# VIDILabs/instantvnr

Hardware: AMD Instinct MI355X
Metric: fps at 1024^2 on 1024^3 volume (higher is better)
Workload: dtype f16

## Files before the change

include/vnr_amd.h:

```cpp
#ifndef VNR_AMD_H
#define VNR_AMD_H

#include <stddef.h>
#include <stdint.h>

#ifdef __cplusplus
extern "C" {
#endif

#define VNR_AMD_OK 0
#define VNR_AMD_ERROR 1

typedef struct vnrAmdVolume_t*           vnrAmdVolume;
typedef struct vnrAmdRenderer_t*         vnrAmdRenderer;
typedef struct vnrAmdTransferFunction_t* vnrAmdTransferFunction;
typedef struct vnrAmdCamera_t*           vnrAmdCamera;

enum {
  VNR_AMD_OPTIX_NO_SHADING = 0,
  VNR_AMD_RAYMARCHING_NO_SHADING_DECODING = 4,
  VNR_AMD_RAYMARCHING_NO_SHADING_SAMPLE_STREAMING = 5,
  VNR_AMD_RAYMARCHING_NO_SHADING_IN_SHADER = 6,
  VNR_AMD_RAYMARCHING_GRADIENT_SHADING_SAMPLE_STREAMING = 8,
  VNR_AMD_RAYMARCHING_SINGLE_SHADE_HEURISTIC_SAMPLE_STREAMING = 11,
  VNR_AMD_PATHTRACING_SAMPLE_STREAMING = 14,
  VNR_AMD_INVALID = 16
};

enum {
  VNR_AMD_TYPE_UINT8 = 0, VNR_AMD_TYPE_INT8, VNR_AMD_TYPE_UINT16, VNR_AMD_TYPE_INT16,
  VNR_AMD_TYPE_UINT32, VNR_AMD_TYPE_INT32, VNR_AMD_TYPE_UINT64, VNR_AMD_TYPE_INT64,
  VNR_AMD_TYPE_FLOAT, VNR_AMD_TYPE_FLOAT2, VNR_AMD_TYPE_FLOAT3, VNR_AMD_TYPE_FLOAT4, VNR_AMD_TYPE_DOUBLE
};

enum {
  VNR_AMD_JSON_TEXT = 0,
  VNR_AMD_JSON_BSON = 1,
  VNR_AMD_JSON_TEXT_FILE = 2,
  VNR_AMD_JSON_BSON_FILE = 3
};

const char* vnrAmdGetLastError(void);
const char* vnrAmdVersion(void);
const char* vnrAmdBuildId(void);
int  vnrAmdInit(int device);
int  vnrAmdDeviceCount(void);
int  vnrAmdHasDevice(void);

void* vnrAmdMalloc(size_t bytes);
int   vnrAmdFree(void* d_ptr);
int   vnrAmdMemcpyH2D(void* d_dst, const void* h_src, size_t bytes);
int   vnrAmdMemcpyD2H(void* h_dst, const void* d_src, size_t bytes);
int   vnrAmdMemset(void* d_dst, int value, size_t bytes);
int   vnrAmdSynchronize(void);
void* vnrAmdDefaultStream(void);

int  vnrAmdJsonConvert(const void* data, size_t size, int format_in, int format_out ,
                       void** out, size_t* out_size);
int  vnrAmdJsonSave(const void* data, size_t size, int format_in, const char* filename, int format_out);
void vnrAmdFreeHost(void* p);

vnrAmdCamera vnrAmdCreateCamera(void);
int  vnrAmdCameraSet(vnrAmdCamera, const float from[3], const float at[3], const float up[3]);
int  vnrAmdCameraSetFromScene(vnrAmdCamera, const void* scene, size_t size, int format);
int  vnrAmdCameraSetFovy(vnrAmdCamera, float fovy_degrees);
int  vnrAmdCameraGet(vnrAmdCamera, float from[3], float at[3], float up[3], float* fovy);
void vnrAmdReleaseCamera(vnrAmdCamera);

vnrAmdTransferFunction vnrAmdCreateTransferFunction(void);
int  vnrAmdTransferFunctionSetColor(vnrAmdTransferFunction, const float* rgb, int n);
int  vnrAmdTransferFunctionSetAlpha(vnrAmdTransferFunction, const float* xy, int n);
int  vnrAmdTransferFunctionSetValueRange(vnrAmdTransferFunction, float lo, float hi);
int  vnrAmdTransferFunctionGetSizes(vnrAmdTransferFunction, int* n_colors, int* n_alphas);
int  vnrAmdTransferFunctionGet(vnrAmdTransferFunction, float* rgb, float* xy, float range[2]);
void vnrAmdReleaseTransferFunction(vnrAmdTransferFunction);

vnrAmdVolume vnrAmdCreateSimpleVolumeFromMemory(const void* host_data, const int dims[3], int value_type,
                                                float range_lo, float range_hi);
vnrAmdVolume vnrAmdCreateSimpleVolumeFromRawFile(const char* filename, const int dims[3], int value_type,
                                                 size_t offset, int big_endian, float range_lo, float range_hi);
vnrAmdVolume vnrAmdCreateSimpleVolumePerlin(const int dims[3], uint32_t seed, int octaves, float base_frequency);
const float* vnrAmdSimpleVolumeDeviceData(vnrAmdVolume);
vnrAmdVolume vnrAmdCreateSimpleVolumeOutOfCore(const char* filename, const int dims[3], int value_type, size_t offset,
                                               float range_lo, float range_hi, uint64_t n_concurrent_blocks, uint64_t n_blocks);
vnrAmdVolume vnrAmdCreateSimpleVolumeFromScene(const void* scene, size_t size, int format, const char* mode, int save_loaded_volume);
int  vnrAmdSimpleVolumeGetNumberOfTimeSteps(vnrAmdVolume);
int  vnrAmdSimpleVolumeSetCurrentTimeStep(vnrAmdVolume, int index);
int  vnrAmdSceneGetValueRange(const void* scene, size_t size, int format, float range[2]);
typedef struct vnrAmdOutOfCoreInfo {
  int file_dims[3];
  int block_dims[3];
  int block_index_space[3];
  uint64_t n_blocks, n_concurrent_blocks, block_size_aligned, bytes_read;
} vnrAmdOutOfCoreInfo;
int  vnrAmdSimpleVolumeOutOfCoreInfo(vnrAmdVolume, vnrAmdOutOfCoreInfo*);
int  vnrAmdSimpleVolumeOutOfCoreSetAsyncRefresh(vnrAmdVolume, int enable);
int  vnrAmdSimpleVolumeOutOfCoreRefreshStats(vnrAmdVolume, uint64_t* refreshes, uint64_t* steps_without_refresh);
int  vnrAmdSimpleVolumeOutOfCoreBlocks(vnrAmdVolume, int* block_index_yz, size_t n_slots);

vnrAmdVolume vnrAmdCreateNeuralVolume(const void* config, size_t size, int format, vnrAmdVolume groundtruth,
                                      int online_macrocell_construction);
vnrAmdVolume vnrAmdCreateNeuralVolumeFromDims(const void* config, size_t size, int format, const int dims[3]);
vnrAmdVolume vnrAmdCreateNeuralVolumeFromParams(const void* params, size_t size, int format);

int    vnrAmdNeuralVolumeSetModel(vnrAmdVolume, const void* config, size_t size, int format);
int    vnrAmdNeuralVolumeSetParams(vnrAmdVolume, const void* params, size_t size, int format);
double vnrAmdNeuralVolumeGetPSNR(vnrAmdVolume, int verbose);
double vnrAmdNeuralVolumeGetSSIM(vnrAmdVolume, int verbose);
double vnrAmdNeuralVolumeGetTestingLoss(vnrAmdVolume);
double vnrAmdNeuralVolumeGetTrainingLoss(vnrAmdVolume);
int    vnrAmdNeuralVolumeGetTrainingStep(vnrAmdVolume);
int    vnrAmdNeuralVolumeGetNumberOfBlobs(vnrAmdVolume);
int    vnrAmdNeuralVolumeTrain(vnrAmdVolume, int steps, int fast_mode);
int    vnrAmdNeuralVolumeDecodeProgressive(vnrAmdVolume);
int    vnrAmdNeuralVolumeDecodeInference(vnrAmdVolume, const char* filename);
int    vnrAmdNeuralVolumeDecodeReference(vnrAmdVolume, const char* filename);
const float* vnrAmdNeuralVolumeDecodedDeviceData(vnrAmdVolume);
int    vnrAmdNeuralVolumeSerializeParamsToFile(vnrAmdVolume, const char* filename);
int    vnrAmdNeuralVolumeSerializeParams(vnrAmdVolume, void** bson, size_t* size);

int    vnrAmdNeuralVolumeInference(vnrAmdVolume, size_t n, const float* d_coords, float* d_values, void* stream);
int    vnrAmdNeuralVolumeEncode(vnrAmdVolume, size_t n, const float* d_coords, uint16_t* d_features, void* stream);
int    vnrAmdNeuralVolumeBrickImageInfo(vnrAmdVolume, int* in_use, size_t* bytes, float* build_ms);
int    vnrAmdNeuralVolumeSetBrickImageMode(vnrAmdVolume, int mode);
int      vnrAmdNeuralVolumeSetBrickImageBudget(vnrAmdVolume, size_t bytes);
unsigned vnrAmdNeuralVolumeBrickImageLevels(vnrAmdVolume);
int      vnrAmdNeuralVolumeBrickImagePolicy(vnrAmdVolume, uint64_t* builds, unsigned* launches_before_next_build, int* tier, uint64_t* small_builds);
int      vnrAmdNeuralVolumeGridBackwardPlan(vnrAmdVolume, uint64_t batch, uint32_t out_u32[4], uint64_t out_u64[2]);
int      vnrAmdNeuralVolumeSetDeterministicTraining(vnrAmdVolume, int enable);
int      vnrAmdNeuralVolumeGetDeterministicTraining(vnrAmdVolume, int* enabled);
int    vnrAmdNeuralVolumeSetTrainProfiling(vnrAmdVolume, int enable);
int    vnrAmdNeuralVolumeGetTrainProfile(vnrAmdVolume, double ms_per_step[5], int* n_steps);
int    vnrAmdNeuralVolumeGetInfo(vnrAmdVolume, int* n_levels, int* n_features_per_level, int* padded_width,
                                 int* n_neurons, int* n_hidden_layers, uint64_t* n_params);
int    vnrAmdNeuralVolumeGetModelKind(vnrAmdVolume, int* activation, int* output_activation, int* grid_type, int* interpolation,
                                      int* mfma_inference, int* mfma_training);
int    vnrAmdNeuralVolumeLevelTable(vnrAmdVolume, int max_levels, uint32_t* resolution, uint32_t* entries, uint32_t* offset, uint32_t* kind);
int    vnrAmdNeuralVolumeGetParamsFP16(vnrAmdVolume, uint16_t* host_out, size_t count);
int    vnrAmdNeuralVolumeSetParamsFP16(vnrAmdVolume, const uint16_t* host_in, size_t count);

int    vnrAmdNeuralVolumeTrainBegin(vnrAmdVolume);
float* vnrAmdNeuralVolumeGradients(vnrAmdVolume, size_t* count);
int    vnrAmdNeuralVolumeTrainEnd(vnrAmdVolume, float grad_scale, int fast_mode);
int    vnrAmdNeuralVolumeForwardBackward(vnrAmdVolume, size_t n, const float* d_coords, const float* d_targets);
int    vnrAmdNeuralVolumeTrainingBuffer(vnrAmdVolume, int which, const void** d_ptr, size_t* bytes);
int    vnrAmdNeuralVolumeRescatterGridGradients(vnrAmdVolume, size_t n, const float* d_coords);
int    vnrAmdNeuralVolumeGradientDistance(vnrAmdVolume, const uint16_t* d_reference, double* out4);
int    vnrAmdNeuralVolumeSetSamplerSeed(vnrAmdVolume, uint64_t seed, uint64_t stream_id);
int    vnrAmdNeuralVolumeSetInitSeed(vnrAmdVolume, uint64_t seed);

int  vnrAmdVolumeSetClippingBox(vnrAmdVolume, const float lower[3], const float upper[3]);
int  vnrAmdVolumeSetScaling(vnrAmdVolume, const float scale[3]);
int  vnrAmdVolumeSetTransform(vnrAmdVolume, const float vx_vy_vz_p[12]);
int  vnrAmdSimpleVolumeGetDataRange(vnrAmdVolume, float range[2]);
int  vnrAmdVolumeGetValueRange(vnrAmdVolume, float range[2]);
int  vnrAmdVolumeGetDims(vnrAmdVolume, int dims[3]);
int  vnrAmdVolumeIsNetwork(vnrAmdVolume);
int  vnrAmdVolumeGetMacrocell(vnrAmdVolume, int mc_dims[3], float mc_spacings[3], const float** d_value_range,
                              const float** d_max_opacity);
void vnrAmdReleaseVolume(vnrAmdVolume);

vnrAmdRenderer vnrAmdCreateRenderer(vnrAmdVolume);
int  vnrAmdRendererSetFramebufferSize(vnrAmdRenderer, int width, int height);
int  vnrAmdRendererSetTransferFunction(vnrAmdRenderer, vnrAmdTransferFunction);
int  vnrAmdRendererSetCamera(vnrAmdRenderer, vnrAmdCamera);
int  vnrAmdRendererSetMode(vnrAmdRenderer, int mode);
int  vnrAmdRendererSetDenoiser(vnrAmdRenderer, int enable);
int  vnrAmdRendererSetVolumeSamplingRate(vnrAmdRenderer, float rate);
int  vnrAmdRendererSetVolumeDensityScale(vnrAmdRenderer, float scale);
int  vnrAmdRendererResetAccumulation(vnrAmdRenderer);
int  vnrAmdRender(vnrAmdRenderer);
const float* vnrAmdRendererMapFrame(vnrAmdRenderer);
int  vnrAmdRendererSetOutputAsDeviceFramebuffer(vnrAmdRenderer, int enable);
int  vnrAmdRendererSetPixelRange(vnrAmdRenderer, uint32_t pixel_lo, uint32_t pixel_hi);
int  vnrAmdRendererSetPixelInterleave(vnrAmdRenderer, uint32_t block_pixels, uint32_t n_parts, uint32_t part);

typedef struct {
  uint64_t n_samples;
  uint64_t n_reference_slots;
  uint32_t n_iterations;
  uint32_t n_rays_hit;
  double   infer_kernel_ms;
  uint64_t infer_kernel_launches;
  double   infer_union_ms;
} vnrAmdFrameStats;
int  vnrAmdRendererGetFrameStats(vnrAmdRenderer, vnrAmdFrameStats*);
int  vnrAmdRendererSetProfiling(vnrAmdRenderer, int enable);
int  vnrAmdRendererSetAsync(vnrAmdRenderer, int enable);
int  vnrAmdRendererSetInShaderKernel(vnrAmdRenderer, int mode);
int  vnrAmdRendererDebugQueues(vnrAmdRenderer, const float** d_coords, const uint32_t** d_counters, float* iteration_ms, int max_iterations);
int  vnrAmdRendererDebugSchedule(vnrAmdRenderer, int out[4]);
void vnrAmdReleaseRenderer(vnrAmdRenderer);

int  vnrAmdDistGetUniqueId(void* out128);
int  vnrAmdDistInit(int rank, int world_size, int local_rank, const void* unique_id, const char* transport, const char* address);
int  vnrAmdDistInitFromEnv(void);
int  vnrAmdDistFinalize(void);
int  vnrAmdDistRank(void);
int  vnrAmdDistWorldSize(void);
const char* vnrAmdDistTransport(void);
int  vnrAmdDistRcclRanksSeen(void);
int  vnrAmdDistBarrier(void);
int  vnrAmdDistAllReduceHost(double* values, int n, int op);
int  vnrAmdDistAllReduce(void* buf, size_t count, int dtype, int op);
int  vnrAmdDistAllGather(const void* send, void* recv, size_t bytes_per_rank);
int  vnrAmdDistReduceScatter(void* buf, size_t count_per_rank, int dtype);
int  vnrAmdDistBroadcast(void* buf, size_t bytes, int root);
int  vnrAmdDistSelfTest(double deadline_s, char* report, size_t report_size);
int  vnrAmdRendererSetDistributed(vnrAmdRenderer, int enable);
const float* vnrAmdRendererGatherFrame(vnrAmdRenderer);
int  vnrAmdRendererRenderPipelined(vnrAmdRenderer, const float** previous_frame);
int  vnrAmdRendererGetCompletedFrameStats(vnrAmdRenderer, vnrAmdFrameStats*);
int  vnrAmdRendererFlushPipeline(vnrAmdRenderer, const float** last_frame);
int  vnrAmdNeuralVolumeTrainDataParallel(vnrAmdVolume, int steps, int fast_mode);
int  vnrAmdNeuralVolumeSyncReplicas(vnrAmdVolume);
int  vnrAmdNeuralVolumeAllReduceGradients(vnrAmdVolume);
int  vnrAmdNeuralVolumeTrainEndDataParallel(vnrAmdVolume, int fast_mode, int sharded);
int  vnrAmdNeuralVolumeSetGradients(vnrAmdVolume, const float* host, size_t count);

int  vnrAmdMarchingCube(vnrAmdVolume, float isovalue, float** xyz, size_t* n_vertices, int on_device);
int  vnrAmdSaveTriangles(const char* filename, const float* xyz, size_t n_vertices);

void vnrAmdMemoryQuery(size_t* used_by_renderer, size_t* used_by_network);
void vnrAmdFreeTemporaryGPUMemory(void);

int  vnrAmdSimpleVolumeTakeSamples(vnrAmdVolume, size_t n, const float lower[3], const float upper[3],
                                   float* d_coords, float* d_values, void* stream);
int  vnrAmdSimpleVolumeTakeSamplesGrid(vnrAmdVolume, const int origin[3], const int size[3], float* d_coords, float* d_values,
                                       void* stream);
int  vnrAmdSimpleVolumeSample(vnrAmdVolume, size_t n, const float* d_coords, float* d_values, int nodal, void* stream);
int  vnrAmdNeuralVolumeUpdateMacrocell(vnrAmdVolume, size_t n, const float* d_coords, const float* d_values, void* stream);
int  vnrAmdVolumeUpdateMaxOpacity(vnrAmdVolume, vnrAmdTransferFunction);

#ifdef __cplusplus
}
#endif
#endif
```

instantvnr_amd/_lib.py:

```python
import ctypes as C
import os
import re
import subprocess
import sys

_HERE = os.path.dirname(os.path.abspath(__file__))
ROOT = os.path.dirname(_HERE)
SO_PATH = os.environ.get("VNR_AMD_LIB_PATH") or os.path.join(_HERE, "libvnr_amd.so")
HEADER = os.path.join(ROOT, "include", "vnr_amd.h")

_lib = None
_torch_imported_before_load = None


class VnrAmdError(RuntimeError):
    pass


def require_torch_loaded_first():
    if _lib is not None and not _torch_imported_before_load:
        raise VnrAmdError("libvnr_amd.so was loaded before `import torch`: PyTorch's bundled ROCm runtime cannot share the "
                          "GPU with the system runtime the library already initialised.  Import torch first (instantvnr_amd."
                          "dist.init_from_env does when WORLD_SIZE > 1; tests/conftest.py does for the test session).")


def build(force=False):
    args = ["make", "-C", os.path.join(_HERE, "csrc"), "-j8", "-s"]
    if force:
        subprocess.check_call(args + ["clean"])
    subprocess.check_call(args)
    return SO_PATH


class FrameStats(C.Structure):
    _fields_ = [("n_samples", C.c_uint64), ("n_reference_slots", C.c_uint64), ("n_iterations", C.c_uint32),
                ("n_rays_hit", C.c_uint32), ("infer_kernel_ms", C.c_double), ("infer_kernel_launches", C.c_uint64), ("infer_union_ms", C.c_double)]


class OutOfCoreInfo(C.Structure):
    _fields_ = [("file_dims", C.c_int * 3), ("block_dims", C.c_int * 3), ("block_index_space", C.c_int * 3),
                ("n_blocks", C.c_uint64), ("n_concurrent_blocks", C.c_uint64), ("block_size_aligned", C.c_uint64),
                ("bytes_read", C.c_uint64)]


def declared_symbols():
    text = open(HEADER).read()
    text = re.sub(r"/\*.*?\*/", "", text, flags=re.S)
    return sorted(set(re.findall(r"\b(vnrAmd[A-Za-z0-9_]+)\s*\(", text)))


def lib():
    global _lib
    if _lib is not None:
        return _lib
    if not os.path.exists(SO_PATH):
        raise VnrAmdError(f"{SO_PATH} is missing: run `python -c 'import __graft_entry__ as g; g.build()'` "
                          "(there is no CPU fallback)")
    global _torch_imported_before_load
    _torch_imported_before_load = "torch" in sys.modules
    L = C.CDLL(SO_PATH)
    P, I, U32, U64, F, D, SZ = C.c_void_p, C.c_int, C.c_uint32, C.c_uint64, C.c_float, C.c_double, C.c_size_t
    FP = C.POINTER(C.c_float)
    IP = C.POINTER(C.c_int)

    def sig(name, res, *args):
        fn = getattr(L, name)
        fn.restype = res
        fn.argtypes = list(args)

    sig("vnrAmdGetLastError", C.c_char_p)
    sig("vnrAmdBuildId", C.c_char_p)
    sig("vnrAmdVersion", C.c_char_p)
    sig("vnrAmdInit", I, I)
    sig("vnrAmdDeviceCount", I)
    sig("vnrAmdHasDevice", I)
    sig("vnrAmdMalloc", P, SZ)
    sig("vnrAmdFree", I, P)
    sig("vnrAmdMemcpyH2D", I, P, P, SZ)
    sig("vnrAmdMemcpyD2H", I, P, P, SZ)
    sig("vnrAmdMemset", I, P, I, SZ)
    sig("vnrAmdSynchronize", I)
    sig("vnrAmdDefaultStream", P)
    sig("vnrAmdJsonConvert", I, P, SZ, I, I, C.POINTER(P), C.POINTER(SZ))
    sig("vnrAmdJsonSave", I, P, SZ, I, C.c_char_p, I)
    sig("vnrAmdFreeHost", None, P)
    sig("vnrAmdCreateCamera", P)
    sig("vnrAmdCameraSet", I, P, FP, FP, FP)
    sig("vnrAmdCameraSetFovy", I, P, F)
    sig("vnrAmdCameraGet", I, P, FP, FP, FP, FP)
    sig("vnrAmdReleaseCamera", None, P)
    sig("vnrAmdCreateTransferFunction", P)
    sig("vnrAmdTransferFunctionSetColor", I, P, FP, I)
    sig("vnrAmdTransferFunctionSetAlpha", I, P, FP, I)
    sig("vnrAmdTransferFunctionSetValueRange", I, P, F, F)
    sig("vnrAmdTransferFunctionGetSizes", I, P, IP, IP)
    sig("vnrAmdTransferFunctionGet", I, P, FP, FP, FP)
    sig("vnrAmdReleaseTransferFunction", None, P)
    sig("vnrAmdCreateSimpleVolumeFromMemory", P, P, IP, I, F, F)
    sig("vnrAmdCreateSimpleVolumeFromRawFile", P, C.c_char_p, IP, I, SZ, I, F, F)
    sig("vnrAmdCreateSimpleVolumePerlin", P, IP, U32, I, F)
    sig("vnrAmdSimpleVolumeDeviceData", P, P)
    sig("vnrAmdCreateSimpleVolumeOutOfCore", P, C.c_char_p, IP, I, SZ, F, F, U64, U64)
    sig("vnrAmdCreateSimpleVolumeFromScene", P, P, SZ, I, C.c_char_p, I)
    sig("vnrAmdSimpleVolumeGetNumberOfTimeSteps", I, P)
    sig("vnrAmdSimpleVolumeSetCurrentTimeStep", I, P, I)
    sig("vnrAmdSceneGetValueRange", I, P, SZ, I, FP)
    sig("vnrAmdCameraSetFromScene", I, P, P, SZ, I)
    sig("vnrAmdSimpleVolumeOutOfCoreInfo", I, P, C.POINTER(OutOfCoreInfo))
    sig("vnrAmdSimpleVolumeOutOfCoreBlocks", I, P, IP, SZ)
    sig("vnrAmdSimpleVolumeOutOfCoreSetAsyncRefresh", I, P, I)
    sig("vnrAmdSimpleVolumeOutOfCoreRefreshStats", I, P, C.POINTER(C.c_uint64), C.POINTER(C.c_uint64))
    sig("vnrAmdCreateNeuralVolume", P, P, SZ, I, P, I)
    sig("vnrAmdCreateNeuralVolumeFromDims", P, P, SZ, I, IP)
    sig("vnrAmdCreateNeuralVolumeFromParams", P, P, SZ, I)
    sig("vnrAmdNeuralVolumeSetModel", I, P, P, SZ, I)
    sig("vnrAmdNeuralVolumeSetParams", I, P, P, SZ, I)
    sig("vnrAmdNeuralVolumeGetPSNR", D, P, I)
    sig("vnrAmdNeuralVolumeGetSSIM", D, P, I)
    sig("vnrAmdNeuralVolumeGetTestingLoss", D, P)
    sig("vnrAmdNeuralVolumeGetTrainingLoss", D, P)
    sig("vnrAmdNeuralVolumeGetTrainingStep", I, P)
    sig("vnrAmdNeuralVolumeGetNumberOfBlobs", I, P)
    sig("vnrAmdNeuralVolumeTrain", I, P, I, I)
    sig("vnrAmdNeuralVolumeSerializeParamsToFile", I, P, C.c_char_p)
    sig("vnrAmdNeuralVolumeDecodeProgressive", I, P)
    sig("vnrAmdNeuralVolumeDecodeInference", I, P, C.c_char_p)
    sig("vnrAmdNeuralVolumeDecodeReference", I, P, C.c_char_p)
    sig("vnrAmdNeuralVolumeDecodedDeviceData", P, P)
    sig("vnrAmdNeuralVolumeSerializeParams", I, P, C.POINTER(P), C.POINTER(SZ))
    sig("vnrAmdNeuralVolumeInference", I, P, SZ, P, P, P)
    sig("vnrAmdNeuralVolumeEncode", I, P, SZ, P, P, P)
    sig("vnrAmdNeuralVolumeBrickImageInfo", I, P, IP, C.POINTER(SZ), FP)
    sig("vnrAmdNeuralVolumeGetInfo", I, P, IP, IP, IP, IP, IP, C.POINTER(U64))
    sig("vnrAmdNeuralVolumeGetModelKind", I, P, IP, IP, IP, IP, IP, IP)
    sig("vnrAmdNeuralVolumeLevelTable", I, P, I, P, P, P, P)
    sig("vnrAmdNeuralVolumeGetParamsFP16", I, P, P, SZ)
    sig("vnrAmdNeuralVolumeSetParamsFP16", I, P, P, SZ)
    sig("vnrAmdNeuralVolumeTrainBegin", I, P)
    sig("vnrAmdNeuralVolumeGradients", P, P, C.POINTER(SZ))
    sig("vnrAmdNeuralVolumeTrainEnd", I, P, F, I)
    sig("vnrAmdNeuralVolumeForwardBackward", I, P, SZ, P, P)
    sig("vnrAmdNeuralVolumeTrainingBuffer", I, P, I, C.POINTER(P), C.POINTER(SZ))
    sig("vnrAmdNeuralVolumeRescatterGridGradients", I, P, SZ, P)
    sig("vnrAmdNeuralVolumeGradientDistance", I, P, P, C.POINTER(C.c_double))
    sig("vnrAmdNeuralVolumeSetSamplerSeed", I, P, U64, U64)
    sig("vnrAmdNeuralVolumeSetInitSeed", I, P, U64)
    sig("vnrAmdVolumeSetClippingBox", I, P, FP, FP)
    sig("vnrAmdVolumeSetScaling", I, P, FP)
    sig("vnrAmdVolumeSetTransform", I, P, FP)
    sig("vnrAmdSimpleVolumeGetDataRange", I, P, FP)
    sig("vnrAmdMarchingCube", I, P, F, C.POINTER(C.POINTER(C.c_float)), C.POINTER(SZ), I)
    sig("vnrAmdSaveTriangles", I, C.c_char_p, C.POINTER(C.c_float), SZ)
    sig("vnrAmdVolumeGetValueRange", I, P, FP)
    sig("vnrAmdVolumeGetDims", I, P, IP)
    sig("vnrAmdVolumeIsNetwork", I, P)
    sig("vnrAmdVolumeGetMacrocell", I, P, IP, FP, C.POINTER(P), C.POINTER(P))
    sig("vnrAmdReleaseVolume", None, P)
    sig("vnrAmdCreateRenderer", P, P)
    sig("vnrAmdRendererSetFramebufferSize", I, P, I, I)
    sig("vnrAmdRendererSetTransferFunction", I, P, P)
    sig("vnrAmdRendererSetCamera", I, P, P)
    sig("vnrAmdRendererSetMode", I, P, I)
    sig("vnrAmdRendererSetDenoiser", I, P, I)
    sig("vnrAmdRendererSetVolumeSamplingRate", I, P, F)
    sig("vnrAmdRendererSetVolumeDensityScale", I, P, F)
    sig("vnrAmdRendererResetAccumulation", I, P)
    sig("vnrAmdRender", I, P)
    sig("vnrAmdRendererMapFrame", P, P)
    sig("vnrAmdRendererSetOutputAsDeviceFramebuffer", I, P, I)
    sig("vnrAmdRendererSetPixelRange", I, P, U32, U32)
    sig("vnrAmdRendererSetPixelInterleave", I, P, U32, U32, U32)
    sig("vnrAmdRendererGetFrameStats", I, P, C.POINTER(FrameStats))
    sig("vnrAmdRendererSetProfiling", I, P, I)
    sig("vnrAmdRendererSetAsync", I, P, I)
    sig("vnrAmdRendererSetInShaderKernel", I, P, I)
    sig("vnrAmdRendererDebugQueues", I, P, C.POINTER(P), C.POINTER(P), FP, I)
    sig("vnrAmdRendererDebugSchedule", I, P, IP)
    sig("vnrAmdReleaseRenderer", None, P)
    sig("vnrAmdDistGetUniqueId", I, P)
    sig("vnrAmdDistInit", I, I, I, I, P, C.c_char_p, C.c_char_p)
    sig("vnrAmdDistInitFromEnv", I)
    sig("vnrAmdDistFinalize", I)
    sig("vnrAmdDistRank", I)
    sig("vnrAmdDistWorldSize", I)
    sig("vnrAmdDistTransport", C.c_char_p)
    sig("vnrAmdDistRcclRanksSeen", I)
    sig("vnrAmdDistBarrier", I)
    sig("vnrAmdDistAllReduceHost", I, C.POINTER(D), I, I)
    sig("vnrAmdDistAllReduce", I, P, SZ, I, I)
    sig("vnrAmdDistAllGather", I, P, P, SZ)
    sig("vnrAmdDistReduceScatter", I, P, SZ, I)
    sig("vnrAmdDistBroadcast", I, P, SZ, I)
    sig("vnrAmdDistSelfTest", I, C.c_double, C.c_char_p, SZ)
    sig("vnrAmdRendererSetDistributed", I, P, I)
    sig("vnrAmdRendererGatherFrame", P, P)
    sig("vnrAmdRendererRenderPipelined", I, P, C.POINTER(P))
    sig("vnrAmdRendererGetCompletedFrameStats", I, P, C.POINTER(FrameStats))
    sig("vnrAmdRendererFlushPipeline", I, P, C.POINTER(P))
    sig("vnrAmdNeuralVolumeTrainDataParallel", I, P, I, I)
    sig("vnrAmdNeuralVolumeSyncReplicas", I, P)
    sig("vnrAmdNeuralVolumeSetBrickImageMode", I, P, I)
    sig("vnrAmdNeuralVolumeSetBrickImageBudget", I, P, SZ)
    sig("vnrAmdNeuralVolumeBrickImageLevels", C.c_uint, P)
    sig("vnrAmdNeuralVolumeGridBackwardPlan", I, P, U64, C.POINTER(U32), C.POINTER(U64))
    sig("vnrAmdNeuralVolumeSetDeterministicTraining", I, P, I)
    sig("vnrAmdNeuralVolumeGetDeterministicTraining", I, P, C.POINTER(I))
    sig("vnrAmdNeuralVolumeBrickImagePolicy", I, P, C.POINTER(U64), C.POINTER(C.c_uint), IP, C.POINTER(U64))
    sig("vnrAmdNeuralVolumeSetTrainProfiling", I, P, I)
    sig("vnrAmdNeuralVolumeGetTrainProfile", I, P, C.POINTER(D), IP)
    sig("vnrAmdNeuralVolumeAllReduceGradients", I, P)
    sig("vnrAmdNeuralVolumeTrainEndDataParallel", I, P, I, I)
    sig("vnrAmdNeuralVolumeSetGradients", I, P, C.POINTER(C.c_float), SZ)
    sig("vnrAmdMemoryQuery", None, C.POINTER(SZ), C.POINTER(SZ))
    sig("vnrAmdFreeTemporaryGPUMemory", None)
    sig("vnrAmdSimpleVolumeTakeSamples", I, P, SZ, FP, FP, P, P, P)
    sig("vnrAmdSimpleVolumeTakeSamplesGrid", I, P, IP, IP, P, P, P)
    sig("vnrAmdSimpleVolumeSample", I, P, SZ, P, P, I, P)
    sig("vnrAmdNeuralVolumeUpdateMacrocell", I, P, SZ, P, P, P)
    sig("vnrAmdVolumeUpdateMaxOpacity", I, P, P)
    _lib = L
    return L


def last_error():
    return lib().vnrAmdGetLastError().decode("utf-8", "replace")


def check(status):
    if status != 0:
        raise VnrAmdError(last_error())


def check_ptr(p):
    if not p:
        raise VnrAmdError(last_error())
    return p


def require_device():
    if not lib().vnrAmdHasDevice():
        raise VnrAmdError("no HIP device: the MI355X path has no CPU fallback")
```

instantvnr_amd/api.py:

```python
import ctypes as C
import json

import numpy as np

from . import _lib
from ._lib import VnrAmdError, check, check_ptr, lib

JSON_TEXT, JSON_BSON, JSON_TEXT_FILE, JSON_BSON_FILE = 0, 1, 2, 3

VALUE_TYPES = {np.dtype(np.uint8): 0, np.dtype(np.int8): 1, np.dtype(np.uint16): 2, np.dtype(np.int16): 3,
               np.dtype(np.uint32): 4, np.dtype(np.int32): 5, np.dtype(np.float32): 8, np.dtype(np.float64): 12}


def _fp(a):
    return a.ctypes.data_as(C.POINTER(C.c_float))


def _vec(v, n=3):
    a = np.ascontiguousarray(v, dtype=np.float32).ravel()
    assert a.size == n
    return a


def _json_arg(j, params=False):
# ... 424 lines not shown
    check(lib().vnrAmdRendererSetFramebufferSize(r.h, int(size[0]), int(size[1])))
    r._size = (int(size[0]), int(size[1]))


def vnrRendererSetTransferFunction(r, t):
    check(lib().vnrAmdRendererSetTransferFunction(r.h, t.h))


def vnrRendererSetCamera(r, cam):
    check(lib().vnrAmdRendererSetCamera(r.h, cam.h))


def vnrRendererSetMode(r, mode):
    check(lib().vnrAmdRendererSetMode(r.h, int(mode)))


def vnrRendererSetDenoiser(r, flag):
    check(lib().vnrAmdRendererSetDenoiser(r.h, 1 if flag else 0))


def vnrRendererSetVolumeSamplingRate(r, v):
    check(lib().vnrAmdRendererSetVolumeSamplingRate(r.h, float(v)))


def vnrRendererSetVolumeDensityScale(r, v):
    check(lib().vnrAmdRendererSetVolumeDensityScale(r.h, float(v)))


def vnrRendererResetAccumulation(r):
    check(lib().vnrAmdRendererResetAccumulation(r.h))


def vnrRender(r):
    check(lib().vnrAmdRender(r.h))


def vnrRendererMapFrame(r):
    p = check_ptr(lib().vnrAmdRendererMapFrame(r.h))
    if r._device_output:
        return p
    w, h = r._size
    return np.ctypeslib.as_array(C.cast(p, C.POINTER(C.c_float)), shape=(h, w, 4))


def vnrMemoryQuery():
    r, n = C.c_size_t(), C.c_size_t()
    lib().vnrAmdMemoryQuery(C.byref(r), C.byref(n))
    return r.value, n.value


def vnrFreeTemporaryGPUMemory():
    lib().vnrAmdFreeTemporaryGPUMemory()


def vnrRendererSetPixelRange(r, lo, hi):
    check(lib().vnrAmdRendererSetPixelRange(r.h, int(lo), int(hi)))


def vnrRendererSetPixelInterleave(r, block_pixels, n_parts, part):
    check(lib().vnrAmdRendererSetPixelInterleave(r.h, int(block_pixels), int(n_parts), int(part)))


def vnrRendererSetOutputAsDeviceFramebuffer(r, flag):
    check(lib().vnrAmdRendererSetOutputAsDeviceFramebuffer(r.h, 1 if flag else 0))
    r._device_output = bool(flag)


def vnrRendererSetProfiling(r, flag):
    check(lib().vnrAmdRendererSetProfiling(r.h, 1 if flag else 0))


def vnrRendererGetFrameStats(r):
    s = _lib.FrameStats()
    check(lib().vnrAmdRendererGetFrameStats(r.h, C.byref(s)))
    return {k: getattr(s, k) for k, _ in s._fields_}


def renderer_schedule(r):
    out = (C.c_int * 4)()
    check(lib().vnrAmdRendererDebugSchedule(r.h, out))
    return {"n_iters": out[0], "n_parts": out[1], "fused_pack": bool(out[2]), "decoupled": bool(out[3])}


def neural_brick_image(v):
    u, b, ms = C.c_int(), C.c_size_t(), C.c_float()
    check(lib().vnrAmdNeuralVolumeBrickImageInfo(v.h, C.byref(u), C.byref(b), C.byref(ms)))
    builds, after, tier, small = C.c_uint64(), C.c_uint(), C.c_int(), C.c_uint64()
    check(lib().vnrAmdNeuralVolumeBrickImagePolicy(v.h, C.byref(builds), C.byref(after), C.byref(tier), C.byref(small)))
    return {"in_use": bool(u.value), "bytes": b.value, "build_ms": ms.value, "levels": int(lib().vnrAmdNeuralVolumeBrickImageLevels(v.h)),
            "builds": int(builds.value), "launches_before_next_build": int(after.value), "tier": int(tier.value), "small_builds": int(small.value)}


def neural_set_brick_budget(v, n_bytes):
    check(lib().vnrAmdNeuralVolumeSetBrickImageBudget(v.h, int(n_bytes)))


def neural_info(v):
    vals = [C.c_int() for _ in range(5)]
    n = C.c_uint64()
    check(lib().vnrAmdNeuralVolumeGetInfo(v.h, *[C.byref(x) for x in vals], C.byref(n)))
    keys = ["n_levels", "n_features_per_level", "padded_width", "n_neurons", "n_hidden_layers"]
    d = {k: x.value for k, x in zip(keys, vals)}
    d["n_params"] = n.value
    kind = [C.c_int() for _ in range(6)]
    check(lib().vnrAmdNeuralVolumeGetModelKind(v.h, *[C.byref(x) for x in kind]))
    d.update({k: x.value for k, x in zip(["activation", "output_activation", "grid_type", "interpolation", "mfma_kernels", "mfma_training_kernels"], kind)})
    return d


def neural_grid_backward_plan(v, batch=65536):
    u32, u64 = (C.c_uint32 * 4)(), (C.c_uint64 * 2)()
    check(lib().vnrAmdNeuralVolumeGridBackwardPlan(v.h, int(batch), u32, u64))
    return {"n_levels": u32[0], "lds_levels": u32[1], "tile_entries": u32[2], "lds_blocks": u32[3], "atomic_requests": int(u64[0]), "flush_requests_at_most": int(u64[1])}


def neural_set_deterministic_training(v, enable=True):
    check(lib().vnrAmdNeuralVolumeSetDeterministicTraining(v.h, 1 if enable else 0))


def neural_get_deterministic_training(v):
    e = C.c_int()
    check(lib().vnrAmdNeuralVolumeGetDeterministicTraining(v.h, C.byref(e)))
    return bool(e.value)


def neural_level_table(v):
    a = [np.zeros(32, np.uint32) for _ in range(4)]
    n = lib().vnrAmdNeuralVolumeLevelTable(v.h, 32, *[x.ctypes.data_as(C.c_void_p) for x in a])
    if n < 0:
        check(1)
    return [{"res": int(a[0][l]), "entries": int(a[1][l]), "offset": int(a[2][l]), "kind": int(a[3][l])} for l in range(n)]


def neural_set_params_fp16(v, params):
    p = np.ascontiguousarray(params).view(np.uint16)
    check(lib().vnrAmdNeuralVolumeSetParamsFP16(v.h, p.ctypes.data_as(C.c_void_p), p.size))


def neural_get_params_fp16(v):
    n = neural_info(v)["n_params"]
    p = np.empty(n, dtype=np.uint16)
    check(lib().vnrAmdNeuralVolumeGetParamsFP16(v.h, p.ctypes.data_as(C.c_void_p), n))
    return p.view(np.float16)


def neural_inference(v, coords):
    c = DeviceArray.from_numpy(np.ascontiguousarray(coords, dtype=np.float32))
    o = DeviceArray((c.shape[0],), np.float32)
    check(lib().vnrAmdNeuralVolumeInference(v.h, c.shape[0], c.ptr, o.ptr, None))
    check(lib().vnrAmdSynchronize())
    return o.numpy()


def neural_encode(v, coords):
    info = neural_info(v)
    c = DeviceArray.from_numpy(np.ascontiguousarray(coords, dtype=np.float32))
    o = DeviceArray((c.shape[0], info["padded_width"]), np.uint16)
    check(lib().vnrAmdNeuralVolumeEncode(v.h, c.shape[0], c.ptr, o.ptr, None))
    check(lib().vnrAmdSynchronize())
    return o.numpy().view(np.float16)


def volume_macrocell(v):
    dims = (C.c_int * 3)()
    sp = (C.c_float * 3)()
    vr, mo = C.c_void_p(), C.c_void_p()
    check(lib().vnrAmdVolumeGetMacrocell(v.h, dims, sp, C.byref(vr), C.byref(mo)))
    n = dims[0] * dims[1] * dims[2]
    value_range = np.empty((dims[2], dims[1], dims[0], 2), np.float32)
    max_opacity = np.empty((dims[2], dims[1], dims[0]), np.float32)
    check(lib().vnrAmdMemcpyD2H(value_range.ctypes.data_as(C.c_void_p), vr, n * 8))
    check(lib().vnrAmdMemcpyD2H(max_opacity.ctypes.data_as(C.c_void_p), mo, n * 4))
    return {"dims": tuple(dims), "spacings": np.array(list(sp), np.float32), "value_range": value_range,
            "max_opacity": max_opacity}


def simple_volume_sample(v, coords, nodal):
    c = DeviceArray.from_numpy(np.ascontiguousarray(coords, dtype=np.float32))
    o = DeviceArray((c.shape[0],), np.float32)
    check(lib().vnrAmdSimpleVolumeSample(v.h, c.shape[0], c.ptr, o.ptr, 1 if nodal else 0, None))
    check(lib().vnrAmdSynchronize())
    return o.numpy()


def simple_volume_take_samples_grid(v, origin, size):
    n = int(size[0]) * int(size[1]) * int(size[2])
    c = DeviceArray((n, 3), np.float32)
    o = DeviceArray((n,), np.float32)
    check(lib().vnrAmdSimpleVolumeTakeSamplesGrid(v.h, (C.c_int * 3)(*[int(x) for x in origin]), (C.c_int * 3)(*[int(x) for x in size]),
                                                  c.ptr, o.ptr, None))
    check(lib().vnrAmdSynchronize())
    return c.numpy(), o.numpy()


def simple_volume_take_samples(v, n, lower=(0, 0, 0), upper=(1, 1, 1)):
    c = DeviceArray((n, 3), np.float32)
    o = DeviceArray((n,), np.float32)
    check(lib().vnrAmdSimpleVolumeTakeSamples(v.h, n, _fp(_vec(lower)), _fp(_vec(upper)), c.ptr, o.ptr, None))
    check(lib().vnrAmdSynchronize())
    return c.numpy(), o.numpy()


def neural_forward_backward(v, coords, targets):
    c = DeviceArray.from_numpy(np.ascontiguousarray(coords, dtype=np.float32))
    t = DeviceArray.from_numpy(np.ascontiguousarray(targets, dtype=np.float32))
    check(lib().vnrAmdNeuralVolumeForwardBackward(v.h, c.shape[0], c.ptr, t.ptr))
    return neural_gradients(v)


def neural_gradients(v):
    n = C.c_size_t()
    p = check_ptr(lib().vnrAmdNeuralVolumeGradients(v.h, C.byref(n)))
    check(lib().vnrAmdSynchronize())
    out = np.empty(n.value, np.float32)
    check(lib().vnrAmdMemcpyD2H(out.ctypes.data_as(C.c_void_p), p, n.value * 4))
    return out


def neural_train_begin(v):
    check(lib().vnrAmdNeuralVolumeTrainBegin(v.h))


def neural_train_end(v, grad_scale=1.0, fast_mode=True):
    check(lib().vnrAmdNeuralVolumeTrainEnd(v.h, float(grad_scale), 1 if fast_mode else 0))
```

instantvnr_amd/csrc/capi.cpp:

```cpp
#include "../../include/vnr_amd.h"

#include <cstdlib>
#include <cstdio>
#include <fstream>
#include <memory>

#include "dist.h"
#include "renderer.h"
#include "scene.h"

using namespace vnr;

struct vnrAmdVolume_t { std::shared_ptr<VolumeBase> v; };
struct vnrAmdRenderer_t { std::unique_ptr<Renderer> r; std::shared_ptr<VolumeBase> volume; };
struct vnrAmdTransferFunction_t { TransferFunctionData d; };
struct vnrAmdCamera_t { CameraData d; };

namespace {
thread_local std::string g_last_error;

template <typename F>
int guarded(F&& f)
{
  try {
// ... 380 lines not shown
    for (size_t i = 0; i < b.size(); ++i) { block_index_yz[2 * i] = b[i].index_y; block_index_yz[2 * i + 1] = b[i].index_z; }
  });
}
const float* vnrAmdSimpleVolumeDeviceData(vnrAmdVolume v)
{
  const float* p = nullptr;
  guarded([&]() { p = as_simple(v)->d_data(); });
  return p;
}

vnrAmdVolume vnrAmdCreateNeuralVolume(const void* config, size_t size, int format, vnrAmdVolume groundtruth, int online_mc)
{
  return guarded_new<vnrAmdVolume_t>([&]() {
    SimpleVolume* src = as_simple(groundtruth);
    const Json cfg = resolve_config(parse_json_arg(config, size, format));
    auto nv = std::make_shared<NeuralVolume>();
    if (const char* e = std::getenv("VNR_AMD_INIT_SEED")) nv->init_seed = std::strtoull(e, nullptr, 10);
    nv->keep_source_alive(groundtruth->v);
    nv->set_network(src->dims(), cfg, src, !online_mc);
    auto* h = new vnrAmdVolume_t();
    h->v = nv;
    return h;
  });
}
vnrAmdVolume vnrAmdCreateNeuralVolumeFromDims(const void* config, size_t size, int format, const int dims[3])
{
  return guarded_new<vnrAmdVolume_t>([&]() {
    const Json cfg = resolve_config(parse_json_arg(config, size, format));
    auto nv = std::make_shared<NeuralVolume>();
    if (const char* e = std::getenv("VNR_AMD_INIT_SEED")) nv->init_seed = std::strtoull(e, nullptr, 10);
    nv->set_network({dims[0], dims[1], dims[2]}, cfg, nullptr, false);
    auto* h = new vnrAmdVolume_t();
    h->v = nv;
    return h;
  });
}
vnrAmdVolume vnrAmdCreateNeuralVolumeFromParams(const void* params, size_t size, int format)
{
  return guarded_new<vnrAmdVolume_t>([&]() {
    const Json p = resolve_params(parse_json_arg(params, size, format));
    if (!p.contains("volume")) throw std::runtime_error("expecting a model config with volume dims tag");
    const Json& d = p.at("volume").at("dims");
    const vec3i dims = {(int)d.at("x").as_int(), (int)d.at("y").as_int(), (int)d.at("z").as_int()};
    auto nv = std::make_shared<NeuralVolume>();
    nv->init_seed = 1;
    nv->set_network(dims, p.at("model"), nullptr, false);
    nv->load_params_from_json(p);
    auto* h = new vnrAmdVolume_t();
    h->v = nv;
    return h;
  });
}
int vnrAmdNeuralVolumeSetModel(vnrAmdVolume v, const void* config, size_t size, int format)
{
  return guarded([&]() { as_neural(v)->set_model(resolve_config(parse_json_arg(config, size, format))); });
}
int vnrAmdNeuralVolumeSetParams(vnrAmdVolume v, const void* params, size_t size, int format)
{
  return guarded([&]() { as_neural(v)->load_params_from_json(resolve_params(parse_json_arg(params, size, format))); });
}
double vnrAmdNeuralVolumeGetPSNR(vnrAmdVolume v, int verbose)
{
  double r = -1.0;
  guarded([&]() { r = as_neural(v)->get_psnr(!verbose); });
  return r;
}
double vnrAmdNeuralVolumeGetSSIM(vnrAmdVolume v, int verbose)
{
  double r = -1.0;
  guarded([&]() { r = as_neural(v)->get_ssim(!verbose); });
  return r;
}
double vnrAmdNeuralVolumeGetTestingLoss(vnrAmdVolume v)
{
  double r = -1.0;
  guarded([&]() { r = as_neural(v)->test_loss(); });
  return r;
}
double vnrAmdNeuralVolumeGetTrainingLoss(vnrAmdVolume v)
{
  double r = -1.0;
  guarded([&]() { NeuralVolume* n = as_neural(v); r = n->network().training_loss(n->stream); });
  return r;
}
int vnrAmdNeuralVolumeGetTrainingStep(vnrAmdVolume v)
{
  int r = -1;
  guarded([&]() { r = (int)as_neural(v)->network().steps(); });
  return r;
}
int vnrAmdNeuralVolumeGetNumberOfBlobs(vnrAmdVolume v)
{
  int r = -1;
  guarded([&]() { r = as_neural(v)->num_blobs(); });
  return r;
}
int vnrAmdNeuralVolumeTrain(vnrAmdVolume v, int steps, int fast_mode)
{
  return guarded([&]() { as_neural(v)->train((size_t)std::max(steps, 0), fast_mode != 0); });
}
int vnrAmdNeuralVolumeDecodeProgressive(vnrAmdVolume v)
{
  return guarded([&]() { as_neural(v)->decode_progressive(); });
}
int vnrAmdNeuralVolumeDecodeInference(vnrAmdVolume v, const char* filename)
{
  return guarded([&]() {
    if (!filename) throw std::runtime_error("filename is null");
    as_neural(v)->save_inference_volume(filename);
  });
}
int vnrAmdNeuralVolumeDecodeReference(vnrAmdVolume v, const char* filename)
{
  return guarded([&]() {
    if (!filename) throw std::runtime_error("filename is null");
    as_neural(v)->save_reference_volume(filename);
  });
}
const float* vnrAmdNeuralVolumeDecodedDeviceData(vnrAmdVolume v)
{
  const float* r = nullptr;
  guarded([&]() { r = as_neural(v)->decoded_data(); });
  return r;
}
int vnrAmdNeuralVolumeSerializeParamsToFile(vnrAmdVolume v, const char* filename)
{
  return guarded([&]() {
    Json root = Json::object();
    as_neural(v)->save_params_to_json(root);
    const std::vector<uint8_t> b = root.to_bson();
    std::ofstream ofs(filename, std::ios::binary | std::ios::out);
    ofs.write((const char*)b.data(), (std::streamsize)b.size());
    if (!ofs) throw std::runtime_error(std::string("cannot write ") + filename);
  });
}
int vnrAmdNeuralVolumeSerializeParams(vnrAmdVolume v, void** bson, size_t* size)
{
  return guarded([&]() {
    Json root = Json::object();
    as_neural(v)->save_params_to_json(root);
    const std::vector<uint8_t> b = root.to_bson();
    *bson = dup_bytes(b.data(), b.size());
    *size = b.size();
  });
}
int vnrAmdNeuralVolumeInference(vnrAmdVolume v, size_t n, const float* d_coords, float* d_values, void* stream)
{
  return guarded([&]() {
    NeuralVolume* nv = as_neural(v);
    if (!nv->network().valid()) throw std::runtime_error("network is not valid");
    nv->inference(n, d_coords, d_values, resolve_stream(stream));
  });
}
int vnrAmdNeuralVolumeEncode(vnrAmdVolume v, size_t n, const float* d_coords, uint16_t* d_features, void* stream)
{
  return guarded([&]() { as_neural(v)->network().encode(d_coords, d_features, n, resolve_stream(stream)); });
}
int vnrAmdNeuralVolumeBrickImageInfo(vnrAmdVolume v, int* in_use, size_t* bytes, float* build_ms)
{
  return guarded([&]() {
    Network& n = as_neural(v)->network();
    if (in_use) *in_use = n.brick_image_in_use() ? 1 : 0;
    if (bytes) *bytes = n.brick_image_bytes();
    if (build_ms) *build_ms = n.brick_build_ms();
  });
}
int vnrAmdNeuralVolumeGetModelKind(vnrAmdVolume v, int* activation, int* output_activation, int* grid_type, int* interpolation, int* mfma_inference,
                                   int* mfma_training)
{
  return guarded([&]() {
    Network& n = as_neural(v)->network();
    if (activation) *activation = (int)n.config().activation;
    if (output_activation) *output_activation = (int)n.config().output_activation;
    if (grid_type) *grid_type = (int)n.config().grid_type;
    if (interpolation) *interpolation = (int)n.config().interpolation;
    if (mfma_inference) *mfma_inference = 1;
    if (mfma_training) *mfma_training = 1;
  });
}

int vnrAmdNeuralVolumeGetInfo(vnrAmdVolume v, int* n_levels, int* n_features, int* padded_width, int* n_neurons,
                              int* n_hidden_layers, uint64_t* n_params)
{
  return guarded([&]() {
    Network& n = as_neural(v)->network();
    if (n_levels) *n_levels = (int)n.config().n_levels;
    if (n_features) *n_features = (int)n.config().n_features;
    if (padded_width) *padded_width = (int)n.padded_width();
    if (n_neurons) *n_neurons = (int)n.config().n_neurons;
    if (n_hidden_layers) *n_hidden_layers = (int)n.config().n_hidden_layers;
    if (n_params) *n_params = (uint64_t)n.n_params();
  });
}
int vnrAmdNeuralVolumeLevelTable(vnrAmdVolume v, int max_levels, uint32_t* resolution, uint32_t* entries, uint32_t* offset, uint32_t* kind)
{
  int n = -1;
  guarded([&]() {
    const Network& net = as_neural(v)->network();
    const GridDevice& g = net.grid();
    n = (int)net.config().n_levels;
    for (int l = 0; l < n && l < max_levels; ++l) {
      if (resolution) resolution[l] = g.levels[l].resolution;
      if (entries) entries[l] = g.levels[l].size;
      if (offset) offset[l] = g.levels[l].offset;
      if (kind) kind[l] = g.levels[l].hashed;
    }
  });
  return n;
}
int vnrAmdNeuralVolumeGetParamsFP16(vnrAmdVolume v, uint16_t* host_out, size_t count)
{
  return guarded([&]() { NeuralVolume* n = as_neural(v); n->network().get_params_f16(host_out, count, n->stream); });
}
int vnrAmdNeuralVolumeSetParamsFP16(vnrAmdVolume v, const uint16_t* host_in, size_t count)
{
  return guarded([&]() { NeuralVolume* n = as_neural(v); n->network().set_params_f16(host_in, count, n->stream); });
}
int vnrAmdNeuralVolumeTrainBegin(vnrAmdVolume v) { return guarded([&]() { as_neural(v)->train_begin(); }); }
float* vnrAmdNeuralVolumeGradients(vnrAmdVolume v, size_t* count)
{
  float* p = nullptr;
  guarded([&]() {
    NeuralVolume* nv = as_neural(v);
    Network& n = nv->network();
    p = n.grads_as_f32(nv->stream);
    if (count) *count = n.grads_count();
  });
  return p;
}
int vnrAmdNeuralVolumeTrainEnd(vnrAmdVolume v, float grad_scale, int fast_mode)
{
  return guarded([&]() { as_neural(v)->train_end(grad_scale, fast_mode != 0); });
}
int vnrAmdNeuralVolumeForwardBackward(vnrAmdVolume v, size_t n, const float* d_coords, const float* d_targets)
{
  return guarded([&]() { as_neural(v)->forward_backward(d_coords, d_targets, n); });
}
int vnrAmdNeuralVolumeTrainingBuffer(vnrAmdVolume v, int which, const void** d_ptr, size_t* bytes)
{
  return guarded([&]() {
    size_t b = 0;
    const void* p = as_neural(v)->network().training_buffer(which, &b);
    if (d_ptr) *d_ptr = p;
    if (bytes) *bytes = b;
  });
}
int vnrAmdNeuralVolumeRescatterGridGradients(vnrAmdVolume v, size_t n, const float* d_coords)
{
  return guarded([&]() { NeuralVolume* nv = as_neural(v); nv->network().rescatter_grid_gradients(d_coords, n, nv->stream); });
}
int vnrAmdNeuralVolumeGradientDistance(vnrAmdVolume v, const uint16_t* d_reference, double* out4)
{
  return guarded([&]() { NeuralVolume* nv = as_neural(v); nv->network().gradient_distance(d_reference, out4, nv->stream); });
}
int vnrAmdNeuralVolumeSetSamplerSeed(vnrAmdVolume v, uint64_t seed, uint64_t stream_id)
{
  return guarded([&]() {
    NeuralVolume* n = as_neural(v);
    if (!n->source()) throw std::runtime_error("missing a reference volume");
    n->source()->set_sampler_seed(seed, stream_id);
  });
}
int vnrAmdNeuralVolumeSetInitSeed(vnrAmdVolume v, uint64_t seed)
{
  return guarded([&]() { as_neural(v)->init_seed = seed; });
}

int vnrAmdVolumeSetClippingBox(vnrAmdVolume v, const float lower[3], const float upper[3])
{
  return guarded([&]() {
    if (!v || !v->v) throw std::runtime_error("null volume");
    VolumeBase& vb = *v->v;
    const vec3f half = {vb.desc.dims.x / 2.0f, vb.desc.dims.y / 2.0f, vb.desc.dims.z / 2.0f};
    const affine3f inv = affine_inverse(vb.transform);
    vb.clipbox.lower = xfm_point(inv, vec3f{lower[0], lower[1], lower[2]} - half);
    vb.clipbox.upper = xfm_point(inv, vec3f{upper[0], upper[1], upper[2]} - half);
  });
}
int vnrAmdVolumeSetScaling(vnrAmdVolume v, const float scale[3])
{
  return guarded([&]() {
    if (!v || !v->v) throw std::runtime_error("null volume");
    v->v->transform = affine_scale_then({scale[0], scale[1], scale[2]}, v->v->transform);
  });
}
int vnrAmdMarchingCube(vnrAmdVolume v, float isovalue, float** xyz, size_t* n_vertices, int on_device)
{
  return guarded([&]() {
    if (!v || !v->v) throw std::runtime_error("null volume");
    if (!xyz || !n_vertices) throw std::runtime_error("null output pointer");
    DeviceBuffer<vec3f> verts;
    const size_t n = marching_cubes(*v->v, isovalue, verts);
    *n_vertices = n;
    *xyz = nullptr;
    if (on_device) {
      *xyz = (float*)verts.ptr;
      verts.counter() -= verts.count * sizeof(vec3f);
      verts.ptr = nullptr; verts.count = 0;
    } else if (n) {
      float* h = (float*)std::malloc(n * sizeof(vec3f));
      if (!h) throw std::runtime_error("out of host memory");
      const hipError_t e = hipMemcpy(h, verts.ptr, n * sizeof(vec3f), hipMemcpyDeviceToHost);
      if (e != hipSuccess) { std::free(h); throw std::runtime_error("device to host copy of the vertices failed"); }
      *xyz = h;
    }
  });
// ... 344 lines not shown
```

instantvnr_amd/csrc/decoupled.h:

```cpp
#pragma once

namespace vnr {

struct DRays {
  uint32_t* pixel; float* jitter; vec3i* cell; vec3f* t_next; float* ncb; uint32_t* walking;
  float* alpha; vec3f* color; uint32_t* done;
};

enum { D_SAMPLES = 0, D_WALKING, D_HIT, D_TICKET_W, D_TICKET_C, D_NREF, D_NSMP, D_COUNT = 8 };
constexpr uint32_t kRecValid = 1u << 16, kRecLast = 1u << 17;

struct DRing {
  vec4f* queue;
  vec2f* arena;
  uint32_t* rec;
  uint32_t* ctr;
};

struct DHost {
  uint32_t walking[256], emitted[256], n_ref[256], n_smp[256];
  uint32_t hit;
};

template <bool FIRST>
__global__ void __launch_bounds__(256) walk_kernel(const RenderParams p, const DRays r, const DRing ring, DHost* __restrict__ host, uint32_t it)
{
  extern __shared__ float s_t[];
  float* s_t0 = s_t;
  float* s_t1 = s_t + (size_t)p.n_iters * 256;
  uint32_t* s_hist = (uint32_t*)(s_t + (size_t)2 * p.n_iters * 256);
  uint32_t* s_claim = s_hist + 256;
  uint16_t* s_rk = (uint16_t*)(s_claim + 16);
  const uint32_t tid = threadIdx.x, lane = tid & 63u;
  const uint32_t P = p.n_local;
  const uint32_t n_round = (P + 255u) & ~255u;
  uint32_t trip = 0;
  uint32_t n_walking = 0, n_hit = 0;
  vec4f* __restrict__ queue = ring.queue;
  vec2f* __restrict__ vd_out = ring.arena;

  for (uint32_t base = blockIdx.x * 256u; base < n_round; base += gridDim.x * 256u) {
    const uint32_t i = base + tid;
    const bool active = i < P;
    uint32_t pixel = 0;
    float jitter = 0.0f;
    DDAState it_;
    it_.t_next = {0, 0, 0}; it_.cell = {0, 0, 0}; it_.next_cell_begin = 0.0f;
    vec3f org = {0, 0, 0}, dir = {0, 0, 1}, m_dir = {0, 0, 1};
    float tmin = 0.0f, tmax = VNR_FLOAT_LARGE;
    bool walk = false;
    if (active) {
      if (FIRST) {
        if (map_pixel(p, i, pixel)) {
          jitter = tea_lcg_first((uint32_t)p.frame_index, pixel);
          compute_ray(p, pixel, org, dir);
          m_dir = dir * p.mc_rcp;
          walk = intersect_box(tmin, tmax, org, dir, p.bbox_lo, p.bbox_hi);
          if (walk) {
            dda_init(it_, org * p.mc_rcp, m_dir, tmin, p.mc_dims);
            r.pixel[i] = pixel; r.jitter[i] = jitter;
            r.alpha[i] = 0.0f; r.color[i] = {0, 0, 0}; r.done[i] = 0u;
            ++n_hit;
          } else {
            write_pixel(p, {0, 0, 0, 0}, pixel);
          }
        }
      } else if (r.walking[i]) {
        if (r.done[i]) {
          r.walking[i] = 0u;
        } else {
          pixel = r.pixel[i];
          jitter = r.jitter[i];
          it_.cell = r.cell[i];
          it_.t_next = r.t_next[i];
          it_.next_cell_begin = r.ncb[i];
          compute_ray(p, pixel, org, dir);
          m_dir = dir * p.mc_rcp;
          intersect_box(tmin, tmax, org, dir, p.bbox_lo, p.bbox_hi);
          walk = true;
        }
      }
    }
    uint32_t k = 0;
    bool last = false;
    if (walk) {
      const int n_iters = p.n_iters;
      iter_exec(p, it_, m_dir, tmin, tmax, p.step, [&](float t0, float t1) -> bool {
        s_t0[k * 256u + tid] = t0;
        s_t1[k * 256u + tid] = t1;
        return (int)(++k) < n_iters;
      });
      last = k == 0 || !dda_resumable(it_, m_dir, tmin, tmax, p.mc_dims);
      r.walking[i] = last ? 0u : 1u;
      if (!last) { r.cell[i] = it_.cell; r.t_next[i] = it_.t_next; r.ncb[i] = it_.next_cell_begin; ++n_walking; }
    } else if (FIRST && active) {
      r.walking[i] = 0u;
    }
    if (active) ring.rec[i] = walk ? (k | kRecValid | (last ? kRecLast : 0u)) : 0u;

    uint32_t incl = k;
#pragma unroll
    for (int d = 1; d < 64; d <<= 1) {
      const uint32_t y = __shfl_up(incl, d);
      if ((int)lane >= d) incl += y;
    }
    const uint32_t wave_samples = __shfl(incl, 63);
    uint32_t* claim = s_claim + 8u * (trip & 1u);
    if (lane == 0) claim[tid >> 6] = wave_samples;
    __syncthreads();
    if (tid == 0) {
      const uint32_t total = claim[0] + claim[1] + claim[2] + claim[3];
      claim[4] = total ? atomicAdd(ring.ctr + D_SAMPLES, total) : 0u;
    }
    __syncthreads();
    uint32_t smp_base = claim[4];
    for (uint32_t w = 0; w < (tid >> 6); ++w) smp_base += claim[w];
    ++trip;
    if (wave_samples == 0) continue;

    const bool emit = k > 0;
    float front = emit ? s_t0[tid] : VNR_FLOAT_LARGE;
#pragma unroll
    for (int d = 32; d > 0; d >>= 1) front = fminf(front, __shfl_xor(front, d));
    uint32_t* hist = s_hist + (tid & ~63u);
    hist[lane] = 0;
    __builtin_amdgcn_wave_barrier();
    if (emit) {
      for (uint32_t j = 0; j < k; ++j) {
        const float t0 = s_t0[j * 256u + tid], t1 = s_t1[j * 256u + tid];
        const float t = (1.0f - jitter) * t0 + jitter * t1;
        s_rk[j * 256u + tid] = (uint16_t)atomicAdd(&hist[depth_bin(p, t, front)], 1u);
      }
    }
    __builtin_amdgcn_wave_barrier();
    const uint32_t h = hist[lane];
    uint32_t hs = h;
#pragma unroll
    for (int d = 1; d < 64; d <<= 1) {
      const uint32_t y = __shfl_up(hs, d);
      if ((int)lane >= d) hs += y;
    }
    hist[lane] = smp_base + hs - h;
    __builtin_amdgcn_wave_barrier();
    if (emit) {
      const uint32_t sb = (i >> 6) * (uint32_t)p.n_iters * 64u + lane;
      for (uint32_t j = 0; j < k; ++j) {
        const float t0 = s_t0[j * 256u + tid], t1 = s_t1[j * 256u + tid];
        const float t = (1.0f - jitter) * t0 + jitter * t1;
        const vec3f c = org + t * dir;
        const uint32_t g = hist[depth_bin(p, t, front)] + s_rk[j * 256u + tid];
        if (g < p.slot_cap) queue[g] = {c.x, c.y, c.z, __uint_as_float(arena_value_index(sb + 64u * j))};
        vd_out[sb + 64u * j].y = t1 - t0;
      }
    }
    __builtin_amdgcn_wave_barrier();
  }

  __syncthreads();
#pragma unroll
  for (int d = 32; d > 0; d >>= 1) { n_walking += __shfl_xor(n_walking, d); n_hit += __shfl_xor(n_hit, d); }
  if (lane == 0) { s_hist[tid >> 6] = n_walking; s_hist[4 + (tid >> 6)] = n_hit; }
  __syncthreads();
// ... 100 lines not shown
```

instantvnr_amd/csrc/infer_kernel.h:

```cpp
#pragma once
#include <algorithm>
#include <cstdlib>

#include "infer_tile.h"
#include "pack_rays.h"

namespace vnr {

struct FusedMlp {
  const uint16_t* packed;
  uint32_t lds_halves, width, n_hidden_matmuls, activation, output_activation;
  bool general;
  bool weights_global;
  float quantize_threshold;
};

struct InferArgs {
  const LevelInfo* levels;
  uint32_t n_levels, interpolation;
  const half_t* table;
  uint32_t table_bytes;
  const uint8_t* brick_image;
  const half_t* packed_mlp;
  const float* coords;
  float* out;
  half_t* features_out;
  half_t* acts_out;
  const uint32_t* n_ptr;
  const uint32_t* dest;
  uint32_t queue_mode;
  uint32_t out_stride;
  uint32_t n;
  uint32_t n_hidden_matmuls;
  uint32_t activation;
  uint32_t output_activation;
  uint32_t lds_halves;
  uint32_t sharers;
  uint32_t weights_global;
  float quantize_threshold;
  PackArgs pack;
};

template <int F, int K_IN, int W, int MODE, bool GENERAL>
__global__ void __launch_bounds__(64 * MlpShape<W>::WAVES) fused_infer_kernel(const InferArgs args)
{
  constexpr int NCHUNK = K_IN / 8;
  constexpr uint32_t WAVES = MlpShape<W>::WAVES;
  extern __shared__ __attribute__((aligned(16))) half_t lds[];

  const uint32_t lane = threadIdx.x & 63u;
  const uint32_t wave = threadIdx.x >> 6;

  if (MODE == 0 && WAVES == 4 && args.pack.n_blocks) {
    uint32_t* s_part = (uint32_t*)lds;
    for (uint32_t item = blockIdx.x; item < args.pack.n_blocks; item += gridDim.x) {
      pack_rays_block<4>(args.pack, item, s_part);
      __syncthreads();
    }
  }
  const uint32_t n = args.n_ptr ? min(*args.n_ptr, args.n) : args.n;
  const uint32_t n_tiles = (n + 63u) >> 6;
  const uint32_t xcd = blockIdx.x & 7u;
  const uint32_t per_xcd = (n_tiles + 7u) >> 3;
  const uint32_t waves_per_xcd = (gridDim.x >> 3) * WAVES;
  const uint32_t tile_end = min(n_tiles, (xcd + 1u) * per_xcd);
  if (xcd * per_xcd + (blockIdx.x >> 3) * WAVES >= tile_end) return;

  constexpr bool CAN_GLOBAL = GENERAL;
  const bool wglobal = CAN_GLOBAL && args.weights_global != 0u;
  if (MODE != 1 && !wglobal) {
    const uint4_t* src = (const uint4_t*)args.packed_mlp;
    uint4_t* dst = (uint4_t*)lds;
    for (uint32_t i = threadIdx.x; i < args.lds_halves / 8; i += blockDim.x) dst[i] = src[i];
    __syncthreads();
  }
  const uint32_t nh = args.n_hidden_matmuls;
  const uint32_t act = args.activation;
  const uint32_t h = lane >> 5;
  const uint32_t r = lane & 31u;
  const table_rsrc_t rsrc = make_table_rsrc(args.table, args.table_bytes);

  for (uint32_t tile = xcd * per_xcd + (blockIdx.x >> 3) * WAVES + wave; tile < tile_end; tile += waves_per_xcd) {
    const uint32_t i = tile * 64u + lane;
    const uint32_t ic = min(i, n - 1u);
    float3_packed p;
    uint32_t out_index = i;
    if (args.queue_mode) {
      const uint4_t rec = ((const uint4_t*)args.coords)[ic];
      p = {__uint_as_float(rec.x), __uint_as_float(rec.y), __uint_as_float(rec.z)};
      out_index = rec.w * args.out_stride;
    } else {
      p = ((const float3_packed*)args.coords)[ic];
      if (args.dest) out_index = args.dest[ic];
    }

    half8_t feat[NCHUNK];
    encode_tile<F, K_IN, GENERAL>(args.levels, args.n_levels, args.interpolation, rsrc, args.brick_image, p.x, p.y, p.z, feat,
                                  GENERAL ? args.quantize_threshold : 0.0f);

    if (MODE != 0 && args.features_out && i < n) {
      half8_t* dst = (half8_t*)(args.features_out + (size_t)i * K_IN);
#pragma unroll
      for (int c = 0; c < NCHUNK; ++c) dst[c] = feat[c];
    }
    if (MODE == 1) continue;

    float y;
    if (CAN_GLOBAL && wglobal)
      y = mlp_tile<W, K_IN, MODE == 2, GENERAL>(args.packed_mlp, feat, nh, act, h, r, args.acts_out, n, tile * 64u);
    else
      y = mlp_tile<W, K_IN, MODE == 2, GENERAL>((const half_t*)lds, feat, nh, act, h, r, args.acts_out, n, tile * 64u);
    if (i < n) args.out[out_index] = finish_output<GENERAL>(y, args.output_activation);
  }
}

template <int F, int K_IN, int W, int MODE, bool GENERAL>
static void launch_one(const InferArgs& a, size_t n_max, hipStream_t s)
{
  constexpr uint32_t WAVES = MlpShape<W>::WAVES;
  const Runtime& rt = Runtime::get();
  const uint32_t n_tiles = div_round_up(n_max, 64);
  uint32_t blocks = div_round_up(n_tiles, WAVES);
  static const uint32_t forced = [] {
    const char* e = std::getenv("VNR_AMD_INFER_BLOCKS_PER_CU");
    const int v = e ? std::atoi(e) : 0;
    return (uint32_t)(v >= 1 && v <= 64 ? v : 0);
  }();
  const size_t shmem = (MODE == 1 || a.weights_global) ? 16 : (size_t)a.lds_halves * sizeof(uint16_t);
  const uint32_t fit = (uint32_t)std::max<size_t>(1, std::min<size_t>(4, (160 * 1024) / std::max<size_t>(shmem, 1)));
  uint32_t max_blocks = (uint32_t)rt.n_cus * (forced ? forced : std::min(fit, a.sharers >= 2 ? 3u : 4u));
  if (!forced && a.n_ptr && a.queue_mode) max_blocks = std::min((uint32_t)rt.n_cus * 32u, std::max((uint32_t)rt.n_cus * 4u, n_tiles / 33u));
  if (blocks > max_blocks) blocks = max_blocks;
  blocks = next_multiple(blocks, 8);
  auto kernel = fused_infer_kernel<F, K_IN, W, MODE, GENERAL>;
  static bool attr_set = false;
  if (!attr_set) {
    VNR_HIP_CHECK(hipFuncSetAttribute((const void*)kernel, hipFuncAttributeMaxDynamicSharedMemorySize, 160 * 1024));
    attr_set = true;
  }
  kernel<<<blocks, 64 * WAVES, shmem, s>>>(a);
  VNR_HIP_CHECK(hipGetLastError());
}

template <int W, int MODE, bool GENERAL>
static void dispatch(uint32_t F, uint32_t K_IN, const InferArgs& a, size_t n_max, hipStream_t s)
{
#define VNR_CASE(f, k) if (F == f && K_IN == k) return launch_one<f, k, W, MODE, GENERAL>(a, n_max, s)
  VNR_CASE(1, 16); VNR_CASE(1, 32);
  VNR_CASE(2, 16); VNR_CASE(2, 32); VNR_CASE(2, 48); VNR_CASE(2, 64);
  VNR_CASE(4, 16); VNR_CASE(4, 32); VNR_CASE(4, 48); VNR_CASE(4, 64); VNR_CASE(4, 80); VNR_CASE(4, 96); VNR_CASE(4, 112); VNR_CASE(4, 128);
  VNR_CASE(8, 16); VNR_CASE(8, 32); VNR_CASE(8, 48); VNR_CASE(8, 64); VNR_CASE(8, 80); VNR_CASE(8, 96); VNR_CASE(8, 112); VNR_CASE(8, 128);
#undef VNR_CASE
  throw std::runtime_error("unsupported encoding shape: n_features_per_level=" + std::to_string(F) +
                           " padded width=" + std::to_string(K_IN));
}

#define VNR_DEFINE_FUSED_WIDTH(W, GENERAL, SUFFIX)                                                                        \
  void launch_fused_w##W##SUFFIX(int mode, uint32_t F, uint32_t K_IN, const InferArgs& a, size_t n_max, hipStream_t s)    \
  {                                                                                                                       \
    if (mode == 0) dispatch<W, 0, GENERAL>(F, K_IN, a, n_max, s);                                                         \
    else dispatch<W, 2, GENERAL>(F, K_IN, a, n_max, s);                                                                   \
  }

}
```

instantvnr_amd/csrc/network.h:

```cpp
#pragma once

#include <functional>
#include <utility>
#include <vector>

#include "common.h"
#include "json.h"

namespace vnr {

constexpr int kMaxLevels = 32;
constexpr size_t kLdsBytes = 160 * 1024;
constexpr int kLossScale = 128;

struct LevelInfo {
  float scale;
  uint32_t resolution;
  uint32_t res2;
  uint32_t size;
  uint32_t offset;
  uint32_t hashed;
  uint32_t brick;
  uint32_t pad1;
};

template <int F> struct BrickShape;
template <> struct BrickShape<1> { static constexpr uint32_t lx = 2, ly = 2, lz = 2; };
template <> struct BrickShape<2> { static constexpr uint32_t lx = 2, ly = 2, lz = 1; };
template <> struct BrickShape<4> { static constexpr uint32_t lx = 2, ly = 1, lz = 1; };
template <> struct BrickShape<8> { static constexpr uint32_t lx = 1, ly = 1, lz = 1; };

struct GridDevice {
  LevelInfo levels[kMaxLevels];
  uint32_t n_levels;
  uint32_t n_features;
  uint32_t interpolation;
};

struct ModelConfig {
  uint32_t n_levels = 8, n_features = 8, log2_hashmap_size = 19, base_resolution = 16;
  float per_level_scale = 2.0f;
  uint32_t interpolation = 0;
  float quantize_threshold = 0.0f;
  float max_level = 1000.0f;
  uint32_t grid_type = 0;
  uint32_t n_neurons = 64, n_hidden_layers = 4;
  uint32_t activation = 1;
  uint32_t output_activation = 0;
  float learning_rate = 5e-3f, beta1 = 0.9f, beta2 = 0.999f, epsilon = 1e-15f, l2_reg = 1e-6f;
  uint32_t decay_start = 2000, decay_interval = 1000;
  float decay_base = 0.99f;
  bool has_decay = true;
  uint32_t loss = 0;
};

struct alignas(16) OptState {
  float master;
  float m, v;
  uint32_t step;
};
static_assert(sizeof(OptState) == 16, "OptState must be one 16-byte record");

struct TileNet;
struct PackArgs;
struct FusedMlp;

struct GradExchange {
  virtual ~GradExchange() = default;
  virtual void range_ready(size_t lo, size_t hi, hipStream_t s) = 0;
  virtual size_t bucket_params() const { return (size_t)16u << 20; }
};

struct GridBackwardPlan {
  uint32_t n_levels, lds_levels, tile_entries, lds_blocks;
  uint64_t atomic_requests, flush_requests_at_most;
};

class Network {
public:
  Network() = default;
  void configure(const Json& model, uint64_t init_seed);
  bool valid() const { return n_params_ > 0; }

  const ModelConfig& config() const { return cfg_; }
  const Json& model_json() const { return model_; }
  const GridDevice& grid() const { return grid_; }
  uint32_t padded_width() const { return in_width_; }
  uint32_t width() const { return cfg_.n_neurons; }
  uint32_t lds_halves() const { return lds_halves_; }
  bool weights_in_lds() const { return (size_t)lds_halves_ * 2 <= kLdsBytes; }
  bool common_kind() const
  {
    return cfg_.activation <= 1u && cfg_.output_activation == 0u && cfg_.interpolation != 2u && cfg_.grid_type != 2u && cfg_.quantize_threshold == 0.0f &&
           weights_in_lds();
  }
  uint32_t n_active_levels() const;
  uint32_t n_hidden_matmuls() const { return cfg_.n_hidden_layers - 1; }
  size_t n_params() const { return n_params_; }
  size_t n_mlp_params() const { return n_mlp_; }
  size_t n_grid_params() const { return n_params_ - n_mlp_; }
  size_t model_size_bytes() const { return n_params_ * sizeof(uint16_t); }
  uint64_t steps() const { return steps_; }

  void set_params_f16(const uint16_t* host, size_t count, hipStream_t s);
  void get_params_f16(uint16_t* host, size_t count, hipStream_t s) const;
  Json serialize_params(hipStream_t s) const;
  void deserialize_params(const Json& j, hipStream_t s);

  void inference(const float* d_coords, float* d_out, size_t n, const uint32_t* d_n, size_t n_max, hipStream_t s,
                 const uint32_t* d_dest = nullptr) const;
  bool tile_net(TileNet* out, hipStream_t s) const;
  bool inference_queue(const float* d_records, float* d_out, uint32_t out_stride, const uint32_t* d_n, size_t n_max, hipStream_t s,
                       uint32_t sharers = 1, const PackArgs* pack = nullptr) const;
  void encode(const float* d_coords, uint16_t* d_features, size_t n, hipStream_t s) const;

  void forward_backward(const float* d_coords, const float* d_targets, size_t batch, hipStream_t s, GradExchange* exchange = nullptr);
  uint16_t* grads_f16() { return grads_.ptr; }
  size_t grads_count() const { return grads_.count ? n_params_ : 0; }
  size_t grads_alloc() const { return n_params_ + (n_params_ & 1); }
  float* grads_as_f32(hipStream_t s);
  void optimizer_step(float grad_scale, hipStream_t s);
  void optimizer_step_range(size_t lo, size_t hi, float grad_scale, hipStream_t s);
  void optimizer_finish_step(hipStream_t s);
  float learning_rate() const { return lr_; }
  uint16_t* params_device() { return params_f16_.ptr; }
  OptState* opt_state_device() { return opt_state_.ptr; }
  void set_replica_state(uint64_t steps, float lr, hipStream_t s) { steps_ = steps; lr_ = lr; refresh_inference_weights(s); }
  void ensure_training_state(hipStream_t s);
  void reset_master_from_params(hipStream_t s);
  double training_loss(hipStream_t s);
  uint64_t params_generation() const { return params_generation_; }
  void set_opt_sharded(bool e) { opt_sharded_ = e; }
  bool opt_sharded() const { return opt_sharded_; }
  void set_deterministic(bool e) { deterministic_ = e; }
  bool deterministic() const { return deterministic_; }
  static bool deterministic_default();
  std::vector<std::pair<uint32_t, uint32_t>> exchange_level_buckets(size_t bucket) const;
  void for_each_exchange_range(size_t bucket, const std::function<void(size_t, size_t)>& fn) const;
  size_t level_range_lo(uint32_t level) const { return n_mlp_ + (size_t)grid_.levels[level].offset * cfg_.n_features; }
  size_t level_range_hi(uint32_t level_end) const { return n_mlp_ + ((size_t)grid_.levels[level_end - 1].offset + grid_.levels[level_end - 1].size) * cfg_.n_features; }
  const void* training_buffer(int which, size_t* bytes) const;
  void rescatter_grid_gradients(const float* d_coords, size_t n, hipStream_t s);
  void gradient_distance(const uint16_t* d_ref, double out[4], hipStream_t s);
  void scatter_grid_gradients(const float* d_coords, size_t batch, hipStream_t s, GradExchange* exchange, hipStream_t s_lds = nullptr);
  void set_grads_from_f32(const float* host, size_t count, hipStream_t s);

  size_t bytes_allocated() const;
  void release_temporary();
  static void release_temporary_of_all();

  void set_brick_resolution_cap(uint32_t cap) { brick_res_cap_ = cap; }
  void set_brick_mode(int mode);
  void set_brick_budget(size_t bytes);
  GridBackwardPlan grid_backward_plan(size_t batch) const;
  uint32_t brick_levels_mask() const { return brick_levels_mask_; }
  bool brick_image_in_use() const { return brick_valid_; }
  size_t brick_image_bytes() const { return brick_image_.bytes(); }
  float brick_build_ms() const { return brick_build_ms_; }
  uint64_t brick_builds() const { return brick_builds_; }
  uint64_t brick_small_builds() const { return brick_small_builds_; }
  int brick_tier() const { return brick_valid_ ? brick_tier_ : 0; }
  uint32_t brick_after_now() const;

private:
  void build_layout();
  void initialize_params(uint64_t seed, hipStream_t s);
  void refresh_inference_weights(hipStream_t s);
  FusedMlp fused_mlp() const;
  const LevelInfo* inference_levels(hipStream_t s, const uint8_t** image, size_t n_max) const;
  void build_brick_image(hipStream_t s, bool small) const;
  static double brick_small_budget();

  ModelConfig cfg_;
  Json model_;
  GridDevice grid_{};
  uint32_t in_width_ = 0;
  size_t n_params_ = 0, n_mlp_ = 0;
  uint64_t steps_ = 0;
  uint64_t params_generation_ = 0;
  bool opt_sharded_ = false;
  bool deterministic_ = deterministic_default();
  float lr_ = 0.0f;

  DeviceBuffer<uint16_t> params_f16_{MemTag::Network};
  DeviceBuffer<uint16_t> mlp_packed_{MemTag::Network};
  DeviceBuffer<uint16_t> mlp_packed_T_{MemTag::Network};
  DeviceBuffer<LevelInfo> levels_dev_{MemTag::Network};
  DeviceBuffer<OptState> opt_state_{MemTag::Network};
  DeviceBuffer<uint16_t> grads_{MemTag::Network};
  DeviceBuffer<float> grads_f32_{MemTag::Network};
  DeviceBuffer<uint16_t> ws_features_{MemTag::Network};
  DeviceBuffer<uint16_t> ws_acts_{MemTag::Network};
  DeviceBuffer<uint16_t> ws_dfeat_{MemTag::Network};
  DeviceBuffer<float> ws_loss_{MemTag::Network};
  size_t ws_batch_ = 0;
  hipStream_t side_stream_ = nullptr;
  hipEvent_t ev_fork_ = nullptr, ev_join_ = nullptr;
  uint32_t lds_halves_ = 0, lds_halves_T_ = 0;
  mutable DeviceBuffer<uint8_t> brick_image_{MemTag::Network};
  mutable DeviceBuffer<LevelInfo> levels_brick_dev_{MemTag::Network};
  mutable bool brick_valid_ = false, brick_refused_ = false;
  mutable uint32_t brick_stable_calls_ = 0;
  static constexpr uint32_t kBrickPaysAfter = 64;
  mutable uint32_t brick_served_calls_ = 0, brick_after_scale_ = 1;
  mutable uint64_t brick_builds_ = 0;
  static constexpr size_t kBrickSmallMinLaunch = (size_t)1 << 20;
  mutable int brick_tier_ = 0;
  mutable bool brick_small_refused_ = false;
  mutable uint64_t brick_small_builds_ = 0;
  mutable float brick_build_ms_ = 0.0f;
  uint32_t brick_res_cap_ = 0;
  size_t brick_budget_ = 0;
  mutable uint32_t brick_levels_mask_ = 0;
  int brick_mode_ = -1;

public:
  static constexpr int kTrainPhases = 5, kTrainProfileSteps = 64;
  void set_train_profiling(bool e);
  int train_profile(double* ms_per_step );
private:
  void profile_mark(int phase_boundary, hipStream_t s);
  bool train_profiling_ = false;
  std::vector<hipEvent_t> prof_events_;
  uint64_t prof_steps_ = 0;

public:
  ~Network();
  Network(const Network&) = delete;
  Network& operator=(const Network&) = delete;
};

uint32_t grid_make_layout(const ModelConfig& cfg, GridDevice* out);

}
```

instantvnr_amd/csrc/network_host.hip:

```cpp
#include "network.h"

#include <algorithm>
#include <cstdlib>
#include <set>

#include "infer_kernel.h"

namespace vnr {

void launch_pack_mlp(const uint16_t* params, uint16_t* packed, uint16_t* packedT, uint32_t in_width, uint32_t W, uint32_t n_hidden_matmuls, hipStream_t s);
void launch_fused(int mode, const GridDevice& grid, uint32_t in_width, const FusedMlp& mlp, const LevelInfo* d_levels, const uint16_t* table, size_t table_bytes,
                  const float* coords, float* out, uint16_t* features_out, uint16_t* acts_out, size_t n, const uint32_t* d_n, size_t n_max, hipStream_t s,
                  const uint32_t* d_dest = nullptr, uint32_t queue_out_stride = 0, const uint8_t* brick_image = nullptr,
                  uint32_t sharers = 1, const struct PackArgs* pack = nullptr);
void launch_init_params(OptState* state, uint16_t* params, size_t n_mlp, size_t n_total, uint32_t in_width,
                        uint32_t n_hidden_matmuls, uint32_t width, uint64_t seed, hipStream_t s);
void launch_master_from_f16(const uint16_t* params, OptState* state, size_t n, bool reset_optimizer, hipStream_t s);

uint16_t f32_to_f16(float f)
{
  uint32_t x;
  std::memcpy(&x, &f, 4);
  const uint32_t sign = (x >> 16) & 0x8000u;
  const uint32_t ax = x & 0x7fffffffu;
  if (ax >= 0x7f800000u) return (uint16_t)(sign | 0x7c00u | ((ax > 0x7f800000u) ? (0x200u | ((ax >> 13) & 0x3ffu)) : 0u));
  if (ax >= 0x477ff000u) return (uint16_t)(sign | 0x7c00u);
  if (ax < 0x33000001u) return (uint16_t)sign;
  const int32_t e = (int32_t)(ax >> 23) - 127;
  const uint32_t m = (ax & 0x7fffffu) | 0x800000u;
  const uint32_t shift = e < -14 ? (uint32_t)(-1 - e) : 13u;
  const uint32_t he = e < -14 ? 0u : (uint32_t)(e + 15);
  uint32_t q = m >> shift;
  const uint32_t rem = m & ((1u << shift) - 1u), half = 1u << (shift - 1);
  if (rem > half || (rem == half && (q & 1u))) q++;
  return (uint16_t)(sign | (he == 0 ? q : ((he - 1) << 10) + q));
}

float f16_to_f32(uint16_t h)
{
  const uint32_t sign = ((uint32_t)h & 0x8000u) << 16, e = (h >> 10) & 0x1fu, m = h & 0x3ffu;
  uint32_t x;
  if (e == 0) {
    if (m == 0) x = sign;
    else { float v = (float)m * 5.9604644775390625e-8f; std::memcpy(&x, &v, 4); x |= sign; }
  } else if (e == 31) x = sign | 0x7f800000u | (m << 13);
  else x = sign | ((e + 112u) << 23) | (m << 13);
  float f;
  std::memcpy(&f, &x, 4);
  return f;
}

uint32_t grid_make_layout(const ModelConfig& cfg, GridDevice* out)
{
  if (cfg.n_levels > (uint32_t)kMaxLevels) throw std::runtime_error("too many hash-grid levels");
  const float log2_pls = std::log2(cfg.per_level_scale);
  uint32_t offset = 0;
  for (uint32_t l = 0; l < cfg.n_levels; ++l) {
    const float scale = exp2f((float)l * log2_pls) * (float)cfg.base_resolution - 1.0f;
    const uint32_t res = (uint32_t)ceilf(scale) + 1u;
    const uint32_t max_params = 0xffffffffu / 2u;
    const double cube = (double)res * (double)res * (double)res;
    uint32_t n = cube > (double)max_params ? max_params : (uint32_t)cube;
    n = next_multiple(n, 8u);
    if (cfg.grid_type == 2u) {
      const double tile = (double)cfg.base_resolution * cfg.base_resolution * cfg.base_resolution;
      if ((double)n > tile) n = (uint32_t)tile;
    } else if (cfg.grid_type == 0u) {
      const uint32_t cap = 1u << cfg.log2_hashmap_size;
      if (n > cap) n = cap;
    }
    if (n == 0) throw std::runtime_error("grid level without entries");
    uint32_t stride = 1, dims = 0;
    for (; dims < 3 && stride <= n; ++dims) stride *= res;
    LevelInfo& lv = out->levels[l];
    lv.scale = scale;
    lv.resolution = res;
    lv.res2 = res * res;
    lv.size = n;
    lv.offset = offset;
    if (cfg.grid_type == 0u) lv.hashed = n < stride ? 1u : 0u;
    else lv.hashed = (dims == 3 && (uint64_t)res * res * res <= (uint64_t)n) ? 0u : 1u + dims;
    lv.brick = lv.pad1 = 0;
    if (lv.hashed == 1u && (n & (n - 1)) != 0) throw std::runtime_error("internal: hashed level with non power-of-two size");
    if ((uint64_t)offset + n > 0xffffffffull) throw std::runtime_error("grid encoding too large (more than 2^32 entries)");
    offset += n;
  }
  out->n_levels = cfg.n_levels;
  out->n_features = cfg.n_features;
  out->interpolation = cfg.interpolation;
  return offset;
}

static std::set<Network*>& live_networks()
{
  static std::set<Network*> s;
  return s;
}

static uint32_t json_u32(const Json& j, const char* key, uint32_t def) { return j.contains(key) ? (uint32_t)j.at(key).as_int() : def; }
static float json_f32(const Json& j, const char* key, float def) { return j.contains(key) ? j.at(key).as_float() : def; }
static std::string json_str(const Json& j, const char* key, const char* def) { return j.contains(key) ? j.at(key).as_string() : std::string(def); }

void Network::configure(const Json& config, uint64_t init_seed)
{
  const Json loss = config.value("loss", Json::object());
  const Json enc = config.value("encoding", Json::object());
  const Json net = config.value("network", Json::object());
  ModelConfig c = cfg_;
  if (config.contains("optimizer")) {
    const Json& opt = config.at("optimizer");
    const std::string ot = json_str(opt, "otype", "Adam");
    const Json* adam = &opt;
    if (ot == "ExponentialDecay") {
      c.has_decay = true;
      c.decay_start = json_u32(opt, "decay_start", 10000);
      c.decay_interval = json_u32(opt, "decay_interval", 10000);
      c.decay_base = json_f32(opt, "decay_base", 0.33f);
      if (!opt.contains("nested")) throw std::runtime_error("ExponentialDecay optimizer needs a 'nested' optimizer");
      adam = &opt.at("nested");
    } else {
      c.has_decay = false;
    }
    if (json_str(*adam, "otype", "Adam") != "Adam") throw std::runtime_error("unsupported optimizer otype (Adam / ExponentialDecay{Adam} only)");
    c.learning_rate = json_f32(*adam, "learning_rate", 1e-3f);
    c.beta1 = json_f32(*adam, "beta1", 0.9f);
    c.beta2 = json_f32(*adam, "beta2", 0.999f);
    c.epsilon = json_f32(*adam, "epsilon", 1e-8f);
    c.l2_reg = json_f32(*adam, "l2_reg", 1e-8f);
  }
  const std::string lt = json_str(loss, "otype", "L2");
  if (lt == "L1") c.loss = 0;
  else if (lt == "L2") c.loss = 1;
  else throw std::runtime_error("unsupported loss otype: " + lt);

  const std::string et = json_str(enc, "otype", "");
  if (et != "HashGrid" && et != "Grid" && et != "DenseGrid" && et != "TiledGrid")
    throw std::runtime_error("unsupported encoding otype: '" + et + "' (HashGrid / Grid / DenseGrid / TiledGrid)");
  const std::string gt = json_str(enc, "type", et == "DenseGrid" ? "Dense" : et == "TiledGrid" ? "Tiled" : "Hash");
  if (gt == "Hash") c.grid_type = 0;
  else if (gt == "Dense") c.grid_type = 1;
  else if (gt == "Tiled") c.grid_type = 2;
  else throw std::runtime_error("unsupported grid type: " + gt + " (Hash / Dense / Tiled)");
  c.n_levels = json_u32(enc, "n_levels", 16);
  c.n_features = json_u32(enc, "n_features_per_level", 2);
  c.log2_hashmap_size = json_u32(enc, "log2_hashmap_size", 19);
  c.base_resolution = json_u32(enc, "base_resolution", 16);
  c.per_level_scale = json_f32(enc, "per_level_scale", 2.0f);
  const std::string it = json_str(enc, "interpolation", "Linear");
  if (it == "Linear") c.interpolation = 0;
  else if (it == "Smoothstep") c.interpolation = 1;
  else if (it == "Nearest") c.interpolation = 2;
  else throw std::runtime_error("unsupported interpolation: " + it);
  c.quantize_threshold = json_f32(enc, "quantize_threshold", 0.0f);
  c.max_level = json_f32(enc, "max_level", 1000.0f);
  if (c.n_features != 1 && c.n_features != 2 && c.n_features != 4 && c.n_features != 8)
    throw std::runtime_error("n_features_per_level must be 1, 2, 4 or 8");
  if (c.log2_hashmap_size > 28) throw std::runtime_error("log2_hashmap_size too large");

  const std::string nt = json_str(net, "otype", "FullyFusedMLP");
  if (nt != "FullyFusedMLP") throw std::runtime_error("unsupported network otype: " + nt + " (FullyFusedMLP only)");
  c.n_neurons = json_u32(net, "n_neurons", 128);
  c.n_hidden_layers = json_u32(net, "n_hidden_layers", 5);
  if (c.n_neurons != 16 && c.n_neurons != 32 && c.n_neurons != 64 && c.n_neurons != 128)
    throw std::runtime_error("FullyFusedMLP n_neurons must be 16, 32, 64 or 128");
  if (c.n_hidden_layers < 1) throw std::runtime_error("n_hidden_layers must be >= 1");
  auto activation_of = [](const std::string& a, const char* what) -> uint32_t {
    if (a == "None") return kActNone;
// ... 289 lines not shown
  if (small) policy = std::min(policy, brick_small_budget());
  const uint64_t budget_lines = (uint64_t)std::min(policy, (double)(free_b + brick_image_.bytes()) / 4.0) / 128u;
  const uint32_t mask_before = brick_valid_ ? brick_levels_mask_ : 0u;
  brick_levels_mask_ = 0;
  hipEvent_t t0, t1;
  VNR_HIP_CHECK(hipEventCreate(&t0)); VNR_HIP_CHECK(hipEventCreate(&t1));
  const uint32_t F = cfg_.n_features;
  const uint32_t lx = F == 8 ? 1 : 2, ly = F >= 4 ? 1 : 2, lz = F == 1 ? 2 : 1;
  const uint64_t entries_per_line = 64u / F;
  std::vector<LevelInfo> lv(grid_.levels, grid_.levels + kMaxLevels);
  std::vector<uint64_t> lines(kMaxLevels, 0);
  uint64_t used = 0;
  const bool finest_first = F <= 2;
  for (int k = 0; k < (int)grid_.n_levels; ++k) {
    const int l = finest_first ? (int)grid_.n_levels - 1 - k : k;
    if (lv[l].hashed != 1u) continue;
    if (brick_res_cap_ && lv[l].resolution > brick_res_cap_ + 1u) continue;
    const uint64_t res = lv[l].resolution;
    uint64_t n = ((res >> lx) + 1) * ((res >> ly) + 1) * ((res >> lz) + 1);
    if (F == 2) {
      if (res >= 13000) continue;
      n = (res / 7 + 1) * ((res >> 1) + 1) * ((res >> 1) + 1);
      lv[l].pad1 = (uint32_t)(res / 7 + 1);
    }
    if (n * entries_per_line >= (1ull << 32) || used + n + 1 > budget_lines || used + n + 1 >= 0xffffffffull) continue;
    lv[l].brick = (uint32_t)used + 1u;
    lines[l] = n;
    used += n;
    brick_levels_mask_ |= 1u << l;
  }
  if (used == 0) {
    if (!small) brick_refused_ = true;
    else brick_small_refused_ = true;
    brick_valid_ = false;
    (void)hipEventDestroy(t0); (void)hipEventDestroy(t1);
    return;
  }
  if (!small && brick_valid_ && mask_before == brick_levels_mask_ && brick_image_.bytes() == (used + 1) * 128u) {
    brick_tier_ = 2;
    (void)hipEventDestroy(t0); (void)hipEventDestroy(t1);
    return;
  }
  if (brick_image_.bytes() != (used + 1) * 128u) {
    if (brick_image_.bytes()) VNR_HIP_CHECK(hipDeviceSynchronize());
    brick_valid_ = false;
  }
  brick_image_.resize((used + 1) * 128u);
  VNR_HIP_CHECK(hipEventRecord(t0, s));
  for (uint32_t l = 0; l < grid_.n_levels; ++l) {
    if (!lv[l].brick) continue;
    const uint64_t n_entries = lines[l] * entries_per_line;
    const uint16_t* table = params_f16_.ptr + n_mlp_;
    switch (F) {
    case 1: launch_brick_build<1>(lv[l], table, brick_image_.ptr, n_entries, s); break;
    case 2: launch_brick_build<2>(lv[l], table, brick_image_.ptr, n_entries, s); break;
    case 4: launch_brick_build<4>(lv[l], table, brick_image_.ptr, n_entries, s); break;
    default: launch_brick_build<8>(lv[l], table, brick_image_.ptr, n_entries, s); break;
    }
  }
  VNR_HIP_CHECK(hipMemsetAsync(brick_image_.ptr + used * 128u, 0, 128, s));
  levels_brick_dev_.resize(kMaxLevels);
  VNR_HIP_CHECK(hipMemcpyAsync(levels_brick_dev_.ptr, lv.data(), kMaxLevels * sizeof(LevelInfo), hipMemcpyHostToDevice, s));
  VNR_HIP_CHECK(hipEventRecord(t1, s));
  VNR_HIP_CHECK(hipEventSynchronize(t1));
  VNR_HIP_CHECK(hipEventElapsedTime(&brick_build_ms_, t0, t1));
  (void)hipEventDestroy(t0); (void)hipEventDestroy(t1);
  brick_valid_ = true;
  brick_tier_ = small ? 1 : 2;
}

const LevelInfo* Network::inference_levels(hipStream_t s, const uint8_t** image, size_t n_max) const
{
  static const int env_mode = [] { const char* e = std::getenv("VNR_AMD_BRICK"); return e ? std::atoi(e) : -1; }();
  const int mode = brick_mode_ >= 0 ? brick_mode_ : env_mode;
  *image = nullptr;
  if (mode == 0 || brick_refused_) return levels_dev_.ptr;
  if (brick_tier_ != 2 || !brick_valid_) {
    if (brick_stable_calls_ < 0xffffffffu) ++brick_stable_calls_;
    const bool want_full = mode == 1 || brick_stable_calls_ > brick_after_now();
    if (want_full) {
      build_brick_image(s, false);
      if (brick_valid_ && brick_tier_ == 2) { ++brick_builds_; brick_served_calls_ = 0; }
    } else if (!brick_valid_ && !brick_small_refused_ && n_max >= kBrickSmallMinLaunch && brick_small_budget() > 0.0 && cfg_.n_features <= 2u) {
      build_brick_image(s, true);
      if (brick_valid_) ++brick_small_builds_;
    }
    if (!brick_valid_) return levels_dev_.ptr;
  }
  if (brick_served_calls_ < 0xffffffffu) ++brick_served_calls_;
  *image = brick_image_.ptr;
  return levels_brick_dev_.ptr;
}

void Network::set_params_f16(const uint16_t* host, size_t count, hipStream_t s)
{
  if (count != n_params_) throw std::runtime_error("parameter count mismatch: got " + std::to_string(count) + ", model has " + std::to_string(n_params_));
  VNR_HIP_CHECK(hipMemcpyAsync(params_f16_.ptr, host, count * sizeof(uint16_t), hipMemcpyHostToDevice, s));
  if (opt_state_.count == n_params_) launch_master_from_f16(params_f16_.ptr, opt_state_.ptr, n_params_, false, s);
  ++params_generation_;
  refresh_inference_weights(s);
  VNR_HIP_CHECK(hipStreamSynchronize(s));
}

void Network::get_params_f16(uint16_t* host, size_t count, hipStream_t s) const
{
  if (count != n_params_) throw std::runtime_error("parameter count mismatch");
  VNR_HIP_CHECK(hipMemcpyAsync(host, params_f16_.ptr, count * sizeof(uint16_t), hipMemcpyDeviceToHost, s));
  VNR_HIP_CHECK(hipStreamSynchronize(s));
}

Json Network::serialize_params(hipStream_t s) const
{
  std::vector<uint16_t> host(n_params_);
  get_params_f16(host.data(), n_params_, s);
  Json j = Json::object();
  j["n_params"] = (uint64_t)n_params_;
  j["params_type"] = "__half";
  j["params_binary"] = Json::binary(host.data(), host.size() * sizeof(uint16_t));
  return j;
}

void Network::deserialize_params(const Json& j, hipStream_t s)
{
  const size_t n = (size_t)j.at("n_params").as_int();
  if (n != n_params_) throw std::runtime_error("Can't set params because buffer has the wrong size: " + std::to_string(n) + " vs " + std::to_string(n_params_));
  const std::string type = j.at("params_type").as_string();
  const std::string& bin = j.at("params_binary").as_binary();
  std::vector<uint16_t> host(n);
  if (type == "__half") {
    if (bin.size() != n * 2) throw std::runtime_error("params_binary has the wrong size");
    std::memcpy(host.data(), bin.data(), n * 2);
  } else if (type == "float") {
    if (bin.size() != n * 4) throw std::runtime_error("params_binary has the wrong size");
    const float* f = (const float*)bin.data();
    for (size_t i = 0; i < n; ++i) host[i] = f32_to_f16(f[i]);
  } else {
    throw std::runtime_error("Unknown params_type: " + type);
  }
  set_params_f16(host.data(), n, s);
  if (j.contains("optimizer") || j.contains("step")) {  }
}

void Network::inference(const float* d_coords, float* d_out, size_t n, const uint32_t* d_n, size_t n_max, hipStream_t s,
                        const uint32_t* d_dest) const
{
  const uint8_t* image;
  const LevelInfo* levels = inference_levels(s, &image, d_n ? n_max : n);
  GridDevice grid = grid_;
  grid.n_levels = n_active_levels();
  launch_fused(0, grid, in_width_, fused_mlp(), levels, params_f16_.ptr + n_mlp_, n_grid_params() * 2, d_coords, d_out, nullptr, nullptr, n, d_n, n_max, s, d_dest, 0, image);
}

bool Network::inference_queue(const float* d_records, float* d_out, uint32_t out_stride, const uint32_t* d_n, size_t n_max, hipStream_t s,
                              uint32_t sharers, const PackArgs* pack) const
{
  const uint8_t* image;
  const LevelInfo* levels = inference_levels(s, &image, n_max);
  GridDevice grid = grid_;
  grid.n_levels = n_active_levels();
  if (cfg_.n_neurons == 128u) pack = nullptr;
  launch_fused(0, grid, in_width_, fused_mlp(), levels, params_f16_.ptr + n_mlp_, n_grid_params() * 2, d_records, d_out, nullptr, nullptr, 0, d_n, n_max, s, nullptr,
               out_stride, image, sharers, pack);
  return pack != nullptr;
}

FusedMlp Network::fused_mlp() const
{
  const bool wglobal = !weights_in_lds();
  return FusedMlp{mlp_packed_.ptr, lds_halves_, cfg_.n_neurons, n_hidden_matmuls(), cfg_.activation, cfg_.output_activation, !common_kind() || wglobal, wglobal,
                  cfg_.quantize_threshold};
}

bool Network::tile_net(TileNet* out, hipStream_t s) const
{
  if (!weights_in_lds()) return false;
  if (n_grid_params() * 2 >= (1ull << 32)) throw std::runtime_error("hash table >= 4 GiB is not supported");
  const uint8_t* image;
  const LevelInfo* levels = inference_levels(s, &image, kBrickSmallMinLaunch);
  out->levels = levels;
  out->n_levels = n_active_levels();
  out->interpolation = grid_.interpolation;
  out->table = (const half_t*)(params_f16_.ptr + n_mlp_);
  out->table_bytes = (uint32_t)(n_grid_params() * 2);
  out->brick_image = image;
  out->packed_mlp = (const half_t*)mlp_packed_.ptr;
  out->lds_halves = lds_halves_;
  out->n_hidden_matmuls = n_hidden_matmuls();
  out->activation = cfg_.activation;
  out->output_activation = cfg_.output_activation;
  out->n_features = grid_.n_features;
  out->in_width = in_width_;
  out->width = cfg_.n_neurons;
  out->general = common_kind() ? 0u : 1u;
  out->quantize_threshold = cfg_.quantize_threshold;
  return true;
}

void Network::encode(const float* d_coords, uint16_t* d_features, size_t n, hipStream_t s) const
{
  const uint8_t* image;
  const LevelInfo* levels = inference_levels(s, &image, n);
  GridDevice grid = grid_;
  grid.n_levels = n_active_levels();
  launch_fused(1, grid, in_width_, fused_mlp(), levels, params_f16_.ptr + n_mlp_, n_grid_params() * 2, d_coords, nullptr, d_features, nullptr, n, nullptr, n, s, nullptr, 0, image);
}

size_t Network::bytes_allocated() const
{
  return brick_image_.bytes() + params_f16_.bytes() + mlp_packed_.bytes() + mlp_packed_T_.bytes() + opt_state_.bytes() + grads_.bytes() + grads_f32_.bytes() + ws_features_.bytes() + ws_acts_.bytes() + ws_dfeat_.bytes() + ws_loss_.bytes();
}

}
```

instantvnr_amd/csrc/network_infer.hip:

```cpp
#include "infer_kernel.h"

namespace vnr {

__global__ void pack_mlp_kernel(const half_t* __restrict__ params, half_t* __restrict__ packed, half_t* __restrict__ packedT, uint32_t in_width,
                                uint32_t W, uint32_t nh)
{
  const uint32_t RW = mlp_rows_padded(W), KS = W / 16u, step = 16u * RW, hidden = KS * step;
  const uint32_t total = packed_mlp_halves(in_width, W, nh), totalT = packedT ? packedT_halves(in_width, W, nh) : 0u;
  const uint32_t l1 = (in_width / 16u) * step;
  const uint32_t first_sz = W * in_width;
  for (uint32_t e = blockIdx.x * blockDim.x + threadIdx.x; e < total + totalT; e += gridDim.x * blockDim.x) {
    half_t v = (half_t)0.0f;
    if (e < total) {
      if (e < l1) {
        const uint32_t j = e & 7u, q = e >> 3, row = q % RW, hs = q / RW, h = hs & 1u, s = hs >> 1;
        if (row < W) v = params[row * in_width + 16u * s + 8u * h + j];
      } else if (e < l1 + nh * hidden) {
        const uint32_t r = e - l1, layer = r / hidden, qq = r % hidden;
        const uint32_t j = qq & 7u, q = qq >> 3, row = q % RW, hs = q / RW, h = hs & 1u, s = hs >> 1;
        const uint32_t k = 16u * s + 8u * (j >> 2) + 4u * h + (j & 3u);
        if (row < W) v = params[first_sz + layer * W * W + row * W + k];
      } else {
        const uint32_t q = e - l1 - nh * hidden;
        const uint32_t j = q & 7u, h = (q >> 3) & 1u, s = q >> 4;
        const uint32_t k = 16u * s + 8u * (j >> 2) + 4u * h + (j & 3u);
        v = params[first_sz + nh * W * W + k];
      }
      packed[e] = v;
    } else {
      const uint32_t t = e - total;
      const uint32_t rp = ((in_width + 31u) / 32u) * 32u;
      if (t < KS * 16u) {
        const uint32_t j = t & 7u, h = (t >> 3) & 1u, s = t >> 4;
        v = params[first_sz + nh * W * W + 16u * s + 8u * (j >> 2) + 4u * h + (j & 3u)];
      } else if (t < KS * 16u + nh * hidden) {
        const uint32_t r = t - KS * 16u, layer = r / hidden, qq = r % hidden;
        const uint32_t j = qq & 7u, q = qq >> 3, row = q % RW, hs = q / RW, h = hs & 1u, s = hs >> 1;
        const uint32_t kk = 16u * s + 8u * (j >> 2) + 4u * h + (j & 3u);
        if (row < W) v = params[first_sz + layer * W * W + kk * W + row];
      } else {
        const uint32_t qq = t - KS * 16u - nh * hidden;
        const uint32_t j = qq & 7u, q = qq >> 3, row = q % rp, hs = q / rp, h = hs & 1u, s = hs >> 1;
        const uint32_t kk = 16u * s + 8u * (j >> 2) + 4u * h + (j & 3u);
        if (row < in_width) v = params[kk * in_width + row];
      }
      packedT[t] = v;
    }
  }
}

void launch_pack_mlp(const uint16_t* params, uint16_t* packed, uint16_t* packedT, uint32_t in_width, uint32_t W, uint32_t n_hidden_matmuls, hipStream_t s)
{
  const uint32_t total = packed_mlp_halves(in_width, W, n_hidden_matmuls) + (packedT ? packedT_halves(in_width, W, n_hidden_matmuls) : 0u);
  pack_mlp_kernel<<<div_round_up(total, 256), 256, 0, s>>>((const half_t*)params, (half_t*)packed, (half_t*)packedT, in_width, W, n_hidden_matmuls);
}

#define VNR_DECL(name) void name(int mode, uint32_t F, uint32_t K_IN, const InferArgs& a, size_t n_max, hipStream_t s)
VNR_DECL(launch_fused_w16); VNR_DECL(launch_fused_w32); VNR_DECL(launch_fused_w64); VNR_DECL(launch_fused_w128);
VNR_DECL(launch_fused_w16g); VNR_DECL(launch_fused_w32g); VNR_DECL(launch_fused_w64g); VNR_DECL(launch_fused_w128g);
#undef VNR_DECL

void launch_fused(int mode, const GridDevice& grid, uint32_t in_width, const FusedMlp& mlp, const LevelInfo* d_levels, const uint16_t* table, size_t table_bytes,
                  const float* coords, float* out, uint16_t* features_out, uint16_t* acts_out, size_t n, const uint32_t* d_n, size_t n_max, hipStream_t s,
                  const uint32_t* d_dest, uint32_t queue_out_stride, const uint8_t* brick_image, uint32_t sharers, const PackArgs* pack)
{
  if (n_max == 0) { if (pack && pack->n_blocks) throw std::runtime_error("internal: ray packing fused into an empty evaluation launch"); return; }
  if (n_max > 0xffffffc0ull) throw std::runtime_error("inference batch too large (max 2^32-64 samples per call)");
  if (table_bytes >= (1ull << 32)) throw std::runtime_error("hash table >= 4 GiB is not supported");
  InferArgs a;
  a.levels = d_levels;
  a.n_levels = grid.n_levels;
  a.interpolation = grid.interpolation;
  a.table = (const half_t*)table;
  a.table_bytes = (uint32_t)table_bytes;
  a.brick_image = brick_image;
  a.sharers = sharers;
  a.packed_mlp = (const half_t*)mlp.packed;
  a.coords = coords;
  a.out = out;
  a.features_out = (half_t*)features_out;
  a.acts_out = (half_t*)acts_out;
  a.n_ptr = d_n;
  a.dest = d_dest;
  a.queue_mode = queue_out_stride ? 1u : 0u;
  a.out_stride = queue_out_stride;
  a.n = d_n ? (uint32_t)n_max : (uint32_t)n;
  a.n_hidden_matmuls = mlp.n_hidden_matmuls;
  a.activation = mlp.activation;
  a.output_activation = mlp.output_activation;
  a.lds_halves = mlp.lds_halves;
  a.weights_global = mlp.weights_global ? 1u : 0u;
  a.quantize_threshold = mlp.quantize_threshold;
  if (mlp.weights_global && !mlp.general) throw std::runtime_error("internal: weights from global memory are a GENERAL instance's");
  if (pack && mode == 0) {
    if (mlp.width == 128u) throw std::runtime_error("internal: the 128-neuron evaluation kernel (8 waves per block) does not take the ray packing prologue");
    a.pack = *pack;
  } else a.pack.n_blocks = 0;
  if (mode == 1) {
    if (mlp.general) return dispatch<64, 1, true>(grid.n_features, in_width, a, n_max, s);
    return dispatch<64, 1, false>(grid.n_features, in_width, a, n_max, s);
  }
  const uint32_t F = grid.n_features;
  switch (mlp.width) {
  case 16: return mlp.general ? launch_fused_w16g(mode, F, in_width, a, n_max, s) : launch_fused_w16(mode, F, in_width, a, n_max, s);
  case 32: return mlp.general ? launch_fused_w32g(mode, F, in_width, a, n_max, s) : launch_fused_w32(mode, F, in_width, a, n_max, s);
  case 64: return mlp.general ? launch_fused_w64g(mode, F, in_width, a, n_max, s) : launch_fused_w64(mode, F, in_width, a, n_max, s);
  case 128: return mlp.general ? launch_fused_w128g(mode, F, in_width, a, n_max, s) : launch_fused_w128(mode, F, in_width, a, n_max, s);
  default: throw std::runtime_error("internal: no MFMA kernel for n_neurons = " + std::to_string(mlp.width));
  }
}

}
```

instantvnr_amd/csrc/network_train.hip:

```cpp
#include "infer_kernel.h"

namespace vnr {

void launch_fused(int mode, const GridDevice& grid, uint32_t in_width, const FusedMlp& mlp, const LevelInfo* d_levels, const uint16_t* table, size_t table_bytes,
                  const float* coords, float* out, uint16_t* features_out, uint16_t* acts_out, size_t n, const uint32_t* d_n, size_t n_max, hipStream_t s,
                  const uint32_t* d_dest = nullptr, uint32_t queue_out_stride = 0, const uint8_t* brick_image = nullptr,
                  uint32_t sharers = 1, const struct PackArgs* pack = nullptr);

struct Pcg32 {
  uint64_t state, inc;
  __host__ __device__ Pcg32(uint64_t initstate, uint64_t initseq = 0xda3e39cb94b95bdbULL)
  {
    state = 0u;
    inc = (initseq << 1u) | 1u;
    next_uint();
    state += initstate;
    next_uint();
  }
  __host__ __device__ uint32_t next_uint()
  {
    const uint64_t old = state;
    state = old * 0x5851f42d4c957f2dULL + inc;
    const uint32_t xs = (uint32_t)(((old >> 18u) ^ old) >> 27u);
    const uint32_t rot = (uint32_t)(old >> 59u);
    return (xs >> rot) | (xs << ((~rot + 1u) & 31));
  }
  __host__ __device__ float next_float()
  {
    const uint32_t u = (next_uint() >> 9) | 0x3f800000u;
    return __builtin_bit_cast(float, u) - 1.0f;
  }
  __host__ __device__ void advance(uint64_t delta)
  {
    uint64_t cur_mult = 0x5851f42d4c957f2dULL, cur_plus = inc, acc_mult = 1u, acc_plus = 0u;
    while (delta > 0) {
      if (delta & 1) { acc_mult *= cur_mult; acc_plus = acc_plus * cur_mult + cur_plus; }
      cur_plus = (cur_mult + 1) * cur_plus;
      cur_mult *= cur_mult;
      delta >>= 1;
    }
    state = acc_mult * state + acc_plus;
  }
};

__global__ void init_params_kernel(OptState* __restrict__ state, half_t* __restrict__ params, size_t n_mlp, size_t n_total,
                                   uint32_t in_width, uint32_t n_hidden_matmuls, uint32_t width, uint64_t seed)
{
  const size_t t = (size_t)blockIdx.x * blockDim.x + threadIdx.x;
  const size_t e0 = t * 4;
  if (e0 >= n_total) return;
  Pcg32 rng(seed);
  rng.advance(e0);
  const size_t first = (size_t)width * in_width, hidden_end = first + (size_t)n_hidden_matmuls * width * width;
  for (size_t e = e0; e < e0 + 4 && e < n_total; ++e) {
    const float u = rng.next_float();
    float scale;
    if (e < first) scale = sqrtf(6.0f / (float)(in_width + width));
    else if (e < hidden_end) scale = sqrtf(6.0f / (float)(width + width));
    else if (e < n_mlp) scale = sqrtf(6.0f / (float)(width + 16));
    else scale = 1e-4f;
    const float v = u * (2.0f * scale) - scale;
    state[e] = OptState{v, 0.0f, 0.0f, 0u};
    params[e] = (half_t)v;
  }
}

void launch_init_params(OptState* state, uint16_t* params, size_t n_mlp, size_t n_total, uint32_t in_width,
                        uint32_t n_hidden_matmuls, uint32_t width, uint64_t seed, hipStream_t s)
{
  const size_t threads = (n_total + 3) / 4;
  init_params_kernel<<<div_round_up(threads, 256), 256, 0, s>>>(state, (half_t*)params, n_mlp, n_total, in_width,
                                                                n_hidden_matmuls, width, seed);
  VNR_HIP_CHECK(hipGetLastError());
}

__global__ void master_from_f16_kernel(const half_t* __restrict__ in, OptState* __restrict__ state, size_t n, bool reset_optimizer)
{
  for (size_t i = (size_t)blockIdx.x * blockDim.x + threadIdx.x; i < n; i += (size_t)gridDim.x * blockDim.x) {
    if (reset_optimizer) state[i] = OptState{(float)in[i], 0.0f, 0.0f, 0u};
    else state[i].master = (float)in[i];
  }
}
void launch_master_from_f16(const uint16_t* params, OptState* state, size_t n, bool reset_optimizer, hipStream_t s)
{
  master_from_f16_kernel<<<min(div_round_up(n, 256), 4096u), 256, 0, s>>>((const half_t*)params, state, n, reset_optimizer);
  VNR_HIP_CHECK(hipGetLastError());
}

__global__ void loss_grad_kernel(const float* __restrict__ y, const float* __restrict__ target, uint32_t n, uint32_t loss_type, uint32_t out_act,
                                 half_t* __restrict__ dy, float* __restrict__ loss_partials)
{
  __shared__ float red[256];
  float acc = 0.0f;
  const float inv_n = 1.0f / (float)n;
  for (uint32_t i = blockIdx.x * blockDim.x + threadIdx.x; i < n; i += gridDim.x * blockDim.x) {
    const float d = y[i] - target[i];
    float g;
    if (loss_type == 0) { acc += fabsf(d) * inv_n; g = copysignf(1.0f, d); }
    else { acc += d * d * inv_n; g = 2.0f * d; }
    dy[i] = act_backward_f16((half_t)((float)kLossScale * g * inv_n), (half_t)y[i], out_act);
  }
  red[threadIdx.x] = acc;
  __syncthreads();
  for (uint32_t s = 128; s > 0; s >>= 1) {
    if (threadIdx.x < s) red[threadIdx.x] += red[threadIdx.x + s];
    __syncthreads();
  }
  if (threadIdx.x == 0) loss_partials[blockIdx.x] = red[0];
}

struct BackwardArgs {
  const half_t* packedT;
  const half_t* dy;
  const half_t* acts;
  half_t* d_out;
  half_t* dfeat;
  uint32_t n, nh, activation, in_width, lds_halves;
  uint32_t weights_global;
};

__device__ __forceinline__ half8_t load_frag_rowmajor(const half_t* row, int s, uint32_t h)
{
  const half4_t lo = *(const half4_t*)(row + 16 * s + 4 * h);
  const half4_t hi = *(const half4_t*)(row + 16 * s + 8 + 4 * h);
  return half8_t{lo[0], lo[1], lo[2], lo[3], hi[0], hi[1], hi[2], hi[3]};
}
__device__ __forceinline__ void store_frag_rowmajor(half_t* row, int s, uint32_t h, const half8_t& v)
{
  *(half4_t*)(row + 16 * s + 4 * h) = half4_t{v[0], v[1], v[2], v[3]};
  *(half4_t*)(row + 16 * s + 8 + 4 * h) = half4_t{v[4], v[5], v[6], v[7]};
}
__device__ __forceinline__ half8_t pack_plain(const f32x16& acc, int sh)
{
  float8_t v;
#pragma unroll
  for (int j = 0; j < 8; ++j) v[j] = acc[8 * sh + j];
  return __builtin_convertvector(v, half8_t);
}
__device__ __noinline__ half8_t act_backward_general8(half8_t d, half8_t a, uint32_t act)
{
#pragma unroll
  for (int j = 0; j < 8; ++j) d[j] = act_backward_f16(d[j], a[j], act);
  return d;
}
template <bool GENERAL>
__device__ __forceinline__ half8_t act_backward8(const half8_t& d, const half8_t& a, uint32_t act)
{
  if (act == kActNone) return d;
  if (GENERAL && act > kActReLU) return act_backward_general8(d, a, act);
  half8_t r;
#pragma unroll
  for (int j = 0; j < 8; ++j) r[j] = a[j] > (half_t)0.0f ? d[j] : (half_t)0.0f;
  return r;
}

template <int W, int MTF, bool GENERAL>
__global__ void __launch_bounds__(256) mlp_backward_kernel(const BackwardArgs args)
{
  typedef MlpShape<W> Sh;
  constexpr int MT = Sh::MT, RW = Sh::RW, KS = Sh::KS;
// ... 1264 lines not shown
```

instantvnr_amd/csrc/pack_rays.h:

```cpp
#pragma once
#include "common.h"

namespace vnr {

struct RayList {
  uint32_t* pixel_index;
  float* jitter;
  float* alpha;
  vec3f* color;
  vec3i* cell;
  vec3f* t_next;
  float* next_cell_begin;
  uint32_t* sample_base;
  uint32_t* sample_count;
};

struct SshLists {
  vec3f* org[2];
  vec3f* color[2];
  float* alpha[2];
};

enum { C_RAYS0 = 0, C_RAYS1 = 1, C_SAMPLES0 = 2, C_SAMPLES1 = 3, C_HIT = 4, C_STAT_SAMPLES = 6, C_STAT_REFRAYS = 8, C_COUNT = 16 };

struct PackArgs {
  RayList src, dst;
  const uint32_t* ray_counts;
  uint32_t n_first;
  uint32_t* counters;
  int parity, first, ssh, grad;
  SshLists ssh_lists;
  uint32_t* host_alive;
  uint32_t* host_stats;
  uint32_t n_blocks;
};

#if defined(__HIPCC__)
template <int WAVES>
__device__ __forceinline__ void pack_rays_block(const PackArgs& a, uint32_t item, uint32_t* s_part)
{
  constexpr uint32_t T = 64u * WAVES;
  const uint32_t tid = threadIdx.x, lane = tid & 63u, wave = tid >> 6;
  uint32_t* counters = a.counters;
  const int parity = a.parity;
  const uint32_t n_in = a.first ? a.n_first : counters[C_RAYS0 + parity];
  const uint32_t n_groups = ((n_in + 255u) & ~255u) >> 6;
  if (item == 0 && tid == 0) counters[C_SAMPLES0 + (parity ^ 1)] = 0;
  if (n_groups == 0) {
    if (item == 0 && tid == 0) { counters[C_RAYS0 + (parity ^ 1)] = 0; *a.host_alive = 0; }
    if (item == 0 && tid >= C_HIT && tid < C_COUNT) a.host_stats[tid] = counters[tid];
    return;
  }
  const uint32_t g0 = item * (uint32_t)WAVES;
  if (g0 >= n_groups) return;
  const uint32_t* __restrict__ ray_counts = a.ray_counts;
  uint32_t sum = 0;
  for (uint32_t g = tid; g < g0; g += T) sum += ray_counts[g] & 0xffu;
#pragma unroll
  for (int d = 32; d > 0; d >>= 1) sum += __shfl_xor(sum, d);
  if (lane == 0) s_part[wave] = sum;
  __syncthreads();
  uint32_t before = 0;
#pragma unroll
  for (int w = 0; w < WAVES; ++w) before += s_part[w];
  const uint32_t mine = (lane < (uint32_t)WAVES && g0 + lane < n_groups) ? ray_counts[g0 + lane] & 0xffu : 0u;
  uint32_t incl = mine;
#pragma unroll
  for (int d = 1; d < WAVES; d <<= 1) {
    const uint32_t y = __shfl_up(incl, d);
    if ((int)lane >= d) incl += y;
  }
  const uint32_t count = __shfl(mine, (int)wave), base = before + __shfl(incl, (int)wave) - count;
  const uint32_t block_total = __shfl(incl, WAVES - 1);
  const bool last_block = g0 + (uint32_t)WAVES >= n_groups;
  if (last_block && tid == 0) { counters[C_RAYS0 + (parity ^ 1)] = before + block_total; *a.host_alive = before + block_total; }
  if (lane < count) {
    const RayList& src = a.src;
    const RayList& dst = a.dst;
    const uint32_t from = ((g0 + wave) << 6) + lane, to = base + lane;
    dst.pixel_index[to] = src.pixel_index[from];
    dst.jitter[to] = src.jitter[from];
    dst.alpha[to] = src.alpha[from];
    dst.color[to] = src.color[from];
    dst.cell[to] = src.cell[from];
    dst.t_next[to] = src.t_next[from];
    dst.next_cell_begin[to] = src.next_cell_begin[from];
    dst.sample_base[to] = src.sample_base[from];
    dst.sample_count[to] = src.sample_count[from];
    if (a.ssh) {
      const SshLists& sl = a.ssh_lists;
      sl.org[0][to] = sl.org[1][from]; sl.color[0][to] = sl.color[1][from]; sl.alpha[0][to] = sl.alpha[1][from];
    }
  }
  if (last_block) {
    uint32_t asum = 0;
    for (uint32_t g = tid; g < n_groups; g += T) asum += ray_counts[g] >> 8;
#pragma unroll
    for (int d = 32; d > 0; d >>= 1) asum += __shfl_xor(asum, d);
    __syncthreads();
    if (lane == 0) s_part[wave] = asum;
    __syncthreads();
    if (tid == 0) {
      uint32_t alive_total = 0;
      for (int w = 0; w < WAVES; ++w) alive_total += s_part[w];
      const uint32_t records = counters[C_SAMPLES0 + parity];
      unsigned long long* c64 = (unsigned long long*)counters;
      c64[C_STAT_SAMPLES / 2] += (unsigned long long)(a.grad ? records >> 2 : records);
      c64[C_STAT_REFRAYS / 2] += (unsigned long long)alive_total;
      if (a.first) counters[C_HIT] += alive_total;
    }
    __syncthreads();
    if (tid >= C_HIT && tid < C_COUNT) a.host_stats[tid] = ((volatile uint32_t*)counters)[tid];
  }
}
#endif

}
```

instantvnr_amd/csrc/render.hip:

```cpp
#include "renderer.h"

#include <algorithm>
#include <cfloat>
#include <cstdlib>

#include "dist.h"
#include "infer_tile.h"
#include "pack_rays.h"
#include "sampling_device.h"
#include "march_device.h"
#include "pt_device.h"

namespace vnr {

template <bool FIRST, int MODE>
__global__ void __launch_bounds__(256) march_kernel(const RenderParams p, const RayList cur, const RayList nxt,
                                                    const vec2f* __restrict__ vd_in, vec4f* __restrict__ queue,
                                                    vec2f* __restrict__ vd_out, uint32_t* __restrict__ counters,
                                                    uint32_t* __restrict__ ray_counts, int parity, const SshLists ssh_lists,
                                                    uint32_t* __restrict__ tail_flag)
{
  extern __shared__ float s_t[];
  float* s_t0 = s_t;
  float* s_t1 = s_t + (size_t)p.n_iters * 256;
// ... 479 lines not shown
      if (exited) r.L = r.L + r.throughput;
      r.tnear = 0.0f; r.tfar = VNR_FLOAT_LARGE;
      const float s0 = r.next_float(), s1 = r.next_float();
      r.dir = xfm_vector(p.wto, pt_uniform_sample_sphere(s0, s1));
      r.shadow = false;
    } else {
      if (exited) {
        if (r.scatter_index > 0u) r.L = r.L + 1.5f * r.throughput;
        break;
      }
      if (r.scatter_index > 4u) {
        const float q = fminf(0.95f, max3f(r.throughput.x, r.throughput.y, r.throughput.z));
        if (r.next_float() > q) break;
        r.throughput = {r.throughput.x / q, r.throughput.y / q, r.throughput.z / q};
      }
      ++r.scatter_index;
      r.org = r.org + t * r.dir;
      r.throughput = r.throughput * (0.6f * albedo);
      r.tnear = 0.0f; r.tfar = VNR_FLOAT_LARGE;
      r.dir = p.shadow_dir;
      r.shadow = true;
    }
  }
  write_pixel(p, {r.L.x, r.L.y, r.L.z, 1.0f}, pixel);
}

__global__ void __launch_bounds__(1024) pt_compact_kernel(const PtRays src, const PtRays dst, const uint32_t* __restrict__ ray_counts,
                                                          uint32_t n_first, uint32_t* __restrict__ counters, int parity, int first,
                                                          vec4f* __restrict__ queue)
{
  __shared__ uint32_t s_part[16];
  const uint32_t tid = threadIdx.x, lane = tid & 63u, wave = tid >> 6;
  const uint32_t n_in = first ? n_first : counters[C_RAYS0 + parity];
  const uint32_t n_groups = ((n_in + 255u) & ~255u) >> 6;
  if (n_groups == 0) {
    if (blockIdx.x == 0 && tid == 0) counters[C_RAYS0 + (parity ^ 1)] = 0;
    return;
  }
  const uint32_t g0 = blockIdx.x * 16u;
  if (g0 >= n_groups) return;
  uint32_t sum = 0;
  for (uint32_t g = tid; g < g0; g += 1024u) sum += ray_counts[g];
#pragma unroll
  for (int d = 32; d > 0; d >>= 1) sum += __shfl_xor(sum, d);
  if (lane == 0) s_part[wave] = sum;
  __syncthreads();
  uint32_t before = 0;
#pragma unroll
  for (int w = 0; w < 16; ++w) before += s_part[w];
  const uint32_t mine = (lane < 16u && g0 + lane < n_groups) ? ray_counts[g0 + lane] : 0u;
  uint32_t incl = mine;
#pragma unroll
  for (int d = 1; d < 16; d <<= 1) {
    const uint32_t y = __shfl_up(incl, d);
    if ((int)lane >= d) incl += y;
  }
  const uint32_t count = __shfl(mine, (int)wave), base = before + __shfl(incl, (int)wave) - count;
  const uint32_t block_total = __shfl(incl, 15);
  if (g0 + 16u >= n_groups && tid == 0) {
    const uint32_t total = before + block_total;
    counters[C_RAYS0 + (parity ^ 1)] = total;
    atomicAdd((unsigned long long*)(counters + C_STAT_SAMPLES), (unsigned long long)total);
  }
  if (lane < count) {
    const uint32_t from = ((g0 + wave) << 6) + lane, to = base + lane;
#pragma unroll
    for (int k = 0; k < kPtPlanes; ++k) dst.base[(size_t)k * dst.stride + to] = src.base[(size_t)k * src.stride + from];
    queue[to] = {src.base[(size_t)8 * src.stride + from], src.base[(size_t)9 * src.stride + from], src.base[(size_t)10 * src.stride + from],
                 __uint_as_float(to)};
  }
}

}
#include "in_shader.h"
#include "decoupled.h"
namespace vnr {

struct PartState {
  RenderParams p;
  RayList rl[2];
  SshLists ssh;
  vec4f* queue;
  vec2f* vd[2];
  uint32_t* c;
  uint32_t* rc;
  uint32_t* hc;
  uint32_t* hs;
  hipStream_t s;
  size_t s_max;
  uint32_t it = 0, used = 0;
  bool done = false;
  bool tail_skipped = false;
  hipEvent_t ev_done = nullptr;
};

struct DPart {
  RenderParams p;
  DRays rays;
  DRing ring[8];
  DHost* host = nullptr;
  hipStream_t sw = nullptr, se = nullptr, sc = nullptr;
  std::vector<hipEvent_t> ev_w, ev_e, ev_c;
  uint32_t it_w = 0, it_c = 0, target = 0;
  size_t s_max = 0;
  bool done = false;
  hipEvent_t& ev(std::vector<hipEvent_t>& v, uint32_t it)
  {
    if (it >= 1024u) throw std::runtime_error("internal: decoupled loop asked for the event of iteration " + std::to_string(it));
    while (v.size() <= it) { hipEvent_t e; VNR_HIP_CHECK(hipEventCreateWithFlags(&e, hipEventDisableTiming)); v.push_back(e); }
    return v[it];
  }
  ~DPart() { for (auto* v : {&ev_w, &ev_e, &ev_c}) for (hipEvent_t e : *v) (void)hipEventDestroy(e); }
};

struct Renderer::StreamingFrame {
  bool pending = false;
  bool decoupled = false;
  int ahead = 2, ring = 3;
  DPart dpart[Renderer::kMaxParts];
  int slot = 0;
  int H = 0, pass_mode = 0;
  bool grad = false, ssh = false;
  NeuralVolume* nv = nullptr;
  size_t shmem = 0, shmem_compose = 0;
  uint32_t max_iterations = 240;
  uint32_t* predicted = nullptr;
  RenderParams p_all;
  uint64_t params_generation = 0;
  PartState part[Renderer::kMaxParts];
  StreamingFrame()
  {
    for (auto& p : part) {
      (void)hipEventCreateWithFlags(&p.ev_done, hipEventDisableTiming);
    }
  }
  ~StreamingFrame() { for (auto& p : part) if (p.ev_done) (void)hipEventDestroy(p.ev_done); }
  void mark(int h) { VNR_HIP_CHECK(hipEventRecord(part[h].ev_done, part[h].s)); }
};

Renderer::Renderer(std::shared_ptr<VolumeBase> volume) : volume_(std::move(volume))
{
  if (!Runtime::get().ready()) Runtime::get().init(-1);
  stream_ = Runtime::get().stream;
  if (const char* e = std::getenv("VNR_RM_N_ITERS")) { n_iters_ = std::max(1, std::min(48, std::atoi(e))); n_iters_fixed_ = true; }
  if (const char* e = std::getenv("VNR_AMD_RENDER_HALVES")) { n_halves_ = std::max(1, std::min(kMaxParts, std::atoi(e))); n_halves_fixed_ = true; }
  if (const char* e = std::getenv("VNR_AMD_SMALL_SHARE_PARTS")) small_share_parts_ = std::max(1, std::min(kMaxParts, std::atoi(e)));
  if (const char* e = std::getenv("VNR_AMD_TILE_W")) {
    const int w = std::atoi(e);
    tile_w_log2_ = w == 16 ? 4u : w == 32 ? 5u : w == 64 ? 6u : 3u;
  }
  if (const char* e = std::getenv("VNR_AMD_DECOUPLED")) decoupled_mode_ = std::max(0, std::min(2, std::atoi(e)));
  if (const char* e = std::getenv("VNR_AMD_DECOUPLED_AHEAD")) decoupled_ahead_ = std::max(1, std::min(7, std::atoi(e)));
  if (const char* e = std::getenv("VNR_AMD_DECOUPLED_PARTS")) decoupled_parts_ = std::max(1, std::min(kMaxParts, std::atoi(e)));
  counters_.resize(2 * kMaxParts * C_COUNT);
  counters_.zero(stream_);
  VNR_HIP_CHECK(hipHostMalloc((void**)&host_counts_, 2 * kMaxParts * (256 + C_COUNT) * sizeof(uint32_t), hipHostMallocDefault));
  VNR_HIP_CHECK(hipEventCreateWithFlags(&ev_fork_, hipEventDisableTiming));
}

Renderer::~Renderer()
{
  if (stream_) (void)hipStreamSynchronize(stream_);
  for (int i = 1; i < kMaxParts; ++i) if (part_streams_[i]) (void)hipStreamSynchronize(part_streams_[i]);
  if (ev_fork_) (void)hipEventDestroy(ev_fork_);
  for (auto& ps : d_streams_) for (hipStream_t st : ps) if (st) { (void)hipStreamSynchronize(st); (void)hipStreamDestroy(st); }
  frame_[0].reset(); frame_[1].reset();
  if (d_host_) (void)hipHostFree(d_host_);
  if (distributed_) (void)hipStreamSynchronize(Dist::get().comm_stream());
  if (ev_rendered_) (void)hipEventDestroy(ev_rendered_);
  for (int i = 0; i < 2; ++i) if (ev_gathered_[i]) (void)hipEventDestroy(ev_gathered_[i]);
  for (int i = 0; i < 2; ++i) if (host_fb_[i]) (void)hipHostFree(host_fb_[i]);
  if (host_counts_) (void)hipHostFree(host_counts_);
  for (auto& sl : events_) for (auto& v : sl) for (auto e : v) (void)hipEventDestroy(e);
}

void Renderer::resize(int w, int h)
{
  finish_pending();
  if (w <= 0 || h <= 0) throw std::runtime_error("invalid framebuffer size");
  VNR_HIP_CHECK(hipDeviceSynchronize());
  width_ = w; height_ = h;
  const size_t n = (size_t)w * h;
  for (int i = 0; i < 2; ++i) { fb_[i].resize(n); fb_[i].zero(stream_); }
  accumulation_.resize(n);
  accumulation_.zero(stream_);
  if (host_fb_pixels_ != n) {
    for (int i = 0; i < 2; ++i) {
      if (host_fb_[i]) (void)hipHostFree(host_fb_[i]);
      VNR_HIP_CHECK(hipHostMalloc((void**)&host_fb_[i], n * sizeof(vec4f), hipHostMallocDefault));
      std::memset(host_fb_[i], 0, n * sizeof(vec4f));
    }
    host_fb_pixels_ = n;
  }
  if (distributed_) ensure_share_buffers();
  reset_ = true;
}

__global__ void assemble_shares_kernel(const vec4f* __restrict__ gathered, vec4f* __restrict__ full, uint32_t width, uint32_t height,
                                       uint32_t world, uint32_t n_local)
{
  const uint32_t n = width * height;
  for (uint32_t i = blockIdx.x * blockDim.x + threadIdx.x; i < n; i += gridDim.x * blockDim.x) {
    const uint32_t y = i / width, x = i - y * width, b = y >> 3;
    full[i] = gathered[(size_t)(b % world) * n_local + ((b / world) * 8u + (y & 7u)) * width + x];
  }
}

void Renderer::set_distributed(bool e)
{
  finish_pending();
  if (e && !Dist::get().active()) throw std::runtime_error("distributed rendering needs vnrAmdDistInitFromEnv / vnrAmdDistInit first");
  distributed_ = e && Dist::get().world() >= 1;
  pipe_prev_ = -1;
  if (distributed_) {
    if (!ev_rendered_) VNR_HIP_CHECK(hipEventCreateWithFlags(&ev_rendered_, hipEventDisableTiming));
    for (int i = 0; i < 2; ++i) if (!ev_gathered_[i]) VNR_HIP_CHECK(hipEventCreateWithFlags(&ev_gathered_[i], hipEventDisableTiming));
    ensure_share_buffers();
  }
  reset_ = true;
}

void Renderer::ensure_share_buffers()
{
  if (width_ <= 0 || height_ <= 0) return;
  const Dist& d = Dist::get();
  const ShareLayout l = share_layout((uint32_t)width_, (uint32_t)height_, (uint32_t)d.world());
  share_world_ = (uint32_t)d.world(); share_rank_ = (uint32_t)d.rank(); share_n_local_ = l.n_local;
  VNR_HIP_CHECK(hipStreamSynchronize(stream_));
  VNR_HIP_CHECK(hipStreamSynchronize(Dist::get().comm_stream()));
  const size_t n = (size_t)width_ * height_;
  for (int i = 0; i < 2; ++i) {
    gathered_[i].resize((size_t)share_world_ * l.n_local);
    gathered_[i].zero(stream_);
    full_[i].resize(n);
    full_[i].zero(stream_);
    gather_issued_[i] = false;
  }
  if (accumulation_.count < l.n_local) { accumulation_.resize(l.n_local); accumulation_.zero(stream_); }
  VNR_HIP_CHECK(hipStreamSynchronize(stream_));
}

void Renderer::issue_gather(int buf)
{
  if (gather_issued_[buf]) return;
  Dist& d = Dist::get();
  hipStream_t comm = d.comm_stream();
  const int fslot = frame_of_buffer_[buf];
  if (fslot >= 0 && frame_[fslot]) {
    for (int h = 0; h < frame_[fslot]->H; ++h) VNR_HIP_CHECK(hipStreamWaitEvent(comm, frame_[fslot]->part[h].ev_done, 0));
  } else {
    VNR_HIP_CHECK(hipEventRecord(ev_rendered_, stream_));
    VNR_HIP_CHECK(hipStreamWaitEvent(comm, ev_rendered_, 0));
  }
  vec4f* g = gathered_[buf].ptr;
  const size_t share_bytes = (size_t)share_n_local_ * sizeof(vec4f);
  d.transport().all_gather(g + (size_t)share_rank_ * share_n_local_, g, share_bytes, comm);
  const uint32_t n = (uint32_t)((size_t)width_ * height_);
  assemble_shares_kernel<<<std::min<uint32_t>(div_round_up(n, 256), (uint32_t)Runtime::get().n_cus * 8u), 256, 0, comm>>>(
      g, full_[buf].ptr, (uint32_t)width_, (uint32_t)height_, share_world_, share_n_local_);
  VNR_HIP_CHECK(hipGetLastError());
  if (!skip_download_) VNR_HIP_CHECK(hipMemcpyAsync(host_fb_[buf], full_[buf].ptr, (size_t)n * sizeof(vec4f), hipMemcpyDeviceToHost, comm));
  VNR_HIP_CHECK(hipEventRecord(ev_gathered_[buf], comm));
  gather_issued_[buf] = true;
}

const float* Renderer::render_pipelined()
{
  const int cur = fb_cur_;
  const bool was_async = async_, was_skip = skip_download_;
  async_ = true;
  if (!distributed_) skip_download_ = true;
  try { render(); } catch (...) { async_ = was_async; skip_download_ = was_skip; throw; }
  async_ = was_async; skip_download_ = was_skip;
  const float* out = nullptr;
  const int prev = pipe_prev_;
  if (prev >= 0) {
    StreamingFrame* older = frame_[slot_ ^ 1].get();
    if (older && older->pending) finish_streaming(*older);
    out = hand_out_frame(prev);
  }
  pipe_prev_ = cur;
  fb_cur_ ^= 1;
  return out;
}

const float* Renderer::flush_pipeline()
{
  if (pipe_prev_ < 0) return nullptr;
  finish_pending();
  const int prev = pipe_prev_;
  pipe_prev_ = -1;
  return hand_out_frame(prev);
}

const float* Renderer::hand_out_frame(int buf)
{
  if (distributed_) {
    issue_gather(buf);
    VNR_HIP_CHECK(hipEventSynchronize(ev_gathered_[buf]));
    return skip_download_ ? (const float*)full_[buf].ptr : (const float*)host_fb_[buf];
  }
  if (skip_download_) return (const float*)fb_[buf].ptr;
  const size_t n = (size_t)width_ * height_;
  VNR_HIP_CHECK(hipMemcpy(host_fb_[buf], fb_[buf].ptr, n * sizeof(vec4f), hipMemcpyDeviceToHost));
  return (const float*)host_fb_[buf];
}

// ... 209 lines not shown
  NeuralVolume* nv = static_cast<NeuralVolume*>(volume_.get());
  TileNet net;
  if (!nv->network().tile_net(&net, stream_)) throw std::runtime_error("internal: in-shader rendering of a model without an MFMA kernel");
  if (is_samples_.count == 0) { is_samples_.resize(kInShaderStatSlots); is_hits_.resize(kInShaderStatSlots); }
  is_samples_.zero(stream_);
  is_hits_.zero(stream_);
  InShaderLaunch l;
  l.blocks = div_round_up(p.n_local, 256);
  l.shmem = (size_t)net.lds_halves * sizeof(uint16_t);
  l.stream = stream_;
  l.stat_samples = is_samples_.ptr;
  l.stat_hits = is_hits_.ptr;
  bool launched = false;
  switch (net.width) {
  case 16: launched = net.general ? launch_in_shader_w16g(p, net, shade, l) : launch_in_shader_w16(p, net, shade, l); break;
  case 32: launched = net.general ? launch_in_shader_w32g(p, net, shade, l) : launch_in_shader_w32(p, net, shade, l); break;
  case 64: launched = net.general ? launch_in_shader_w64g(p, net, shade, l) : launch_in_shader_w64(p, net, shade, l); break;
  case 128: launched = !net.general && launch_in_shader_w128(p, net, shade, l); break;
  default: break;
  }
  if (!launched) throw std::runtime_error("internal: no in-shader instance for this model shape");
  VNR_HIP_CHECK(hipGetLastError());
  unsigned long long hs[kInShaderStatSlots];
  uint32_t hh[kInShaderStatSlots];
  VNR_HIP_CHECK(hipMemcpyAsync(hs, is_samples_.ptr, sizeof(hs), hipMemcpyDeviceToHost, stream_));
  VNR_HIP_CHECK(hipMemcpyAsync(hh, is_hits_.ptr, sizeof(hh), hipMemcpyDeviceToHost, stream_));
  VNR_HIP_CHECK(hipStreamSynchronize(stream_));
  for (int k = 0; k < kInShaderStatSlots; ++k) { stats_.n_samples += hs[k]; stats_.n_rays_hit += hh[k]; }
  stats_.n_reference_slots = stats_.n_samples;
  stats_.n_iterations = 1;
}

void Renderer::render_monolithic(const RenderParams& p)
{
  monolithic_kernel<<<div_round_up(p.n_local, 128), 128, 0, stream_>>>(p);
  VNR_HIP_CHECK(hipGetLastError());
}

void Renderer::render_pathtracing(const RenderParams& p)
{
  const uint32_t P = p.n_local;
  NeuralVolume* nv = volume_->is_network() ? static_cast<NeuralVolume*>(volume_.get()) : nullptr;
  if (nv && !nv->network().valid()) throw std::runtime_error("neural volume has no valid network");
  if (!nv && !p.volume) throw std::runtime_error("this volume has no resident data to sample");
  pt_rays_.ensure((size_t)2 * kPtPlanes * P);
  pt_values_.ensure(P);
  if (queue_.count < P) queue_.resize(P);
  ray_counts_.ensure(P / 64 + 64);
  const PtRays dense = {pt_rays_.ptr, P}, scratch = {pt_rays_.ptr + (size_t)kPtPlanes * P, P};
  uint32_t* c = counters_.ptr;
  hipStream_t s = stream_;
  VNR_HIP_CHECK(hipMemsetAsync(c, 0, C_COUNT * sizeof(uint32_t), s));
  const uint32_t blocks = std::min<uint32_t>(div_round_up(P, 256), 4096u);
  const uint32_t cblocks = div_round_up(P, 1024);
  uint32_t it = 0;
  auto launch = [&]() {
    const int parity = (int)(it & 1u);
    if (it == 0) {
      pt_kernel<true><<<blocks, 256, 0, s>>>(p, dense, scratch, pt_values_.ptr, c, ray_counts_.ptr, 0);
    } else {
      if (nv) nv->network().inference_queue((const float*)queue_.ptr, pt_values_.ptr, 1, c + C_RAYS0 + parity, P, s, 1);
      else gt_sample_kernel<<<std::min<uint32_t>(div_round_up(P, 256), (uint32_t)Runtime::get().n_cus * 8u), 256, 0, s>>>(
               c + C_RAYS0 + parity, p.volume, p.vol_dims, queue_.ptr, pt_values_.ptr);
      pt_kernel<false><<<blocks, 256, 0, s>>>(p, dense, scratch, pt_values_.ptr, c, ray_counts_.ptr, parity);
    }
    pt_compact_kernel<<<cblocks, 1024, 0, s>>>(scratch, dense, ray_counts_.ptr, P, c, parity, it == 0 ? 1 : 0, queue_.ptr);
    VNR_HIP_CHECK(hipGetLastError());
    VNR_HIP_CHECK(hipMemcpyAsync(host_counts_ + (it & 255u), c + C_RAYS0 + (parity ^ 1), sizeof(uint32_t), hipMemcpyDeviceToHost, s));
    ++it;
  };
  const uint32_t max_iterations = 1u << 16;
  while (it < std::max<uint32_t>(predicted_pt_, 1u)) launch();
  for (;;) {
    VNR_HIP_CHECK(hipStreamSynchronize(s));
    if (host_counts_[(it - 1) & 255u] == 0 || it >= max_iterations) break;
    for (int k = 0; k < 8; ++k) launch();
  }
  uint32_t used = it;
  if (it <= 256) { while (used > 1 && host_counts_[(used - 2) & 255u] == 0) --used; }
  predicted_pt_ = used;
  uint32_t hc[C_COUNT];
  VNR_HIP_CHECK(hipMemcpy(hc, c, sizeof(hc), hipMemcpyDeviceToHost));
  stats_.n_rays_hit += hc[C_HIT];
  const uint64_t n = (uint64_t)hc[C_STAT_SAMPLES] | ((uint64_t)hc[C_STAT_SAMPLES + 1] << 32);
  stats_.n_samples += n;
  stats_.n_reference_slots += n;
  stats_.n_iterations += used > 0 ? used - 1 : 0;
}

void Renderer::launch_iteration(StreamingFrame& f, int h)
{
  PartState* half = f.part;
  const int pass_mode = f.pass_mode;
  const size_t shmem = f.shmem, shmem_compose = f.shmem_compose;
  const uint32_t max_iterations = f.max_iterations;
  {
    PartState& hf = half[h];
    const uint32_t it = hf.it;
    const int parity = (int)(it & 1u);
    const uint32_t P = hf.p.n_local;
    uint32_t* c = hf.c;
    const hipStream_t s_it = hf.s;
    const bool skip_tail = it >= 1 && it + 1 == f.predicted[h] && it + 1 < max_iterations;
    uint32_t* tail_flag = nullptr;
    if (skip_tail) { hf.hs[0] = 0; tail_flag = hf.hs; }
    {
      const bool first = it == 0;
      const uint32_t blocks = std::min<uint32_t>(div_round_up(P, 256), first ? 4096u : 2048u);
      const size_t lds = first ? shmem : shmem_compose;
      const vec2f* vd_in = hf.vd[parity ^ 1];
      vec2f* vd_out = hf.vd[parity];
#define VNR_MARCH(FIRST_, MODE_) march_kernel<FIRST_, MODE_><<<blocks, 256, lds, s_it>>>(hf.p, hf.rl[0], hf.rl[1], vd_in, hf.queue, vd_out, c, hf.rc, parity, hf.ssh, tail_flag)
      switch (pass_mode) {
      case M_GRADIENT: if (first) VNR_MARCH(true, M_GRADIENT); else VNR_MARCH(false, M_GRADIENT); break;
      case M_SSH: if (first) VNR_MARCH(true, M_SSH); else VNR_MARCH(false, M_SSH); break;
      case M_SHADOW: if (first) VNR_MARCH(true, M_SHADOW); else VNR_MARCH(false, M_SHADOW); break;
      default: if (first) VNR_MARCH(true, M_NONE); else VNR_MARCH(false, M_NONE); break;
      }
#undef VNR_MARCH
    }
    VNR_HIP_CHECK(hipGetLastError());
    if (skip_tail) {
      if (profiling_) { VNR_HIP_CHECK(hipEventRecord(events_[f.slot][h][2 * it], hf.s)); VNR_HIP_CHECK(hipEventRecord(events_[f.slot][h][2 * it + 1], hf.s)); }
      hf.tail_skipped = true;
      ++hf.it;
      if (hf.it >= max_iterations) hf.done = true;
      return;
    }
  }
  {
    PartState& hf = half[h];
    const uint32_t it = hf.it;
    launch_tail(f, h, it, hf.s);
    ++hf.it;
    if (hf.it >= max_iterations) hf.done = true;
  }
}

void Renderer::launch_tail(StreamingFrame& f, int h, uint32_t it, hipStream_t s_it)
{
  PartState* half = f.part;
  const int H = f.H;
  const bool grad = f.grad, ssh = f.ssh;
  NeuralVolume* nv = f.nv;
  {
    PartState& hf = half[h];
    const int parity = (int)(it & 1u);
    const uint32_t P = hf.p.n_local;
    uint32_t* c = hf.c;
    PackArgs pk;
    pk.src = hf.rl[1]; pk.dst = hf.rl[0]; pk.ray_counts = hf.rc; pk.n_first = P; pk.counters = c; pk.parity = parity; pk.first = it == 0 ? 1 : 0;
    pk.ssh = ssh ? 1 : 0; pk.grad = grad ? 1 : 0; pk.ssh_lists = hf.ssh; pk.host_alive = hf.hc + (it & 255u); pk.host_stats = hf.hs;
    pk.n_blocks = div_round_up(P, 256);
    const bool fused_pack = P <= 262144u;
    bool packed = false;
    if (!s_it) s_it = hf.s;
    if (profiling_) VNR_HIP_CHECK(hipEventRecord(events_[f.slot][h][2 * it], s_it));
#if defined(VNR_DIAG)
    static const bool skip_eval = [] { const char* e = std::getenv("VNR_AMD_DEBUG_SKIP_EVAL"); return e && std::atoi(e) != 0; }();
#else
    constexpr bool skip_eval = false;
#endif
    if (skip_eval) {
    } else if (nv) {
      packed = nv->network().inference_queue((const float*)hf.queue, (float*)hf.vd[parity], 1, c + C_SAMPLES0 + parity, hf.s_max, s_it, (uint32_t)H,
                                             fused_pack ? &pk : nullptr);
    } else {
      const uint32_t blocks = std::min<uint32_t>(div_round_up(hf.s_max, 256), (uint32_t)Runtime::get().n_cus * 8u);
      gt_sample_kernel<<<blocks, 256, 0, s_it>>>(c + C_SAMPLES0 + parity, hf.p.volume, hf.p.vol_dims, hf.queue, (float*)hf.vd[parity]);
    }
    if (profiling_) VNR_HIP_CHECK(hipEventRecord(events_[f.slot][h][2 * it + 1], s_it));
    last_schedule_[2] = packed ? 1 : 0;
    if (!packed) {
      constexpr uint32_t kCompactSmallLimit = 262144u;
      if (P <= kCompactSmallLimit) {
        compact_rays_kernel<4><<<pk.n_blocks, 256, 0, s_it>>>(pk);
      } else {
        pk.n_blocks = div_round_up(P, 1024);
        compact_rays_kernel<16><<<pk.n_blocks, 1024, 0, s_it>>>(pk);
      }
    }
    VNR_HIP_CHECK(hipGetLastError());
  }
}

void Renderer::render_streaming(const RenderParams& p_all, int pass_mode, bool defer)
{
  if (decoupled_applies(p_all, pass_mode)) { render_decoupled(p_all, defer); return; }
  const uint32_t row_items = p_all.tiles_per_row * 64u;
  const uint32_t R = p_all.n_local / row_items;
  const int want = (!n_halves_fixed_ && p_all.n_local <= 524288u) ? small_share_parts_ : n_halves_;
  const int H = (int)std::min<uint32_t>((uint32_t)want, std::max(R, 1u));
  const uint32_t P_total = p_all.n_local;
  const bool grad = pass_mode == M_GRADIENT;
  const bool ssh = pass_mode == M_SSH;
  uint32_t* predicted = predicted_iterations_[pass_mode == M_SHADOW ? 1 : 0];
  ensure_queues(P_total, p_all.n_iters, grad || ssh || pass_mode == M_SHADOW);
  const size_t QP = queue_pixels_;
  if (ssh) q_ssh_.ensure(14 * QP);
  const size_t QI = (size_t)queue_iters_;
  const size_t slot_floats = queue_grad_ ? 6 : 2;
  const size_t rec_per_slot = queue_grad_ ? 4 : 1;
  if ((size_t)P_total * QI * 6 >= (1ull << 32)) throw std::runtime_error("frame share too large for 32-bit result indices");
  NeuralVolume* nv = volume_->is_network() ? static_cast<NeuralVolume*>(volume_.get()) : nullptr;
  if (nv && !nv->network().valid()) throw std::runtime_error("neural volume has no valid network");

  StreamingFrame* older = frame_[slot_] && frame_[slot_]->pending ? frame_[slot_].get() : nullptr;
  const int slot = older ? slot_ ^ 1 : slot_;
  if (!frame_[slot]) frame_[slot].reset(new StreamingFrame());
  StreamingFrame& f = *frame_[slot];
  if (f.pending) throw std::runtime_error("internal: both frame slots are pending");
  f.slot = slot;
  slot_ = slot;
  f.decoupled = false;
  PartState* half = f.part;
  for (int h = 0; h < kMaxParts; ++h) { half[h].it = 0; half[h].used = 0; half[h].done = false; half[h].tail_skipped = false; }
  const size_t n_groups_slot = QP / 64 + 64 + 8 * kMaxParts;
  uint32_t* const u32_base = q_u32_.ptr + (size_t)slot * 6 * QP;
  float* const f32_base = q_f32_.ptr + (size_t)slot * 18 * QP;
  int* const i32_base = q_i32_.ptr + (size_t)slot * 6 * QP;
  uint32_t* const rc_base = ray_counts_.ptr + (size_t)slot * n_groups_slot;
  vec4f* const queue_base = queue_.ptr + (size_t)slot * rec_per_slot * QP * QI;
  float* const arena_base = arena_.ptr + (size_t)slot * 2 * slot_floats * QP * QI;
  uint32_t* const counters_base = counters_.ptr + (size_t)slot * kMaxParts * C_COUNT;
  uint32_t* const host_base = host_counts_ + (size_t)slot * kMaxParts * (256 + C_COUNT);
  size_t off = 0;
  for (int h = 0; h < H; ++h) {
    PartState& hf = half[h];
    hf.p = p_all;
    if (H > 1) {
      hf.p.il_parts = p_all.il_parts * (uint32_t)H;
      hf.p.il_part = p_all.il_part + p_all.il_parts * (uint32_t)h;
      hf.p.n_local = ((R + (uint32_t)(H - 1 - h)) / (uint32_t)H) * row_items;
    }
    for (int b = 0; b < 2; ++b) {
      hf.rl[b].pixel_index = u32_base + (size_t)(0 + b) * QP + off;
      hf.rl[b].sample_base = u32_base + (size_t)(2 + b) * QP + off;
      hf.rl[b].sample_count = u32_base + (size_t)(4 + b) * QP + off;
      float* f = f32_base + (size_t)b * 9 * QP;
      hf.rl[b].jitter = f + off;
      hf.rl[b].alpha = f + QP + off;
      hf.rl[b].color = (vec3f*)(f + 2 * QP) + off;
      hf.rl[b].t_next = (vec3f*)(f + 5 * QP) + off;
      hf.rl[b].next_cell_begin = f + 8 * QP + off;
      hf.rl[b].cell = (vec3i*)(i32_base + (size_t)b * 3 * QP) + off;
      hf.ssh.org[b] = nullptr; hf.ssh.color[b] = nullptr; hf.ssh.alpha[b] = nullptr;
      if (ssh) {
        float* g = q_ssh_.ptr + (size_t)b * 7 * QP;
        hf.ssh.org[b] = (vec3f*)g + off;
        hf.ssh.color[b] = (vec3f*)(g + 3 * QP) + off;
        hf.ssh.alpha[b] = g + 6 * QP + off;
      }
      hf.vd[b] = (vec2f*)(arena_base + (size_t)b * slot_floats * QP * QI + slot_floats * off * QI);
    }
    hf.p.slot_cap = (uint32_t)((size_t)hf.p.n_local * QI);
    hf.queue = queue_base + rec_per_slot * off * QI;
    hf.c = counters_base + (size_t)h * C_COUNT;
    hf.rc = rc_base + off / 64 + (size_t)h * 8;
    hf.hc = host_base + (size_t)h * 256;
    hf.hs = host_base + kMaxParts * 256 + (size_t)h * C_COUNT;
    if (h > 0 && !part_streams_[h]) part_streams_[h] = Runtime::get().part_stream(h);
    hf.s = h == 0 ? stream_ : part_streams_[h];
    hf.s_max = (size_t)hf.p.n_local * hf.p.n_iters * (grad ? 4 : 1);
    off += hf.p.n_local;
  }

  f.params_generation = nv ? nv->network().params_generation() : 0;
  VNR_HIP_CHECK(hipMemsetAsync(counters_base, 0, (size_t)H * C_COUNT * sizeof(uint32_t), stream_));
  if (H > 1) {
    VNR_HIP_CHECK(hipEventRecord(ev_fork_, stream_));
    for (int h = 1; h < H; ++h) VNR_HIP_CHECK(hipStreamWaitEvent(part_streams_[h], ev_fork_, 0));
  }
  const size_t shmem = ((size_t)2 * p_all.n_iters + 1) * 256 * sizeof(float) + 16 * sizeof(uint32_t);
  const size_t shmem_compose = shmem + (p_all.tfn_in_lds ? (size_t)p_all.tfn.n_colors * sizeof(vec4f) + (size_t)p_all.tfn.n_alphas * sizeof(float) : 0);
  if (shmem_compose > 160 * 1024) throw std::runtime_error("VNR_RM_N_ITERS too large for the LDS of one workgroup");
  static bool lds_attr_set = false;
  if (!lds_attr_set) {
#define VNR_ATTR(FIRST_, MODE_) VNR_HIP_CHECK(hipFuncSetAttribute((const void*)march_kernel<FIRST_, MODE_>, hipFuncAttributeMaxDynamicSharedMemorySize, 160 * 1024))
    VNR_ATTR(true, M_NONE); VNR_ATTR(false, M_NONE); VNR_ATTR(true, M_GRADIENT); VNR_ATTR(false, M_GRADIENT);
    VNR_ATTR(true, M_SSH); VNR_ATTR(false, M_SSH); VNR_ATTR(true, M_SHADOW); VNR_ATTR(false, M_SHADOW);
#undef VNR_ATTR
    lds_attr_set = true;
  }
  uint32_t max_iterations = 240;
#if defined(VNR_DIAG)
  if (const char* e = std::getenv("VNR_AMD_DEBUG_MAX_ITERS")) max_iterations = std::max(1, std::min(240, std::atoi(e)));
#endif
  if (profiling_) {
    iter_ms_.assign(max_iterations, 0.0f);
    for (int h = 0; h < H; ++h)
      while (events_[slot][h].size() < 2 * max_iterations) { hipEvent_t e; VNR_HIP_CHECK(hipEventCreate(&e)); events_[slot][h].push_back(e); }
  }

  last_schedule_[0] = p_all.n_iters; last_schedule_[1] = H; last_schedule_[2] = 0; last_schedule_[3] = 0;
  f.H = H; f.pass_mode = pass_mode; f.grad = grad; f.ssh = ssh; f.nv = nv; f.shmem = shmem; f.shmem_compose = shmem_compose;
  f.max_iterations = max_iterations; f.predicted = predicted; f.p_all = p_all;
  if (older) {
    for (int h = 0; h < H; ++h) launch_iteration(f, h);
    finish_streaming(*older);
    stats_ = FrameStats();
  }
  frame_of_buffer_[fb_cur_] = slot;
  for (;;) {
    bool launched = false;
    for (int h = 0; h < H; ++h)
      if (!half[h].done && half[h].it < predicted[h]) { launch_iteration(f, h); launched = true; }
    if (!launched) break;
  }
  for (int h = 0; h < H; ++h) f.mark(h);
  f.pending = true;
  if (!defer) finish_streaming(f);
}

void Renderer::finish_streaming(StreamingFrame& f)
{
  if (!f.pending) return;
  if (f.decoupled) { finish_decoupled(f); return; }
  f.pending = false;
  PartState* half = f.part;
  const int H = f.H, pass_mode = f.pass_mode;
  uint32_t* predicted = f.predicted;
  const RenderParams& p_all = f.p_all;
  for (;;) {
    bool pending = false;
    for (int h = 0; h < H; ++h) {
      PartState& hf = half[h];
      if (hf.done) continue;
      if (hf.it > 0) {
        VNR_HIP_CHECK(hipEventSynchronize(hf.ev_done));
        if (hf.tail_skipped) {
          hf.tail_skipped = false;
          if (hf.hs[0] == 0) { hf.hc[(hf.it - 1) & 255u] = 0; hf.done = true; continue; }
          launch_tail(f, h, hf.it - 1, hf.s);
          f.mark(h);
          pending = true;
          continue;
        }
        if (hf.hc[(hf.it - 1) & 255u] == 0) { hf.done = true; continue; }
      }
      launch_iteration(f, h);
      f.mark(h);
      pending = true;
    }
    if (!pending) break;
  }

  uint32_t pass_iterations = 0;
  uint64_t n_samples = 0, n_refrays = 0;
  for (int h = 0; h < H; ++h) {
    PartState& hf = half[h];
    VNR_HIP_CHECK(hipEventSynchronize(hf.ev_done));
    uint32_t used = hf.it;
    while (used > 1 && hf.hc[(used - 2) & 255u] == 0) --used;
    predicted[h] = used;
    hf.used = used;
    const uint32_t* hc = hf.hs;
    if (pass_mode != M_SHADOW) stats_.n_rays_hit += hc[C_HIT];
    n_samples += (uint64_t)hc[C_STAT_SAMPLES] | ((uint64_t)hc[C_STAT_SAMPLES + 1] << 32);
    n_refrays += (uint64_t)hc[C_STAT_REFRAYS] | ((uint64_t)hc[C_STAT_REFRAYS + 1] << 32);
    pass_iterations = std::max<uint32_t>(pass_iterations, used > 0 ? used - 1 : 0);
    if (profiling_) stats_.infer_kernel_launches += used > 0 ? used - 1 : 0;
  }
  {
    uint32_t launched[kMaxParts] = {};
    for (int h = 0; h < H; ++h) launched[h] = half[h].it;
    collect_eval_profile(f, launched, nullptr);
  }
  stats_.n_iterations += pass_iterations;
  stats_.n_samples += n_samples;
  stats_.n_reference_slots += n_refrays * (uint64_t)p_all.n_iters;
  completed_stats_ = stats_;
}


void Renderer::collect_eval_profile(StreamingFrame& f, const uint32_t* launched, const uint32_t* )
{
  if (!profiling_) return;
  const int H = f.H;
  bool any = false;
  for (int h = 0; h < H; ++h) {
    for (uint32_t k = 0; k < launched[h]; ++k) {
      float ms = 0.0f;
      VNR_HIP_CHECK(hipEventElapsedTime(&ms, events_[f.slot][h][2 * k], events_[f.slot][h][2 * k + 1]));
      stats_.infer_kernel_ms += ms;
      if (k < iter_ms_.size()) iter_ms_[k] += ms;
      any = true;
    }
  }
  if (!any || launched[0] == 0) return;
  std::vector<std::pair<float, float>> iv;
  for (int h = 0; h < H; ++h)
    for (uint32_t k = 0; k < launched[h]; ++k) {
      float t0 = 0.0f, t1 = 0.0f;
      VNR_HIP_CHECK(hipEventElapsedTime(&t0, events_[f.slot][0][0], events_[f.slot][h][2 * k]));
      VNR_HIP_CHECK(hipEventElapsedTime(&t1, events_[f.slot][0][0], events_[f.slot][h][2 * k + 1]));
      iv.emplace_back(t0, t1);
    }
  std::sort(iv.begin(), iv.end());
  float lo = iv[0].first, hi = iv[0].second;
  double total = 0.0;
  for (size_t e = 1; e < iv.size(); ++e) {
    if (iv[e].first > hi) { total += hi - lo; lo = iv[e].first; hi = iv[e].second; }
    else hi = std::max(hi, iv[e].second);
  }
  stats_.infer_union_ms += total + (hi - lo);
}

bool Renderer::decoupled_applies(const RenderParams& p, int pass_mode) const
{
  if (pass_mode != M_NONE || decoupled_mode_ == 0) return false;
  if ((size_t)p.n_local * (size_t)p.n_iters >= (1ull << 28)) return false;
  return decoupled_mode_ == 2 || p.n_local <= 20480u;
}

void Renderer::render_decoupled(const RenderParams& p_all, bool defer)
{
  const uint32_t row_items = p_all.tiles_per_row * 64u;
  const uint32_t R = p_all.n_local / row_items;
  const int H = (int)std::min<uint32_t>((uint32_t)decoupled_parts_, std::max(R, 1u));
  const uint32_t P_total = p_all.n_local;
  const int A = decoupled_ahead_, RING = A + 1;
  last_schedule_[0] = p_all.n_iters; last_schedule_[1] = H; last_schedule_[2] = 0; last_schedule_[3] = 1;
  NeuralVolume* nv = volume_->is_network() ? static_cast<NeuralVolume*>(volume_.get()) : nullptr;
  if (nv && !nv->network().valid()) throw std::runtime_error("neural volume has no valid network");
  if (!nv && !p_all.volume) throw std::runtime_error("this volume has no resident data to sample");

  const size_t Pt = (size_t)P_total + 256u * kMaxParts;
  if (d_rays_ < Pt || d_iters_ < p_all.n_iters || d_ring_ < RING) {
    finish_pending();
    VNR_HIP_CHECK(hipDeviceSynchronize());
    d_rays_ = std::max(d_rays_, Pt); d_iters_ = std::max(d_iters_, p_all.n_iters); d_ring_ = std::max(d_ring_, RING);
    const size_t words = 15 * d_rays_ + (size_t)d_ring_ * d_rays_ + (size_t)d_ring_ * kMaxParts * D_COUNT;
    for (int sl = 0; sl < 2; ++sl) {
      d_words_[sl].resize(words);
      d_words_[sl].zero(stream_);
      d_queue_[sl].resize((size_t)d_ring_ * d_rays_ * d_iters_);
      d_arena_[sl].resize((size_t)d_ring_ * d_rays_ * d_iters_);
    }
    VNR_HIP_CHECK(hipStreamSynchronize(stream_));
  }
  if (!d_host_) {
    VNR_HIP_CHECK(hipHostMalloc(&d_host_, 2 * kMaxParts * sizeof(DHost), hipHostMallocDefault));
    std::memset(d_host_, 0, 2 * kMaxParts * sizeof(DHost));
  }
  int prio_least = 0, prio_greatest = 0;
  VNR_HIP_CHECK(hipDeviceGetStreamPriorityRange(&prio_least, &prio_greatest));
  for (int h = 0; h < H; ++h)
    for (int k = 0; k < 3; ++k)
      if (!d_streams_[h][k]) VNR_HIP_CHECK(hipStreamCreateWithPriority(&d_streams_[h][k], hipStreamNonBlocking, k == 1 ? prio_least : prio_greatest));

  StreamingFrame* older = frame_[slot_] && frame_[slot_]->pending ? frame_[slot_].get() : nullptr;
  const int slot = older ? slot_ ^ 1 : slot_;
  if (!frame_[slot]) frame_[slot].reset(new StreamingFrame());
  StreamingFrame& f = *frame_[slot];
  if (f.pending) throw std::runtime_error("internal: both frame slots are pending");
  f.slot = slot;
  slot_ = slot;
  f.decoupled = true; f.ahead = A; f.ring = RING;
  f.H = H; f.pass_mode = M_NONE; f.grad = false; f.ssh = false; f.nv = nv; f.p_all = p_all;
  f.shmem = ((size_t)2 * p_all.n_iters + 1) * 256 * sizeof(float) + 16 * sizeof(uint32_t) + (size_t)p_all.n_iters * 256 * sizeof(uint16_t);
  f.shmem_compose = p_all.tfn_in_lds ? (size_t)p_all.tfn.n_colors * sizeof(vec4f) + (size_t)p_all.tfn.n_alphas * sizeof(float) : 0;
  if (f.shmem > 160 * 1024) throw std::runtime_error("VNR_RM_N_ITERS too large for the LDS of one workgroup");
  f.max_iterations = 240;
#if defined(VNR_DIAG)
  if (const char* e = std::getenv("VNR_AMD_DEBUG_MAX_ITERS")) f.max_iterations = std::max(1, std::min(240, std::atoi(e)));
#endif
  static bool lds_attr_set = false;
  if (!lds_attr_set) {
    VNR_HIP_CHECK(hipFuncSetAttribute((const void*)walk_kernel<true>, hipFuncAttributeMaxDynamicSharedMemorySize, 160 * 1024));
    VNR_HIP_CHECK(hipFuncSetAttribute((const void*)walk_kernel<false>, hipFuncAttributeMaxDynamicSharedMemorySize, 160 * 1024));
    lds_attr_set = true;
  }
  if (profiling_) {
    iter_ms_.assign(f.max_iterations, 0.0f);
    for (int h = 0; h < H; ++h)
      while (events_[slot][h].size() < 2 * f.max_iterations) { hipEvent_t e; VNR_HIP_CHECK(hipEventCreate(&e)); events_[slot][h].push_back(e); }
  }

  uint32_t* w = d_words_[slot].ptr;
  uint32_t* const rec_base = w + 15 * d_rays_;
  uint32_t* const ctr_base = rec_base + (size_t)d_ring_ * d_rays_;
  size_t off = 0;
  for (int h = 0; h < H; ++h) {
    DPart& d = f.dpart[h];
    d.p = p_all;
    if (H > 1) {
      d.p.il_parts = p_all.il_parts * (uint32_t)H;
      d.p.il_part = p_all.il_part + p_all.il_parts * (uint32_t)h;
      d.p.n_local = ((R + (uint32_t)(H - 1 - h)) / (uint32_t)H) * row_items;
    }
    d.p.slot_cap = (uint32_t)((size_t)d.p.n_local * d.p.n_iters);
    const size_t Pr = ((size_t)d.p.n_local + 255u) & ~(size_t)255u;
    uint32_t* b = w + off;
    const size_t N = d_rays_;
    d.rays.pixel = b; d.rays.jitter = (float*)(b + N); d.rays.ncb = (float*)(b + 2 * N); d.rays.walking = b + 3 * N;
    d.rays.alpha = (float*)(b + 4 * N); d.rays.done = b + 5 * N;
    d.rays.cell = (vec3i*)(w + 6 * N) + off; d.rays.t_next = (vec3f*)(w + 9 * N) + off; d.rays.color = (vec3f*)(w + 12 * N) + off;
    for (int q = 0; q < RING; ++q) {
      d.ring[q].queue = d_queue_[slot].ptr + ((size_t)q * d_rays_ + off) * d_iters_;
      d.ring[q].arena = d_arena_[slot].ptr + ((size_t)q * d_rays_ + off) * d_iters_;
      d.ring[q].rec = rec_base + (size_t)q * d_rays_ + off;
      d.ring[q].ctr = ctr_base + ((size_t)q * kMaxParts + h) * D_COUNT;
    }
    d.host = (DHost*)d_host_ + (size_t)slot * kMaxParts + h;
    d.sw = d_streams_[h][0]; d.se = d_streams_[h][1]; d.sc = d_streams_[h][2];
    d.it_w = d.it_c = 0;
    d.target = std::max<uint32_t>(decoupled_predicted_[h], 1u);
    d.s_max = (size_t)d.p.n_local * d.p.n_iters;
    d.done = false;
    f.part[h].s = d.sc;
    off += Pr;
  }
  VNR_HIP_CHECK(hipEventRecord(ev_fork_, stream_));
  for (int h = 0; h < H; ++h)
    for (int k = 0; k < 3; ++k) VNR_HIP_CHECK(hipStreamWaitEvent(d_streams_[h][k], ev_fork_, 0));

  if (older) {
    for (bool any = true; any;) {
      any = false;
      for (int h = 0; h < H; ++h) { const uint32_t before = f.dpart[h].it_w; decoupled_step(f, h, true); any = any || f.dpart[h].it_w != before; }
    }
    finish_streaming(*older);
    stats_ = FrameStats();
  }
  frame_of_buffer_[fb_cur_] = slot;
  for (bool any = true; any;) {
    any = false;
    for (int h = 0; h < H; ++h) {
      DPart& d = f.dpart[h];
      const uint32_t bw = d.it_w, bc = d.it_c;
      decoupled_step(f, h, false);
      any = any || d.it_w != bw || d.it_c != bc;
    }
  }
  for (int h = 0; h < H; ++h) f.mark(h);
  f.pending = true;
  if (!defer) finish_streaming(f);
}

void Renderer::decoupled_step(StreamingFrame& f, int h, bool head_only)
{
  DPart& d = f.dpart[h];
  const uint32_t A = (uint32_t)f.ahead, RING = (uint32_t)f.ring;
  if (d.it_w < d.target && d.it_w < d.it_c + A) {
    const uint32_t it = d.it_w;
    const DRing& ring = d.ring[it % RING];
    if (it >= A) VNR_HIP_CHECK(hipStreamWaitEvent(d.sw, d.ev(d.ev_c, it - A), 0));
    const uint32_t P = d.p.n_local;
    const uint32_t blocks = std::min<uint32_t>(div_round_up(P, 256), 2048u);
    if (it == 0) walk_kernel<true><<<blocks, 256, f.shmem, d.sw>>>(d.p, d.rays, ring, d.host, it);
    else walk_kernel<false><<<blocks, 256, f.shmem, d.sw>>>(d.p, d.rays, ring, d.host, it);
    VNR_HIP_CHECK(hipGetLastError());
    VNR_HIP_CHECK(hipEventRecord(d.ev(d.ev_w, it), d.sw));
    VNR_HIP_CHECK(hipStreamWaitEvent(d.se, d.ev(d.ev_w, it), 0));
    if (profiling_) VNR_HIP_CHECK(hipEventRecord(events_[f.slot][h][2 * it], d.se));
#if defined(VNR_DIAG)
    static const bool skip_eval = [] { const char* e = std::getenv("VNR_AMD_DEBUG_SKIP_EVAL"); return e && std::atoi(e) != 0; }();
#else
    constexpr bool skip_eval = false;
#endif
    if (skip_eval) {
    } else if (f.nv) {
      f.nv->network().inference_queue((const float*)ring.queue, (float*)ring.arena, 1, ring.ctr + D_SAMPLES, d.s_max, d.se, (uint32_t)f.H, nullptr);
    } else {
      const uint32_t eb = std::min<uint32_t>(div_round_up(d.s_max, 256), (uint32_t)Runtime::get().n_cus * 8u);
      gt_sample_kernel<<<eb, 256, 0, d.se>>>(ring.ctr + D_SAMPLES, d.p.volume, d.p.vol_dims, ring.queue, (float*)ring.arena);
      VNR_HIP_CHECK(hipGetLastError());
    }
    if (profiling_) VNR_HIP_CHECK(hipEventRecord(events_[f.slot][h][2 * it + 1], d.se));
    VNR_HIP_CHECK(hipEventRecord(d.ev(d.ev_e, it), d.se));
    ++d.it_w;
    return;
  }
  if (!head_only && d.it_c < d.it_w) {
    const uint32_t it = d.it_c;
    const DRing& ring = d.ring[it % RING];
    VNR_HIP_CHECK(hipStreamWaitEvent(d.sc, d.ev(d.ev_e, it), 0));
    const uint32_t blocks = std::min<uint32_t>(div_round_up(d.p.n_local, 256), 2048u);
    compose_kernel<<<blocks, 256, f.shmem_compose, d.sc>>>(d.p, d.rays, ring, d.host, it);
    VNR_HIP_CHECK(hipGetLastError());
    VNR_HIP_CHECK(hipEventRecord(d.ev(d.ev_c, it), d.sc));
    ++d.it_c;
  }
}

void Renderer::finish_decoupled(StreamingFrame& f)
{
  if (!f.pending) return;
  f.pending = false;
  const int H = f.H;
  for (;;) {
    bool more = false;
    for (int h = 0; h < H; ++h) {
      DPart& d = f.dpart[h];
      if (d.done) continue;
      for (;;) {
        const uint32_t bw = d.it_w, bc = d.it_c;
        decoupled_step(f, h, false);
        if (d.it_w == bw && d.it_c == bc) break;
      }
    }
    for (int h = 0; h < H; ++h) {
      DPart& d = f.dpart[h];
      if (d.done) continue;
      if (d.it_c == 0 || d.it_w == 0) throw std::runtime_error("internal: a decoupled frame with nothing enqueued");
      VNR_HIP_CHECK(hipEventSynchronize(d.ev(d.ev_c, d.it_c - 1)));
      if (d.host->walking[(d.it_w - 1) & 255u] == 0 || d.it_w >= f.max_iterations) { d.done = true; continue; }
      ++d.target;
      more = true;
    }
    if (!more) break;
  }
  uint32_t pass_iterations = 0, launched[kMaxParts] = {};
  uint64_t n_samples = 0, n_ref = 0;
  for (int h = 0; h < H; ++h) {
    DPart& d = f.dpart[h];
    f.mark(h);
    uint32_t used = 0;
    while (used < d.it_w && used < 256u) { ++used; if (d.host->walking[(used - 1) & 255u] == 0) break; }
    decoupled_predicted_[h] = used;
    uint32_t with_samples = 0;
    for (uint32_t it = 0; it < used; ++it) {
      n_samples += d.host->n_smp[it & 255u];
      n_ref += d.host->n_ref[it & 255u];
      if (d.host->n_ref[it & 255u]) with_samples = it + 1;
    }
    pass_iterations = std::max(pass_iterations, with_samples);
    stats_.n_rays_hit += d.host->hit;
    launched[h] = d.it_w;
    if (profiling_) stats_.infer_kernel_launches += with_samples;
  }
  collect_eval_profile(f, launched, nullptr);
  stats_.n_iterations += pass_iterations;
  stats_.n_samples += n_samples;
  stats_.n_reference_slots += n_ref * (uint64_t)f.p_all.n_iters;
  completed_stats_ = stats_;
}

const float* Renderer::map_frame()
{
  finish_pending();
  if (distributed_) {
    issue_gather(fb_cur_);
    VNR_HIP_CHECK(hipEventSynchronize(ev_gathered_[fb_cur_]));
    const float* out = skip_download_ ? (const float*)full_[fb_cur_].ptr : (const float*)host_fb_[fb_cur_];
    fb_cur_ ^= 1;
    return out;
  }
  VNR_HIP_CHECK(hipStreamSynchronize(stream_));
  const float* out = skip_download_ ? (const float*)fb_[fb_cur_].ptr : (const float*)host_fb_[fb_cur_];
  fb_cur_ ^= 1;
  return out;
}

}
```

Baseline: 273.6.

## Add atomic per-XCD tile claiming with cross-XCD stealing to queued inference kernel

Queued neural evaluation now has waves claim tiles dynamically through per-XCD atomic counters, and steal from other XCDs' ranges once their own runs out, in place of a static strided split. The launch no longer scales its block count from the expected tile count when claiming is on. The MLP weights are staged into LDS with async global_load_lds so the copy overlaps the first tile's encoding instead of blocking it. Claim counters are added to the render counter blocks and reset by the ray-packing prologue. This is meant to fix load imbalance from variable sample counts, at the cost of atomics per tile and larger counter buffers.

```diff
diff --git a/include/vnr_amd.h b/include/vnr_amd.h
--- a/include/vnr_amd.h
+++ b/include/vnr_amd.h
@@ -120,6 +120,8 @@
 int    vnrAmdNeuralVolumeSerializeParams(vnrAmdVolume, void** bson, size_t* size);
 
 int    vnrAmdNeuralVolumeInference(vnrAmdVolume, size_t n, const float* d_coords, float* d_values, void* stream);
+int    vnrAmdNeuralVolumeInferenceQueue(vnrAmdVolume, const float* d_records, const uint32_t* d_n, size_t n_max, unsigned parts, float* d_values,
+                                        uint32_t* d_claim, void* stream);
 int    vnrAmdNeuralVolumeEncode(vnrAmdVolume, size_t n, const float* d_coords, uint16_t* d_features, void* stream);
 int    vnrAmdNeuralVolumeBrickImageInfo(vnrAmdVolume, int* in_use, size_t* bytes, float* build_ms);
 int    vnrAmdNeuralVolumeSetBrickImageMode(vnrAmdVolume, int mode);
diff --git a/instantvnr_amd/_lib.py b/instantvnr_amd/_lib.py
--- a/instantvnr_amd/_lib.py
+++ b/instantvnr_amd/_lib.py
@@ -129,6 +129,7 @@
     sig("vnrAmdNeuralVolumeDecodedDeviceData", P, P)
     sig("vnrAmdNeuralVolumeSerializeParams", I, P, C.POINTER(P), C.POINTER(SZ))
     sig("vnrAmdNeuralVolumeInference", I, P, SZ, P, P, P)
+    sig("vnrAmdNeuralVolumeInferenceQueue", I, P, P, P, SZ, C.c_uint, P, P, P)
     sig("vnrAmdNeuralVolumeEncode", I, P, SZ, P, P, P)
     sig("vnrAmdNeuralVolumeBrickImageInfo", I, P, IP, C.POINTER(SZ), FP)
     sig("vnrAmdNeuralVolumeGetInfo", I, P, IP, IP, IP, IP, IP, C.POINTER(U64))
diff --git a/instantvnr_amd/api.py b/instantvnr_amd/api.py
--- a/instantvnr_amd/api.py
+++ b/instantvnr_amd/api.py
@@ -600,6 +600,29 @@
     return o.numpy()
 
 
+def neural_inference_queue(v, coords, n_max=None, parts=1, launches=1):
+    coords = np.ascontiguousarray(coords, dtype=np.float32)
+    n = coords.shape[0]
+    n_max = n if n_max is None else int(n_max)
+    if n_max < n:
+        raise ValueError("n_max is smaller than the number of records")
+    rec = np.zeros((max(n_max, 1), 4), np.uint32)
+    rec[:n, :3] = coords.view(np.uint32)
+    rec[:, 3] = np.arange(rec.shape[0], dtype=np.uint32)
+    r = DeviceArray.from_numpy(rec)
+    cnt = DeviceArray.from_numpy(np.array([n], np.uint32))
+    claim = DeviceArray.from_numpy(np.full(8, 0xdeadbeef, np.uint32))
+    out = None
+    for _ in range(launches):
+        o = DeviceArray.from_numpy(np.full(rec.shape[0], np.nan, np.float32))
+        check(lib().vnrAmdNeuralVolumeInferenceQueue(v.h, r.ptr, cnt.ptr, n_max, parts, o.ptr, claim.ptr, None))
+        check(lib().vnrAmdSynchronize())
+        out = o.numpy()
+        if not np.isnan(out[n:]).all():
+            raise VnrAmdError("the evaluation launch wrote results for records beyond its count")
+    return out[:n]
+
+
 def neural_encode(v, coords):
     info = neural_info(v)
     c = DeviceArray.from_numpy(np.ascontiguousarray(coords, dtype=np.float32))
diff --git a/instantvnr_amd/csrc/capi.cpp b/instantvnr_amd/csrc/capi.cpp
--- a/instantvnr_amd/csrc/capi.cpp
+++ b/instantvnr_amd/csrc/capi.cpp
@@ -556,6 +556,18 @@
     nv->inference(n, d_coords, d_values, resolve_stream(stream));
   });
 }
+int vnrAmdNeuralVolumeInferenceQueue(vnrAmdVolume v, const float* d_records, const uint32_t* d_n, size_t n_max, unsigned parts, float* d_values,
+                                     uint32_t* d_claim, void* stream)
+{
+  return guarded([&]() {
+    NeuralVolume* nv = as_neural(v);
+    if (!nv->network().valid()) throw std::runtime_error("network is not valid");
+    if (!d_records || !d_n || !d_values || !d_claim) throw std::runtime_error("vnrAmdNeuralVolumeInferenceQueue: null pointer");
+    hipStream_t s = resolve_stream(stream);
+    VNR_HIP_CHECK(hipMemsetAsync(d_claim, 0, 8 * sizeof(uint32_t), s));
+    nv->network().inference_queue(d_records, d_values, 1, d_n, n_max, s, parts ? parts : 1u, nullptr, d_claim);
+  });
+}
 int vnrAmdNeuralVolumeEncode(vnrAmdVolume v, size_t n, const float* d_coords, uint16_t* d_features, void* stream)
 {
   return guarded([&]() { as_neural(v)->network().encode(d_coords, d_features, n, resolve_stream(stream)); });
diff --git a/instantvnr_amd/csrc/decoupled.h b/instantvnr_amd/csrc/decoupled.h
--- a/instantvnr_amd/csrc/decoupled.h
+++ b/instantvnr_amd/csrc/decoupled.h
@@ -7,7 +7,7 @@
   float* alpha; vec3f* color; uint32_t* done;
 };
 
-enum { D_SAMPLES = 0, D_WALKING, D_HIT, D_TICKET_W, D_TICKET_C, D_NREF, D_NSMP, D_COUNT = 8 };
+enum { D_SAMPLES = 0, D_WALKING, D_HIT, D_TICKET_W, D_TICKET_C, D_NREF, D_NSMP, D_CLAIM = 8, D_COUNT = 16 };
 constexpr uint32_t kRecValid = 1u << 16, kRecLast = 1u << 17;
 
 struct DRing {
diff --git a/instantvnr_amd/csrc/infer_kernel.h b/instantvnr_amd/csrc/infer_kernel.h
--- a/instantvnr_amd/csrc/infer_kernel.h
+++ b/instantvnr_amd/csrc/infer_kernel.h
@@ -39,6 +39,7 @@
   uint32_t weights_global;
   float quantize_threshold;
   PackArgs pack;
+  uint32_t* claim;
 };
 
 template <int F, int K_IN, int W, int MODE, bool GENERAL>
@@ -63,16 +64,25 @@
   const uint32_t xcd = blockIdx.x & 7u;
   const uint32_t per_xcd = (n_tiles + 7u) >> 3;
   const uint32_t waves_per_xcd = (gridDim.x >> 3) * WAVES;
-  const uint32_t tile_end = min(n_tiles, (xcd + 1u) * per_xcd);
-  if (xcd * per_xcd + (blockIdx.x >> 3) * WAVES >= tile_end) return;
+  const bool claimed = MODE == 0 && args.claim != nullptr;
+  if (claimed ? n_tiles == 0u : xcd * per_xcd + (blockIdx.x >> 3) * WAVES >= min(n_tiles, (xcd + 1u) * per_xcd)) return;
 
   constexpr bool CAN_GLOBAL = GENERAL;
   const bool wglobal = CAN_GLOBAL && args.weights_global != 0u;
-  if (MODE != 1 && !wglobal) {
-    const uint4_t* src = (const uint4_t*)args.packed_mlp;
-    uint4_t* dst = (uint4_t*)lds;
-    for (uint32_t i = threadIdx.x; i < args.lds_halves / 8; i += blockDim.x) dst[i] = src[i];
-    __syncthreads();
+  uint32_t cx = xcd, tried = 0, pend = 0;
+  uint32_t opaque0;
+  asm volatile("v_mov_b32 %0, 0" : "=v"(opaque0));
+  auto claim_issue = [&](uint32_t c) { uint32_t t = 0; if (lane == 0) t = atomicAdd(args.claim + c + opaque0, 1u); return t; };
+  if (claimed) pend = claim_issue(cx);
+
+  bool staged = MODE == 1 || wglobal;
+  if (!staged) {
+    const uint32_t n16 = args.lds_halves / 8u;
+    const uint8_t* src = (const uint8_t*)args.packed_mlp;
+    for (uint32_t base = wave * 64u; base < n16; base += 64u * WAVES)
+      if (base + lane < n16)
+        __builtin_amdgcn_global_load_lds((const __attribute__((address_space(1))) void*)(src + (size_t)(base + lane) * 16u),
+                                         (__attribute__((address_space(3))) void*)((uint8_t*)lds + base * 16u), 16, 0, 0);
   }
   const uint32_t nh = args.n_hidden_matmuls;
   const uint32_t act = args.activation;
@@ -80,29 +90,49 @@
   const uint32_t r = lane & 31u;
   const table_rsrc_t rsrc = make_table_rsrc(args.table, args.table_bytes);
 
-  for (uint32_t tile = xcd * per_xcd + (blockIdx.x >> 3) * WAVES + wave; tile < tile_end; tile += waves_per_xcd) {
+  uint32_t tile = xcd * per_xcd + (blockIdx.x >> 3) * WAVES + wave, tile_end = min(n_tiles, (xcd + 1u) * per_xcd);
+  for (;; tile += waves_per_xcd) {
+    if (claimed) {
+      tile = cx * per_xcd + (uint32_t)__builtin_amdgcn_readfirstlane((int)pend);
+      tile_end = min(n_tiles, (cx + 1u) * per_xcd);
+      while (tile >= tile_end && ++tried < 8u) {
+        cx = (cx + 1u) & 7u;
+        tile = cx * per_xcd + (uint32_t)__builtin_amdgcn_readfirstlane((int)claim_issue(cx));
+        tile_end = min(n_tiles, (cx + 1u) * per_xcd);
+      }
+    }
+    const bool have = tile < tile_end;
     const uint32_t i = tile * 64u + lane;
-    const uint32_t ic = min(i, n - 1u);
-    float3_packed p;
     uint32_t out_index = i;
-    if (args.queue_mode) {
-      const uint4_t rec = ((const uint4_t*)args.coords)[ic];
-      p = {__uint_as_float(rec.x), __uint_as_float(rec.y), __uint_as_float(rec.z)};
-      out_index = rec.w * args.out_stride;
-    } else {
-      p = ((const float3_packed*)args.coords)[ic];
-      if (args.dest) out_index = args.dest[ic];
+    half8_t feat[NCHUNK];
+    if (have) {
+      const uint32_t ic = min(i, n - 1u);
+      float3_packed p;
+      if (args.queue_mode) {
+        const uint4_t rec = ((const uint4_t*)args.coords)[ic];
+        if (claimed) pend = claim_issue(cx);
+        p = {__uint_as_float(rec.x), __uint_as_float(rec.y), __uint_as_float(rec.z)};
+        out_index = rec.w * args.out_stride;
+      } else {
+        p = ((const float3_packed*)args.coords)[ic];
+        if (args.dest) out_index = args.dest[ic];
+      }
+
+      encode_tile<F, K_IN, GENERAL>(args.levels, args.n_levels, args.interpolation, rsrc, args.brick_image, p.x, p.y, p.z, feat,
+                                    GENERAL ? args.quantize_threshold : 0.0f);
+
+      if (MODE != 0 && args.features_out && i < n) {
+        half8_t* dst = (half8_t*)(args.features_out + (size_t)i * K_IN);
+#pragma unroll
+        for (int c = 0; c < NCHUNK; ++c) dst[c] = feat[c];
+      }
     }
-
-    half8_t feat[NCHUNK];
-    encode_tile<F, K_IN, GENERAL>(args.levels, args.n_levels, args.interpolation, rsrc, args.brick_image, p.x, p.y, p.z, feat,
-                                  GENERAL ? args.quantize_threshold : 0.0f);
-
-    if (MODE != 0 && args.features_out && i < n) {
-      half8_t* dst = (half8_t*)(args.features_out + (size_t)i * K_IN);
-#pragma unroll
-      for (int c = 0; c < NCHUNK; ++c) dst[c] = feat[c];
+    if (!staged) {
+      asm volatile("s_waitcnt vmcnt(0)" ::: "memory");
+      __syncthreads();
+      staged = true;
     }
+    if (!have) break;
     if (MODE == 1) continue;
 
     float y;
@@ -129,7 +159,8 @@
   const size_t shmem = (MODE == 1 || a.weights_global) ? 16 : (size_t)a.lds_halves * sizeof(uint16_t);
   const uint32_t fit = (uint32_t)std::max<size_t>(1, std::min<size_t>(4, (160 * 1024) / std::max<size_t>(shmem, 1)));
   uint32_t max_blocks = (uint32_t)rt.n_cus * (forced ? forced : std::min(fit, a.sharers >= 2 ? 3u : 4u));
-  if (!forced && a.n_ptr && a.queue_mode) max_blocks = std::min((uint32_t)rt.n_cus * 32u, std::max((uint32_t)rt.n_cus * 4u, n_tiles / 33u));
+  const bool claimed = MODE == 0 && a.claim && a.n_ptr && a.queue_mode;
+  if (!forced && !claimed && a.n_ptr && a.queue_mode) max_blocks = std::min((uint32_t)rt.n_cus * 32u, std::max((uint32_t)rt.n_cus * 4u, n_tiles / 33u));
   if (blocks > max_blocks) blocks = max_blocks;
   blocks = next_multiple(blocks, 8);
   auto kernel = fused_infer_kernel<F, K_IN, W, MODE, GENERAL>;
diff --git a/instantvnr_amd/csrc/network.h b/instantvnr_amd/csrc/network.h
--- a/instantvnr_amd/csrc/network.h
+++ b/instantvnr_amd/csrc/network.h
@@ -111,7 +111,7 @@
                  const uint32_t* d_dest = nullptr) const;
   bool tile_net(TileNet* out, hipStream_t s) const;
   bool inference_queue(const float* d_records, float* d_out, uint32_t out_stride, const uint32_t* d_n, size_t n_max, hipStream_t s,
-                       uint32_t sharers = 1, const PackArgs* pack = nullptr) const;
+                       uint32_t sharers = 1, const PackArgs* pack = nullptr, uint32_t* d_claim = nullptr) const;
   void encode(const float* d_coords, uint16_t* d_features, size_t n, hipStream_t s) const;
 
   void forward_backward(const float* d_coords, const float* d_targets, size_t batch, hipStream_t s, GradExchange* exchange = nullptr);
diff --git a/instantvnr_amd/csrc/network_host.hip b/instantvnr_amd/csrc/network_host.hip
--- a/instantvnr_amd/csrc/network_host.hip
+++ b/instantvnr_amd/csrc/network_host.hip
@@ -12,7 +12,7 @@
 void launch_fused(int mode, const GridDevice& grid, uint32_t in_width, const FusedMlp& mlp, const LevelInfo* d_levels, const uint16_t* table, size_t table_bytes,
                   const float* coords, float* out, uint16_t* features_out, uint16_t* acts_out, size_t n, const uint32_t* d_n, size_t n_max, hipStream_t s,
                   const uint32_t* d_dest = nullptr, uint32_t queue_out_stride = 0, const uint8_t* brick_image = nullptr,
-                  uint32_t sharers = 1, const struct PackArgs* pack = nullptr);
+                  uint32_t sharers = 1, const struct PackArgs* pack = nullptr, uint32_t* claim = nullptr);
 void launch_init_params(OptState* state, uint16_t* params, size_t n_mlp, size_t n_total, uint32_t in_width,
                         uint32_t n_hidden_matmuls, uint32_t width, uint64_t seed, hipStream_t s);
 void launch_master_from_f16(const uint16_t* params, OptState* state, size_t n, bool reset_optimizer, hipStream_t s);
@@ -608,7 +608,7 @@
 }
 
 bool Network::inference_queue(const float* d_records, float* d_out, uint32_t out_stride, const uint32_t* d_n, size_t n_max, hipStream_t s,
-                              uint32_t sharers, const PackArgs* pack) const
+                              uint32_t sharers, const PackArgs* pack, uint32_t* d_claim) const
 {
   const uint8_t* image;
   const LevelInfo* levels = inference_levels(s, &image, n_max);
@@ -616,7 +616,7 @@
   grid.n_levels = n_active_levels();
   if (cfg_.n_neurons == 128u) pack = nullptr;
   launch_fused(0, grid, in_width_, fused_mlp(), levels, params_f16_.ptr + n_mlp_, n_grid_params() * 2, d_records, d_out, nullptr, nullptr, 0, d_n, n_max, s, nullptr,
-               out_stride, image, sharers, pack);
+               out_stride, image, sharers, pack, d_claim);
   return pack != nullptr;
 }
 
diff --git a/instantvnr_amd/csrc/network_infer.hip b/instantvnr_amd/csrc/network_infer.hip
--- a/instantvnr_amd/csrc/network_infer.hip
+++ b/instantvnr_amd/csrc/network_infer.hip
@@ -62,7 +62,7 @@
 
 void launch_fused(int mode, const GridDevice& grid, uint32_t in_width, const FusedMlp& mlp, const LevelInfo* d_levels, const uint16_t* table, size_t table_bytes,
                   const float* coords, float* out, uint16_t* features_out, uint16_t* acts_out, size_t n, const uint32_t* d_n, size_t n_max, hipStream_t s,
-                  const uint32_t* d_dest, uint32_t queue_out_stride, const uint8_t* brick_image, uint32_t sharers, const PackArgs* pack)
+                  const uint32_t* d_dest, uint32_t queue_out_stride, const uint8_t* brick_image, uint32_t sharers, const PackArgs* pack, uint32_t* claim)
 {
   if (n_max == 0) { if (pack && pack->n_blocks) throw std::runtime_error("internal: ray packing fused into an empty evaluation launch"); return; }
   if (n_max > 0xffffffc0ull) throw std::runtime_error("inference batch too large (max 2^32-64 samples per call)");
@@ -96,6 +96,7 @@
     if (mlp.width == 128u) throw std::runtime_error("internal: the 128-neuron evaluation kernel (8 waves per block) does not take the ray packing prologue");
     a.pack = *pack;
   } else a.pack.n_blocks = 0;
+  a.claim = (mode == 0 && d_n && queue_out_stride) ? claim : nullptr;
   if (mode == 1) {
     if (mlp.general) return dispatch<64, 1, true>(grid.n_features, in_width, a, n_max, s);
     return dispatch<64, 1, false>(grid.n_features, in_width, a, n_max, s);
diff --git a/instantvnr_amd/csrc/network_train.hip b/instantvnr_amd/csrc/network_train.hip
--- a/instantvnr_amd/csrc/network_train.hip
+++ b/instantvnr_amd/csrc/network_train.hip
@@ -5,7 +5,7 @@
 void launch_fused(int mode, const GridDevice& grid, uint32_t in_width, const FusedMlp& mlp, const LevelInfo* d_levels, const uint16_t* table, size_t table_bytes,
                   const float* coords, float* out, uint16_t* features_out, uint16_t* acts_out, size_t n, const uint32_t* d_n, size_t n_max, hipStream_t s,
                   const uint32_t* d_dest = nullptr, uint32_t queue_out_stride = 0, const uint8_t* brick_image = nullptr,
-                  uint32_t sharers = 1, const struct PackArgs* pack = nullptr);
+                  uint32_t sharers = 1, const struct PackArgs* pack = nullptr, uint32_t* claim = nullptr);
 
 struct Pcg32 {
   uint64_t state, inc;
diff --git a/instantvnr_amd/csrc/pack_rays.h b/instantvnr_amd/csrc/pack_rays.h
--- a/instantvnr_amd/csrc/pack_rays.h
+++ b/instantvnr_amd/csrc/pack_rays.h
@@ -21,7 +21,8 @@
   float* alpha[2];
 };
 
-enum { C_RAYS0 = 0, C_RAYS1 = 1, C_SAMPLES0 = 2, C_SAMPLES1 = 3, C_HIT = 4, C_STAT_SAMPLES = 6, C_STAT_REFRAYS = 8, C_COUNT = 16 };
+enum { C_RAYS0 = 0, C_RAYS1 = 1, C_SAMPLES0 = 2, C_SAMPLES1 = 3, C_HIT = 4, C_STAT_SAMPLES = 6, C_STAT_REFRAYS = 8, C_COUNT = 16,
+       C_CLAIM0 = 16, C_WORDS = 32 };
 
 struct PackArgs {
   RayList src, dst;
@@ -46,6 +47,7 @@
   const uint32_t n_in = a.first ? a.n_first : counters[C_RAYS0 + parity];
   const uint32_t n_groups = ((n_in + 255u) & ~255u) >> 6;
   if (item == 0 && tid == 0) counters[C_SAMPLES0 + (parity ^ 1)] = 0;
+  if (item == 0 && tid < 8u) counters[C_CLAIM0 + 8 * (parity ^ 1) + tid] = 0;
   if (n_groups == 0) {
     if (item == 0 && tid == 0) { counters[C_RAYS0 + (parity ^ 1)] = 0; *a.host_alive = 0; }
     if (item == 0 && tid >= C_HIT && tid < C_COUNT) a.host_stats[tid] = counters[tid];
diff --git a/instantvnr_amd/csrc/render.hip b/instantvnr_amd/csrc/render.hip
--- a/instantvnr_amd/csrc/render.hip
+++ b/instantvnr_amd/csrc/render.hip
@@ -655,7 +655,7 @@
   if (const char* e = std::getenv("VNR_AMD_DECOUPLED")) decoupled_mode_ = std::max(0, std::min(2, std::atoi(e)));
   if (const char* e = std::getenv("VNR_AMD_DECOUPLED_AHEAD")) decoupled_ahead_ = std::max(1, std::min(7, std::atoi(e)));
   if (const char* e = std::getenv("VNR_AMD_DECOUPLED_PARTS")) decoupled_parts_ = std::max(1, std::min(kMaxParts, std::atoi(e)));
-  counters_.resize(2 * kMaxParts * C_COUNT);
+  counters_.resize(2 * kMaxParts * C_WORDS);
   counters_.zero(stream_);
   VNR_HIP_CHECK(hipHostMalloc((void**)&host_counts_, 2 * kMaxParts * (256 + C_COUNT) * sizeof(uint32_t), hipHostMallocDefault));
   VNR_HIP_CHECK(hipEventCreateWithFlags(&ev_fork_, hipEventDisableTiming));
@@ -1171,7 +1171,10 @@
     pk.src = hf.rl[1]; pk.dst = hf.rl[0]; pk.ray_counts = hf.rc; pk.n_first = P; pk.counters = c; pk.parity = parity; pk.first = it == 0 ? 1 : 0;
     pk.ssh = ssh ? 1 : 0; pk.grad = grad ? 1 : 0; pk.ssh_lists = hf.ssh; pk.host_alive = hf.hc + (it & 255u); pk.host_stats = hf.hs;
     pk.n_blocks = div_round_up(P, 256);
-    const bool fused_pack = P <= 262144u;
+#if !defined(VNR_FUSED_PACK_MAX_RAYS)
+#define VNR_FUSED_PACK_MAX_RAYS 262144u
+#endif
+    const bool fused_pack = P <= VNR_FUSED_PACK_MAX_RAYS;
     bool packed = false;
     if (!s_it) s_it = hf.s;
     if (profiling_) VNR_HIP_CHECK(hipEventRecord(events_[f.slot][h][2 * it], s_it));
@@ -1183,7 +1186,7 @@
     if (skip_eval) {
     } else if (nv) {
       packed = nv->network().inference_queue((const float*)hf.queue, (float*)hf.vd[parity], 1, c + C_SAMPLES0 + parity, hf.s_max, s_it, (uint32_t)H,
-                                             fused_pack ? &pk : nullptr);
+                                             fused_pack ? &pk : nullptr, c + C_CLAIM0 + 8 * parity);
     } else {
       const uint32_t blocks = std::min<uint32_t>(div_round_up(hf.s_max, 256), (uint32_t)Runtime::get().n_cus * 8u);
       gt_sample_kernel<<<blocks, 256, 0, s_it>>>(c + C_SAMPLES0 + parity, hf.p.volume, hf.p.vol_dims, hf.queue, (float*)hf.vd[parity]);
@@ -1241,7 +1244,7 @@
   uint32_t* const rc_base = ray_counts_.ptr + (size_t)slot * n_groups_slot;
   vec4f* const queue_base = queue_.ptr + (size_t)slot * rec_per_slot * QP * QI;
   float* const arena_base = arena_.ptr + (size_t)slot * 2 * slot_floats * QP * QI;
-  uint32_t* const counters_base = counters_.ptr + (size_t)slot * kMaxParts * C_COUNT;
+  uint32_t* const counters_base = counters_.ptr + (size_t)slot * kMaxParts * C_WORDS;
   uint32_t* const host_base = host_counts_ + (size_t)slot * kMaxParts * (256 + C_COUNT);
   size_t off = 0;
   for (int h = 0; h < H; ++h) {
@@ -1274,7 +1277,7 @@
     }
     hf.p.slot_cap = (uint32_t)((size_t)hf.p.n_local * QI);
     hf.queue = queue_base + rec_per_slot * off * QI;
-    hf.c = counters_base + (size_t)h * C_COUNT;
+    hf.c = counters_base + (size_t)h * C_WORDS;
     hf.rc = rc_base + off / 64 + (size_t)h * 8;
     hf.hc = host_base + (size_t)h * 256;
     hf.hs = host_base + kMaxParts * 256 + (size_t)h * C_COUNT;
@@ -1285,7 +1288,7 @@
   }
 
   f.params_generation = nv ? nv->network().params_generation() : 0;
-  VNR_HIP_CHECK(hipMemsetAsync(counters_base, 0, (size_t)H * C_COUNT * sizeof(uint32_t), stream_));
+  VNR_HIP_CHECK(hipMemsetAsync(counters_base, 0, (size_t)H * C_WORDS * sizeof(uint32_t), stream_));
   if (H > 1) {
     VNR_HIP_CHECK(hipEventRecord(ev_fork_, stream_));
     for (int h = 1; h < H; ++h) VNR_HIP_CHECK(hipStreamWaitEvent(part_streams_[h], ev_fork_, 0));
@@ -1580,7 +1583,7 @@
 #endif
     if (skip_eval) {
     } else if (f.nv) {
-      f.nv->network().inference_queue((const float*)ring.queue, (float*)ring.arena, 1, ring.ctr + D_SAMPLES, d.s_max, d.se, (uint32_t)f.H, nullptr);
+      f.nv->network().inference_queue((const float*)ring.queue, (float*)ring.arena, 1, ring.ctr + D_SAMPLES, d.s_max, d.se, (uint32_t)f.H, nullptr, ring.ctr + D_CLAIM);
     } else {
       const uint32_t eb = std::min<uint32_t>(div_round_up(d.s_max, 256), (uint32_t)Runtime::get().n_cus * 8u);
       gt_sample_kernel<<<eb, 256, 0, d.se>>>(ring.ctr + D_SAMPLES, d.p.volume, d.p.vol_dims, ring.queue, (float*)ring.arena);
```

Result: slower. 93.61 (-65.8%).
